# HSG-AIML/MaskedSST

Measured on AMD Instinct MI355X. Metric: pretrain samples/sec, higher is better.
Workload: dtype bf16; 1 GPU; SimMIM pretrain step (fwd+bwd+AdamW), EnMAP-shape cubes 8x8x200, depth 12x2, dim 96, heads 8, mlp 64, mask 0.7/4/tube, dropout 0.1; global_batch=256, per_gpu_batch=256, parallelism=dp1

## Files before the change

include/msst.h:

```cpp
#ifndef MSST_H
#define MSST_H
#include <stdint.h>

#ifdef __cplusplus
extern "C" {
#endif

#define MSST_VERSION 109
#define MSST_DIM 96
#define MSST_DIM_HEAD 64
#define MSST_MLP 64

#define MSST_PREC_F32 0
#define MSST_PREC_BF16 1

#define MSST_KERNEL_GENERIC (16 << 8)
#define MSST_KERNEL_FWD_4WAVE (64 << 8)
#define MSST_X1_BF16 (1024 << 8)
#define MSST_FWD_HALF (4096 << 8)
#define MSST_LSE_RENORM (8192 << 8)
#define MSST_LN1_FROM_XN (2048 << 8)
#define MSST_BWD_DEFER_REDUCE (512 << 8)
#define MSST_KERNEL_ATTN_R3 (128 << 8)

// ... 54 lines not shown
                            const float* b_emb, const float* post_g, const float* post_b, const float* dx0, float* slab,
                            int nchunk, float* dpre_g, float* dpre_b, float* dw_emb, float* db_emb, float* dpost_g,
                            float* dpost_b, float* dpos_a, float* dpos_b, int pos_split, int Bs, int Hs, int Ws, int window,
                            int stride, long win0, int nwin, int S, int P, float emb_dropout_p, uint32_t seed, void* stream);

int msst_tokenize_at_fwd(const float* scene, const int32_t* origins, const float* pre_g, const float* pre_b, const float* w_emb,
                         const float* b_emb, const float* post_g, const float* post_b, const float* pos_a, const float* pos_b,
                         int pos_split, float* out, int Bs, int Hs, int Ws, int window, int nwin, int S, int P,
                         float emb_dropout_p, uint32_t seed, void* stream);
int msst_tokenize_at_bwd(const float* scene, const int32_t* origins, const float* pre_g, const float* pre_b, const float* w_emb,
                         const float* b_emb, const float* post_g, const float* post_b, const float* dx0, float* slab, int nchunk,
                         float* dpre_g, float* dpre_b, float* dw_emb, float* db_emb, float* dpost_g, float* dpost_b, float* dpos_a,
                         float* dpos_b, int pos_split, int Bs, int Hs, int Ws, int window, int nwin, int S, int P,
                         float emb_dropout_p, uint32_t seed, void* stream);

int msst_tokenize_at_fwd_masked(const float* scene, const int32_t* origins, const float* pre_g, const float* pre_b, const float* w_emb,
                                const float* b_emb, const float* post_g, const float* post_b, const float* pos_a, const float* pos_b,
                                int pos_split, const float* mask_token, const uint8_t* mask, float* out, int Bs, int Hs, int Ws,
                                int window, int nwin, int S, int P, void* stream);
int msst_tokenize_at_bwd_masked(const float* scene, const int32_t* origins, const float* pre_g, const float* pre_b, const float* w_emb,
                                const float* b_emb, const float* post_g, const float* post_b, const uint8_t* mask, const float* dx0,
                                float* slab, int nchunk, float* dpre_g, float* dpre_b, float* dw_emb, float* db_emb, float* dpost_g,
                                float* dpost_b, float* dpos_a, float* dpos_b, int pos_split, float* dmask_token, int Bs, int Hs, int Ws,
                                int window, int nwin, int S, int P, void* stream);
int msst_head_at_fwd(const float* y, const float* scene, const int32_t* origins, const int32_t* idx, const float* w_pix,
                     const float* b_pix, int per_block, float* dpred, float* pred , float* partial, float* loss, int Bs,
                     int Hs, int Ws, int window, int nwin, int S, int P, int K, void* stream);

int msst_tokenize_at_fwd_orient(const float* scene, const int32_t* origins, const uint8_t* orient, const float* pre_g, const float* pre_b,
                                const float* w_emb, const float* b_emb, const float* post_g, const float* post_b, const float* pos_a,
                                const float* pos_b, int pos_split, float* out, int Bs, int Hs, int Ws, int window, int nwin, int S, int P,
                                float emb_dropout_p, uint32_t seed, void* stream);
int msst_tokenize_at_bwd_orient(const float* scene, const int32_t* origins, const uint8_t* orient, const float* pre_g, const float* pre_b,
                                const float* w_emb, const float* b_emb, const float* post_g, const float* post_b, const float* dx0,
                                float* slab, int nchunk, float* dpre_g, float* dpre_b, float* dw_emb, float* db_emb, float* dpost_g,
                                float* dpost_b, float* dpos_a, float* dpos_b, int pos_split, int Bs, int Hs, int Ws, int window, int nwin,
                                int S, int P, float emb_dropout_p, uint32_t seed, void* stream);
int msst_tokenize_at_fwd_masked_orient(const float* scene, const int32_t* origins, const uint8_t* orient, const float* pre_g,
                                       const float* pre_b, const float* w_emb, const float* b_emb, const float* post_g,
                                       const float* post_b, const float* pos_a, const float* pos_b, int pos_split,
                                       const float* mask_token, const uint8_t* mask, float* out, int Bs, int Hs, int Ws, int window,
                                       int nwin, int S, int P, void* stream);
int msst_tokenize_at_bwd_masked_orient(const float* scene, const int32_t* origins, const uint8_t* orient, const float* pre_g,
                                       const float* pre_b, const float* w_emb, const float* b_emb, const float* post_g,
                                       const float* post_b, const uint8_t* mask, const float* dx0, float* slab, int nchunk, float* dpre_g,
                                       float* dpre_b, float* dw_emb, float* db_emb, float* dpost_g, float* dpost_b, float* dpos_a,
                                       float* dpos_b, int pos_split, float* dmask_token, int Bs, int Hs, int Ws, int window, int nwin,
                                       int S, int P, void* stream);
int msst_head_at_fwd_orient(const float* y, const float* scene, const int32_t* origins, const uint8_t* orient, const int32_t* idx,
                            const float* w_pix, const float* b_pix, int per_block, float* dpred, float* pred , float* partial,
                            float* loss, int Bs, int Hs, int Ws, int window, int nwin, int S, int P, int K, void* stream);

int msst_scene_assemble(const float* win_logits, long win0, int nwin, float* logits, int64_t* classes, int Bs,
                        int n_classes, int Hs, int Ws, int window, int stride, int finalize, void* stream);

int msst_tokenize_scene_fwd_masked(const float* scene, const float* pre_g, const float* pre_b, const float* w_emb,
                                   const float* b_emb, const float* post_g, const float* post_b, const float* pos_a,
                                   const float* pos_b, int pos_split, const float* mask_token, const uint8_t* scene_mask, float* out,
                                   int Bs, int Hs, int Ws, int window, int stride, long win0, int nwin, int S, int P, void* stream);

int msst_scene_recon_assemble(const float* win_recon, long win0, int nwin, const float* scene, const uint8_t* scene_mask, float* cube,
                              double* band_err , int32_t* band_cnt , int32_t* cover, int Bs, int S, int P,
                              int Hs, int Ws, int window, int stride, int finalize, int blend, void* stream);

int msst_pool_spectral_fwd(const float* y, float* out, int B, int S, int N, void* stream);

int msst_scene_embed_assemble(const float* win_feat, long win0, int nwin, float* feat, int32_t* cover, int Bs, int D, int Hs, int Ws,
                              int window, int stride, int finalize, int l2norm, void* stream);

#define MSST_ATTN_PER_SEQ 0
#define MSST_ATTN_MEAN_SEQ 1
int msst_attn_maps(const float* x, const float* ln_g, const float* ln_b, const float* wqkv, float* maps, long sample_stride, int mode,
                   int B, int S, int N, int heads, int reduce, void* stream);

#define MSST_SAVED_XN 1
#define MSST_SAVED_LSE 2
#define MSST_SAVED_RSTD 4
long msst_block_lse_floats(int mode, int B, int S, int N, int heads);
long msst_block_tiles(int mode, int B, int S, int N);
int msst_block_fwd(const MsstBlockWeights* w , const float* x, float* y, float* x1, int mode,
                   int B, int S, int N, int heads, int prec, int max_grid, float dropout_p, uint32_t seed,
                   int layer, void* xn_out, float* lse_out, int* saved , void* stream);

int msst_block_fwd_stack(const MsstBlockWeights* const* w , int nblk, const float* x0, float* const* y ,
                         float* const* x1 , void* const* xn_out , float* const* lse_out , int mode,
                         int B, int S, int N, int heads, int prec, int max_grid, float dropout_p, uint32_t seed, int layer0,
                         int* saved , void* stream);

int msst_head_fwd(const float* y, const float* img, const int32_t* idx, const float* w_pix,
                  const float* b_pix, int per_block, float* dpred, float* pred, float* partial,
                  float* loss, int B, int S, int N, int P, int K, void* stream);

int msst_recon_fwd(const float* y, const float* img, const uint8_t* mask, const float* w_pix, const float* b_pix, int per_block,
                   int blend, float* recon, double* band_err , int32_t* band_cnt , int B, int S, int N,
                   int P, void* stream);


int msst_head_bwd(const float* y, const float* dpred, const int32_t* csr_ptr, const int32_t* csr_pos,
                  const float* w_pix, int per_block, float gscale, const float* gout, float* dy, float* slab,
                  int nchunk, float* dw_pix, float* db_pix, int B, int S, int N, int P, int K, void* stream);

typedef struct MsstBlockGrads {
    float* ln1_g; float* ln1_b; float* wqkv; float* wout; float* bo;
    float* ln2_g; float* ln2_b; float* w1; float* b1; float* w2; float* b2;
} MsstBlockGrads;

#define MSST_MLP_SLAB (64 * 96 + 96 * 64 + 64 + 96 + 96 + 96)
#define MSST_ATTN_SLAB (3 * 64 * 96 + 96 * 64)
#define MSST_LN1_SLAB 288

int msst_block_bwd(const MsstBlockWeights* w , const MsstBlockGrads* g , const float* x,
                   const float* x1, const float* dy, float* dx, float* dx1, void* dxn_part, float* slab,
                   int grid_rows, int nchunk, int mode, int B, int S, int N, int heads, int prec,
                   float dropout_p, uint32_t seed, int layer, const void* xn_saved ,
                   const float* lse_saved ,
                   void* dab_ws ,
                   void* stream);

#define MSST_TILE_QUEUE_WORDS 64
int msst_block_bwd_chain(const MsstBlockWeights* w , const MsstBlockGrads* g ,
                         const MsstBlockWeights* w_prev , const MsstBlockGrads* g_prev ,
                         const float* x, const float* x1, const float* x1_prev, const float* dy, float* dx, float* dx1,
                         void* dxn_part, float* slab, int grid_rows, int nchunk, int mode, int B, int S, int N, int heads,
                         int prec, float dropout_p, uint32_t seed, int layer, const void* xn_saved, const float* lse_saved ,
                         void* dab_ws, int first, int32_t* tile_queue , void* stream);

int msst_block_bwd_reduce(const MsstBlockGrads* g , const MsstBlockGrads* g_prev ,
                          float* slab, long slab_stride, long grad_stride, int count, int count_prev, int first,
                          int grid_rows, int nchunk, int mode, int B, int S, int N, int heads, int prec, void* stream);

int msst_tokenize_bwd(const float* img, const float* pre_g, const float* pre_b, const float* w_emb,
                      const float* b_emb, const float* post_g, const float* post_b, const uint8_t* mask,
                      const float* dx0, float* slab, int nchunk, float* dpre_g, float* dpre_b,
                      float* dw_emb, float* db_emb, float* dpost_g, float* dpost_b, float* dpos_a,
                      float* dpos_b, int pos_split, float* dmask_token, int B, int S, int N, int P,
                      float emb_dropout_p, uint32_t seed, void* stream);

int msst_tokenize_bwd_input(const float* img, const float* pre_g, const float* pre_b, const float* w_emb, const float* b_emb,
                            const float* post_g, const float* post_b, const uint8_t* mask , const float* dx0,
                            const float* dtarget , float* dimg, int B, int S, int N, int P, float emb_dropout_p,
                            uint32_t seed, void* stream);
int msst_head_bwd_target(const float* dpred, const int32_t* csr_ptr, const int32_t* csr_pos, const float* gout ,
                         float* dtarget, int B, int S, int N, int P, int K, void* stream);
int msst_tokenize_scene_bwd_input(const float* scene, const float* pre_g, const float* pre_b, const float* w_emb, const float* b_emb,
                                  const float* post_g, const float* post_b, const float* dx0, float* dscene, int Bs, int Hs, int Ws,
                                  int window, int stride, long win0, int nwin, int S, int P, float emb_dropout_p, uint32_t seed,
                                  void* stream);

int msst_tokenize_at_bwd_input(const float* scene, const int32_t* origins, const float* pre_g, const float* pre_b, const float* w_emb,
                               const float* b_emb, const float* post_g, const float* post_b, const float* dx0, float* dwin, int Bs,
                               int Hs, int Ws, int window, int nwin, int S, int P, float emb_dropout_p, uint32_t seed, void* stream);
int msst_scene_fold_at(const float* dwin, const int32_t* cell_ptr, const int32_t* cell_win, float* dscene, int Bs, int C, int Hs, int Ws,
                       int window, int nwin, int group, int accumulate, void* stream);

int msst_cls_head_fwd(const float* y, const float* ln_g, const float* ln_b, const float* w, const float* b,
                      float* logits, int B, int S, int N, int n_classes, void* stream);
int msst_cls_head_bwd(const float* y, const float* dlogits, const float* ln_g, const float* ln_b, const float* w,
                      float* dy, float* slab, float* dln_g, float* dln_b, float* dw, float* db, int B, int S,
                      int N, int n_classes, void* stream);

int msst_spec_head_fwd(const float* y, const float* ln_g, const float* ln_b, const float* w, const float* b,
                       float* logits, int B, int S, int N, int n_classes, void* stream);
long msst_spec_head_bwd_slab(int B, int S, int N, int n_classes);
int msst_spec_head_bwd(const float* y, const float* dlogits, const float* ln_g, const float* ln_b, const float* w,
                       float* dy, float* slab, float* dln_g, float* dln_b, float* dw, float* db, int B, int S,
                       int N, int n_classes, void* stream);
// ... 82 lines not shown
```

maskedsst_amd/_lib.py:

```python
import ctypes
import os
from ctypes import c_int, c_int32, c_uint32, c_long, c_float, c_void_p, c_char_p, POINTER, Structure

HERE = os.path.dirname(os.path.abspath(__file__))
LIB_PATH = os.path.join(HERE, "libmsst.so")
HEADER_PATH = os.path.normpath(os.path.join(HERE, "..", "include", "msst.h"))

PREC_F32 = 0
PREC_BF16 = 1
MODE_SPATIAL = 0
MODE_SPECTRAL = 1
MLP_SLAB = 64 * 96 + 96 * 64 + 64 + 96 + 96 + 96
ATTN_SLAB = 3 * 64 * 96 + 96 * 64
LN1_SLAB = 288


class MsstError(RuntimeError):
    pass


class MsstPrepJob(Structure):
    _fields_ = [("src", c_void_p), ("dst", c_void_p), ("rows", c_int32), ("cols", c_int32),
                ("transpose", c_int32), ("pack", c_int32), ("scale_rows", c_int32), ("scale", c_float)]


class MsstBlockWeights(Structure):
    _fields_ = [("struct_bytes", ctypes.c_uint64)] + [(n, c_void_p) for n in (
        "wqkv", "wout", "w1", "w2", "wqkvT", "woutT", "w1T", "w2T",
        "ln1_g", "ln1_b", "bo", "ln2_g", "ln2_b", "b1", "b2", "wqkv32", "woutT32", "wqkvT32",
        "wqkv_h", "wout_h", "w1_h", "w2_h")]


class MsstBlockGrads(Structure):
    _fields_ = [(n, c_void_p) for n in (
        "ln1_g", "ln1_b", "wqkv", "wout", "bo", "ln2_g", "ln2_b", "w1", "b1", "w2", "b2")]


class MsstAdamGroup(Structure):
    _fields_ = [("start", c_long), ("end", c_long), ("lr", c_float), ("weight_decay", c_float), ("step", c_int), ("flags", c_int)]


class MsstGradRange(Structure):
    _fields_ = [("start", c_long), ("end", c_long)]


_P = c_void_p
GRAD_MAX_RANGES = 64
ADAM_DECOUPLED = 1
ADAM_MAX_GROUPS = 64
BWD_DEFER_REDUCE = 512 << 8
X1_BF16 = 1024 << 8
SAVED_XN, SAVED_LSE, SAVED_RSTD = 1, 2, 4
LN1_FROM_XN = 2048 << 8
FWD_HALF = 4096 << 8
LSE_RENORM = 8192 << 8
PREP_HALF = 256
CE_LOSS_SUM, CE_N_VALID, CE_N_CORRECT, CE_BAD_LABELS, CE_NONFINITE, CE_SUPPORT = range(6)
CE_EXT_LOSS_SUM, CE_EXT_WEIGHT_SUM = range(2)
CE_CONFUSION_MAX_CLASSES = 128
ATTN_PER_SEQ, ATTN_MEAN_SEQ = 0, 1
_SIGS = {
    "msst_version": (c_int, []),
    "msst_last_error": (c_char_p, []),
    "msst_prep_weights": (c_int, [_P, c_int, c_int, c_int, c_int, _P, _P]),
    "msst_tokenize_fwd": (c_int, [_P] * 9 + [c_int, _P, _P, _P, c_int, c_int, c_int, c_int, c_float, c_uint32, _P]),
    "msst_tokenize_scene_fwd": (c_int, [_P] * 9 + [c_int, _P, c_int, c_int, c_int, c_int, c_int, c_long, c_int, c_int, c_int, _P]),
    "msst_tokenize_scene_fwd_train": (c_int, [_P] * 9 + [c_int, _P, c_int, c_int, c_int, c_int, c_int, c_long, c_int, c_int, c_int,
                                              c_float, c_uint32, _P]),
    "msst_tokenize_scene_bwd": (c_int, [_P] * 9 + [c_int] + [_P] * 8 + [c_int] * 6 + [c_long, c_int, c_int, c_int, c_float, c_uint32, _P]),
    "msst_tokenize_at_fwd": (c_int, [_P] * 10 + [c_int, _P] + [c_int] * 7 + [c_float, c_uint32, _P]),
    "msst_tokenize_at_bwd": (c_int, [_P] * 10 + [c_int] + [_P] * 8 + [c_int] * 8 + [c_float, c_uint32, _P]),
    "msst_tokenize_at_fwd_masked": (c_int, [_P] * 10 + [c_int, _P, _P, _P] + [c_int] * 7 + [_P]),
    "msst_tokenize_at_bwd_masked": (c_int, [_P] * 11 + [c_int] + [_P] * 8 + [c_int, _P] + [c_int] * 7 + [_P]),
    "msst_head_at_fwd": (c_int, [_P] * 6 + [c_int] + [_P] * 4 + [c_int] * 8 + [_P]),
    "msst_tokenize_at_fwd_orient": (c_int, [_P] * 11 + [c_int, _P] + [c_int] * 7 + [c_float, c_uint32, _P]),
    "msst_tokenize_at_bwd_orient": (c_int, [_P] * 11 + [c_int] + [_P] * 8 + [c_int] * 8 + [c_float, c_uint32, _P]),
    "msst_tokenize_at_fwd_masked_orient": (c_int, [_P] * 11 + [c_int, _P, _P, _P] + [c_int] * 7 + [_P]),
    "msst_tokenize_at_bwd_masked_orient": (c_int, [_P] * 12 + [c_int] + [_P] * 8 + [c_int, _P] + [c_int] * 7 + [_P]),
    "msst_head_at_fwd_orient": (c_int, [_P] * 7 + [c_int] + [_P] * 4 + [c_int] * 8 + [_P]),
    "msst_tokenize_bwd_input": (c_int, [_P] * 11 + [c_int] * 4 + [c_float, c_uint32, _P]),
    "msst_head_bwd_target": (c_int, [_P] * 5 + [c_int] * 5 + [_P]),
    "msst_tokenize_scene_bwd_input": (c_int, [_P] * 9 + [c_int] * 5 + [c_long, c_int, c_int, c_int, c_float, c_uint32, _P]),
    "msst_tokenize_at_bwd_input": (c_int, [_P] * 10 + [c_int] * 7 + [c_float, c_uint32, _P]),
    "msst_scene_fold_at": (c_int, [_P] * 4 + [c_int] * 8 + [_P]),
    "msst_tokenize_scene_fwd_masked": (c_int, [_P] * 9 + [c_int, _P, _P, _P, c_int, c_int, c_int, c_int, c_int, c_long, c_int, c_int, c_int, _P]),
    "msst_scene_recon_assemble": (c_int, [_P, c_long, c_int, _P, _P, _P, _P, _P, _P] + [c_int] * 9 + [_P]),
    "msst_pool_spectral_fwd": (c_int, [_P, _P, c_int, c_int, c_int, _P]),
    "msst_scene_embed_assemble": (c_int, [_P, c_long, c_int, _P, _P] + [c_int] * 8 + [_P]),
    "msst_attn_maps": (c_int, [_P, _P, _P, _P, _P, c_long, c_int, c_int, c_int, c_int, c_int, c_int, _P]),
    "msst_scene_assemble": (c_int, [_P, c_long, c_int, _P, _P, c_int, c_int, c_int, c_int, c_int, c_int, c_int, _P]),
    "msst_cls_head_fwd": (c_int, [_P] * 6 + [c_int, c_int, c_int, c_int, _P]),
    "msst_cls_head_bwd": (c_int, [_P] * 11 + [c_int, c_int, c_int, c_int, _P]),
    "msst_spec_head_fwd": (c_int, [_P] * 6 + [c_int, c_int, c_int, c_int, _P]),
    "msst_spec_head_bwd_slab": (c_long, [c_int, c_int, c_int, c_int]),
    "msst_spec_head_bwd": (c_int, [_P] * 11 + [c_int, c_int, c_int, c_int, _P]),
    "msst_pix_head_fwd_ws": (c_long, [c_int, c_int]),
    "msst_pix_head_fwd": (c_int, [_P] * 7 + [c_int, c_int, c_int, c_int, _P]),
    "msst_pix_head_bwd_slab": (c_long, [c_int, c_int, c_int, c_int]),
    "msst_pix_head_bwd": (c_int, [_P] * 11 + [c_int, c_int, c_int, c_int, _P]),
    "msst_scene_centre_assemble": (c_int, [_P, c_long, c_int, _P, _P, c_int, c_int, c_int, c_int, c_int, c_int, c_int, _P]),
    "msst_block_lse_floats": (c_long, [c_int, c_int, c_int, c_int, c_int]),
    "msst_block_tiles": (c_long, [c_int, c_int, c_int, c_int]),
    "msst_block_fwd": (c_int, [POINTER(MsstBlockWeights), _P, _P, _P, c_int, c_int, c_int, c_int, c_int,
                               c_int, c_int, c_float, c_uint32, c_int, _P, _P, POINTER(c_int), _P]),
    "msst_block_fwd_stack": (c_int, [_P, c_int, _P, _P, _P, _P, _P, c_int, c_int, c_int, c_int, c_int, c_int, c_int, c_float, c_uint32, c_int,
                                     POINTER(c_int), _P]),
    "msst_head_fwd": (c_int, [_P, _P, _P, _P, _P, c_int, _P, _P, _P, _P, c_int, c_int, c_int, c_int,
                              c_int, _P]),
    "msst_head_bwd": (c_int, [_P, _P, _P, _P, _P, c_int, c_float, _P, _P, _P, c_int, _P, _P, c_int, c_int, c_int,
                              c_int, c_int, _P]),
    "msst_block_bwd": (c_int, [POINTER(MsstBlockWeights), POINTER(MsstBlockGrads), _P, _P, _P, _P, _P, _P, _P,
                               c_int, c_int, c_int, c_int, c_int, c_int, c_int, c_int, c_float, c_uint32, c_int, _P, _P, _P, _P]),
    "msst_block_bwd_chain": (c_int, [POINTER(MsstBlockWeights), POINTER(MsstBlockGrads), POINTER(MsstBlockWeights),
                                     POINTER(MsstBlockGrads), _P, _P, _P, _P, _P, _P, _P, _P,
                                     c_int, c_int, c_int, c_int, c_int, c_int, c_int, c_int, c_float, c_uint32, c_int, _P, _P, _P,
                                     c_int, _P, _P]),
    "msst_block_bwd_reduce": (c_int, [POINTER(MsstBlockGrads), POINTER(MsstBlockGrads), _P, ctypes.c_long, ctypes.c_long,
                                      c_int, c_int, c_int, c_int, c_int, c_int, c_int, c_int, c_int, c_int, c_int, _P]),
    "msst_tokenize_bwd": (c_int, [_P] * 10 + [c_int] + [_P] * 8 + [c_int, _P, c_int, c_int, c_int, c_int, c_float,
                                  c_uint32, _P]),
    "msst_debug_stamps": (c_int, [_P]),
    "msst_debug_cu_thief": (c_int, [c_int, c_int, _P, _P]),
    "msst_debug_box_probe": (c_int, [_P, _P, c_long, _P]),
    "msst_profile_enable": (c_int, [c_int]),
    "msst_profile_select": (c_int, [ctypes.c_ulonglong]),
    "msst_profile_sample": (c_int, [c_int]),
    "msst_profile_kernels": (c_int, []),
    "msst_profile_name": (c_char_p, [c_int]),
    "msst_profile_collect": (c_int, [_P, _P]),
    "msst_layernorm_fwd": (c_int, [_P, _P, _P, _P, _P, _P, c_long, c_int, c_float, _P]),
    "msst_layernorm_bwd_slab": (c_long, [c_long, c_int]),
    "msst_layernorm_bwd": (c_int, [_P, _P, _P, _P, _P, _P, _P, c_long, c_int, c_float, _P]),
    "msst_ce_scratch_bytes": (c_long, [c_int, c_int, c_int]),
    "msst_ce_stats_fwd": (c_int, [_P, _P, _P, c_long, _P, _P, _P, _P, c_int, c_int, c_int, _P]),
    "msst_ce_bwd": (c_int, [_P, _P, _P, _P, c_int, c_int, c_int, _P]),
    "msst_ce_ext_scratch_bytes": (c_long, [c_int, c_int, c_int, c_int]),
    "msst_ce_ext_fwd": (c_int, [_P, _P, _P, c_long, _P, c_float, _P, _P, _P, _P, _P, _P, c_int, c_int, c_int, _P]),
    "msst_ce_ext_bwd": (c_int, [_P, _P, _P, _P, c_int, c_int, c_int, _P]),
    "msst_recon_fwd": (c_int, [_P, _P, _P, _P, _P, c_int, c_int, _P, _P, _P, c_int, c_int, c_int, c_int, _P]),
    "msst_adamw": (c_int, [_P, _P, _P, _P, c_long, c_float, c_float, c_float, c_float, c_float, c_int,
                           c_float, c_float, _P]),
    "msst_adam_groups": (c_int, [_P, _P, _P, _P, POINTER(MsstAdamGroup), c_int, c_int, ctypes.c_double, ctypes.c_double,
                                 c_float, c_float, _P]),
    "msst_grad_accum_scratch_bytes": (c_long, [c_int]),
    "msst_grad_accumulate": (c_int, [_P, _P, POINTER(MsstGradRange), c_int, c_int, c_int, _P, c_float, _P, _P]),
    "msst_grad_finalize": (c_int, [_P, _P, POINTER(MsstGradRange), c_int, c_int, c_float, c_float, _P, _P, _P]),
}

_lib = None


def declared_symbols():
    return sorted(_SIGS)


def header_version(path=None):
    import re
    with open(path or HEADER_PATH) as f:
        m = re.search(r"^#define\s+MSST_VERSION\s+(\d+)", f.read(), re.M)
    if not m:
        raise MsstError(f"no MSST_VERSION in {path or HEADER_PATH}")
    return int(m.group(1))


def load():
    global _lib
    if _lib is not None:
        return _lib
    if not os.path.exists(LIB_PATH):
        raise MsstError(
            f"{LIB_PATH} not found: build the HIP extension first (python -m maskedsst_amd.build). "
            "maskedsst_amd has no CPU / eager fallback.")
    lib = ctypes.CDLL(LIB_PATH)
    for name, (res, args) in _SIGS.items():
        fn = getattr(lib, name, None)
        if fn is None:
            raise MsstError(f"libmsst.so does not export {name} (stale build? run python -m maskedsst_amd.build)")
        fn.restype = res
        fn.argtypes = args
    got, want = int(lib.msst_version()), header_version()
    if got == -want and os.environ.get("MSST_ALLOW_LAB") == "1":
        import warnings
        warnings.warn("maskedsst_amd: loading a -DMSST_LAB kernel-study build (results may be wrong by design)")
        got = want
    if got != want:
        raise MsstError(
            f"{LIB_PATH} reports msst_version() = {got}, include/msst.h says MSST_VERSION {want}: "
# ... 11 lines not shown
```

maskedsst_amd/build.py:

```python
import os
import subprocess
import sys
from concurrent.futures import ThreadPoolExecutor

HERE = os.path.dirname(os.path.abspath(__file__))
CSRC = os.path.join(HERE, "csrc")
LIB = os.path.join(HERE, "libmsst.so")
SOURCES = ["msst_fwd.hip", "msst_fwd3.hip", "msst_bwd.hip", "msst_bwd3.hip", "msst_bwd4.hip", "msst_bwd5.hip", "msst_ln.hip", "msst_opt.hip", "msst_accum.hip", "msst_head.hip", "msst_pixhead.hip", "msst_loss.hip", "msst_recon.hip", "msst_scene_recon.hip", "msst_scene_embed.hip", "msst_input_grad.hip", "msst_attn_maps.hip", "msst_api.hip"]
HEADERS = ["msst_dev.h", "msst_kernels.h", os.path.join("..", "..", "include", "msst.h")]
FLAGS = ["--offload-arch=gfx950", "-O3", "-std=c++17", "-fPIC", "-fno-gpu-rdc", "-Wno-unused-result"]


def _hipcc():
    for c in (os.environ.get("HIPCC"), "/opt/rocm/bin/hipcc", "hipcc"):
        if c and (os.path.isabs(c) and os.path.exists(c) or not os.path.isabs(c)):
            return c
    return "hipcc"


def _stale(target, deps):
    if not os.path.exists(target):
        return True
    t = os.path.getmtime(target)
    return any(os.path.getmtime(d) > t for d in deps if os.path.exists(d))


def build(force=False, verbose=False, extra_flags=(), lib=None, tag=None):
    srcs = [os.path.join(CSRC, s) for s in SOURCES if os.path.exists(os.path.join(CSRC, s))]
    hdrs = [os.path.normpath(os.path.join(CSRC, h)) for h in HEADERS]
    objdir = os.path.join(HERE, "build", tag) if tag else os.path.join(HERE, "build")
    LIB = lib or globals()["LIB"]
    os.makedirs(objdir, exist_ok=True)
    hipcc = _hipcc()

    def compile_one(src):
        obj = os.path.join(objdir, os.path.basename(src) + ".o")
        if force or _stale(obj, [src] + hdrs):
            cmd = [hipcc] + FLAGS + list(extra_flags) + ["-c", src, "-o", obj]
            if verbose:
                print(" ".join(cmd), flush=True)
            r = subprocess.run(cmd, capture_output=True, text=True)
            if r.returncode != 0:
                raise RuntimeError(f"hipcc failed for {src}:\n{r.stdout}\n{r.stderr}")
        return obj

    with ThreadPoolExecutor(max_workers=4) as ex:
        objs = list(ex.map(compile_one, srcs))
    if force or _stale(LIB, objs):
        cmd = [hipcc, "--offload-arch=gfx950", "-shared", "-fPIC", "-o", LIB] + objs
        if verbose:
            print(" ".join(cmd), flush=True)
        r = subprocess.run(cmd, capture_output=True, text=True)
        if r.returncode != 0:
            raise RuntimeError(f"link failed:\n{r.stdout}\n{r.stderr}")
    return LIB


if __name__ == "__main__":
    print(build(force="--force" in sys.argv or "--stamps" in sys.argv, verbose=True,
                extra_flags=("-DMSST_STAMPS",) if "--stamps" in sys.argv else ()))
```

maskedsst_amd/csrc/msst_api.hip:

```cpp
#include "../../include/msst.h"
#include "msst_kernels.h"
#include <stdio.h>
#include <stdlib.h>
#include <string.h>
#include <math.h>
#include <atomic>
#include <mutex>
#include <vector>

namespace msst {

static thread_local char g_err[256] = "";

static int fail(int code, const char* what) {
    if (code > 0) snprintf(g_err, sizeof(g_err), "%s: hip error %d (%s)", what, code, hipGetErrorString((hipError_t)code));
    else if (code < 0) snprintf(g_err, sizeof(g_err), "%s: msst error %d", what, code);
    return code;
}

template <class E>
__global__ __launch_bounds__(256) void prep_weights_kernel(const MsstPrepJob* jobs, int* err_flag) {
    const MsstPrepJob j = jobs[blockIdx.y];
    const bool half = sizeof(E) == 2 && (j.pack & MSST_PREP_HALF);
    if (j.pack < 0 || (j.pack & ~MSST_PREP_HALF) > 1 || (sizeof(E) != 2 && (j.pack & MSST_PREP_HALF)) || j.rows < 1 || j.cols < 1) {
// ... 434 lines not shown
    hipStream_t st = (hipStream_t)stream;
    int rc = launch_scene_fold(a, win_logits, logits, n_classes, 16, scene_call_rows(a, wps), st);
    if (!rc && finalize) rc = launch_scene_finalize(a, st);
    return fail(rc, "msst_scene_assemble");
}

int msst_scene_recon_assemble(const float* win_recon, long win0, int nwin, const float* scene, const uint8_t* scene_mask, float* cube,
                              double* band_err, int32_t* band_cnt, int32_t* cover, int Bs, int S, int P, int Hs, int Ws, int window,
                              int stride, int finalize, int blend, void* stream) {
    if (Bs < 1 || S < 1 || P < 1 || Hs < 1 || Ws < 1 || window < 1 || stride < 1 || nwin < 0 || win0 < 0)
        return fail(MSST_ERR_BADARG, "msst_scene_recon_assemble");
    if (stride > window || window > Hs || window > Ws || window * window > 64 || S > 64 || P > 16)
        return fail(MSST_ERR_UNSUPPORTED, "msst_scene_recon_assemble (1 <= stride <= window <= Hs, Ws; window * window <= 64, S <= 64, P <= 16)");
    if ((nwin > 0 && !win_recon) || !scene || !scene_mask || !cube || !cover || (band_err == nullptr) != (band_cnt == nullptr))
        return fail(MSST_ERR_BADARG, "msst_scene_recon_assemble (null argument, or one of band_err / band_cnt without the other)");
    int nr = 0, nq = 0;
    scene_grid(Bs, Hs, Ws, window, stride, &nr, &nq);
    const long wps = (long)nr * nq;
    if (win0 + nwin > (long)Bs * wps) return fail(MSST_ERR_BADARG, "msst_scene_recon_assemble (windows out of range)");
    if (((long)Bs * Hs * Ws + 255) / 256 > 0x7fffffffL || (long)Bs * S * P > 0x7fffffffL) return fail(MSST_ERR_UNSUPPORTED, "msst_scene_recon_assemble (scene batch too large)");
    SceneReconArgs a;
    fill_grid(a, win0, nwin, Bs, Hs, Ws, window, stride, nr, nq);
    a.win_recon = win_recon; a.scene = scene; a.scene_mask = scene_mask; a.cube = cube; a.band_err = band_err; a.band_cnt = band_cnt;
    a.cover = cover; a.S = S; a.P = P; a.blend = blend != 0;
    hipStream_t st = (hipStream_t)stream;
    int rc = launch_scene_fold(a, win_recon, cube, S * P, P, scene_call_rows(a, wps), st);
    if (!rc && finalize) rc = launch_scene_recon_finalize(a, st);
    return fail(rc, "msst_scene_recon_assemble");
}

int msst_pool_spectral_fwd(const float* y, float* out, int B, int S, int N, void* stream) {
    if (B < 1 || S < 1 || N < 1) return fail(MSST_ERR_BADARG, "msst_pool_spectral_fwd");
    if (N > 64 || S > 64) return fail(MSST_ERR_UNSUPPORTED, "msst_pool_spectral_fwd (N <= 64, S <= 64)");
    if (!y || !out || ((uintptr_t)y & 15)) return fail(MSST_ERR_BADARG, "msst_pool_spectral_fwd (null argument, or y not 16-byte aligned)");
    return fail(launch_pool_spectral(y, out, B, S, N, (hipStream_t)stream), "msst_pool_spectral_fwd");
}

int msst_attn_maps(const float* x, const float* ln_g, const float* ln_b, const float* wqkv, float* maps, long sample_stride, int mode,
                   int B, int S, int N, int heads, int reduce, void* stream) {
    if (B < 1 || S < 1 || N < 1 || heads < 1) return fail(MSST_ERR_BADARG, "msst_attn_maps");
    if (N > 64 || S > 64 || heads > 16) return fail(MSST_ERR_UNSUPPORTED, "msst_attn_maps (N <= 64, S <= 64, heads <= 16)");
    if ((mode != MSST_MODE_SPATIAL && mode != MSST_MODE_SPECTRAL) || (reduce != MSST_ATTN_PER_SEQ && reduce != MSST_ATTN_MEAN_SEQ))
        return fail(MSST_ERR_BADARG, "msst_attn_maps (mode or reduce outside {0, 1})");
    if (!x || !ln_g || !ln_b || !wqkv || !maps || ((uintptr_t)x & 15) || ((uintptr_t)maps & 15))
        return fail(MSST_ERR_BADARG, "msst_attn_maps (null argument, or x / maps not 16-byte aligned)");
    const long L = mode == MSST_MODE_SPATIAL ? N : S, G = mode == MSST_MODE_SPATIAL ? S : N;
    if (sample_stride < (reduce == MSST_ATTN_PER_SEQ ? G : 1) * heads * L * L)
        return fail(MSST_ERR_BADARG, "msst_attn_maps (sample_stride smaller than one sample's maps)");
    return fail(launch_attn_maps(x, ln_g, ln_b, wqkv, maps, sample_stride, mode, B, S, N, heads, reduce, (hipStream_t)stream),
                "msst_attn_maps");
}

int msst_scene_embed_assemble(const float* win_feat, long win0, int nwin, float* feat, int32_t* cover, int Bs, int D, int Hs, int Ws,
                              int window, int stride, int finalize, int l2norm, void* stream) {
    if (Bs < 1 || D < 1 || Hs < 1 || Ws < 1 || window < 1 || stride < 1 || nwin < 0 || win0 < 0)
        return fail(MSST_ERR_BADARG, "msst_scene_embed_assemble");
    if (stride > window || window > Hs || window > Ws || window * window > 64 || D > 128)
        return fail(MSST_ERR_UNSUPPORTED, "msst_scene_embed_assemble (1 <= stride <= window <= Hs, Ws; window * window <= 64, D <= 128)");
    if ((nwin > 0 && !win_feat) || !feat || (finalize && !cover)) return fail(MSST_ERR_BADARG, "msst_scene_embed_assemble (null argument)");
    int nr = 0, nq = 0;
    scene_grid(Bs, Hs, Ws, window, stride, &nr, &nq);
    const long wps = (long)nr * nq;
    if (win0 + nwin > (long)Bs * wps) return fail(MSST_ERR_BADARG, "msst_scene_embed_assemble (windows out of range)");
    if (((long)Bs * Hs * Ws + 255) / 256 > 0x7fffffffL) return fail(MSST_ERR_UNSUPPORTED, "msst_scene_embed_assemble (scene batch too large)");
    SceneEmbedArgs a;
    fill_grid(a, win0, nwin, Bs, Hs, Ws, window, stride, nr, nq);
    a.win_feat = win_feat; a.feat = feat; a.cover = cover; a.D = D; a.l2norm = l2norm != 0;
    hipStream_t st = (hipStream_t)stream;
    int rc = launch_scene_fold(a, win_feat, feat, D, 16, scene_call_rows(a, wps), st);
    if (!rc && finalize) rc = launch_scene_embed_finalize(a, st);
    return fail(rc, "msst_scene_embed_assemble");
}

long msst_block_lse_floats(int mode, int B, int S, int N, int heads) {
    if (B < 1 || S < 1 || N < 1 || heads < 1 || N > 64 || S > 64) return 0;
    return (long)ntiles_of(make_tilemap(mode, B, S, N)) * heads * 64 + (long)B * S * N;
}

long msst_block_tiles(int mode, int B, int S, int N) {
    if (B < 1 || S < 1 || N < 1 || N > 64 || S > 64) return 0;
    return (long)ntiles_of(make_tilemap(mode, B, S, N));
}

int msst_block_fwd(const MsstBlockWeights* w, const float* x, float* y, float* x1, int mode, int B, int S,
                   int N, int heads, int prec, int max_grid, float dropout_p, uint32_t seed, int layer,
                   void* xn_out, float* lse_out, int* saved, void* stream) {
    if (int rc = block_shape(mode, B, S, N, heads)) return fail(rc, "msst_block_fwd (B, S, N, heads < 1, mode not 0 / 1, or sequence length > 64)");
    if (!bw_ok(w) || !x || !y || x == y) return fail(MSST_ERR_BADARG, "msst_block_fwd (null argument, or MsstBlockWeights of another header revision)");
    const int dbg = (prec >> 8) & 0xffff;
    prec &= 0xff;
    BlockArgs a;
    a.w = to_bw(w);
    a.x = x; a.y = y; a.x1 = x1;
    a.tm = make_tilemap(mode, B, S, N);
    a.ntiles = ntiles_of(a.tm);
    a.max_grid = max_grid > 0 ? max_grid : a.ntiles;
    a.H = heads;
    a.scale = 0.125f;
    a.dbg = dbg & ~8;
    a.stamps = nullptr;
#ifdef MSST_STAMPS
    a.stamps = g_stamps;
    if (g_stamps) a.dbg = dbg;
#elif defined(MSST_LAB)
    a.stamps = g_stamps;
#endif
    a.x1_bf16 = (dbg & 1024) ? 1 : 0;
    if (a.x1_bf16 && !(prec == MSST_PREC_BF16 && heads == 8 && !(dbg & (16 | 64))))
        return fail(MSST_ERR_UNSUPPORTED, "msst_block_fwd (MSST_X1_BF16 needs the role-split bf16 forward: 8 heads, no MSST_KERNEL_* flags)");
    a.half = (dbg & 4096) ? 1 : 0;
    if (a.half) {
        if (!(prec == MSST_PREC_BF16 && heads == 8 && !(dbg & (16 | 64))))
            return fail(MSST_ERR_UNSUPPORTED, "msst_block_fwd (MSST_FWD_HALF needs the role-split bf16 forward: 8 heads, no MSST_KERNEL_* flags)");
        if (!w->wqkv_h || !w->wout_h || !w->w1_h || !w->w2_h) return fail(MSST_ERR_BADARG, "msst_block_fwd (MSST_FWD_HALF without the half weight copies)");
        a.w.wqkv = w->wqkv_h; a.w.wout = w->wout_h; a.w.w1 = w->w1_h; a.w.w2 = w->w2_h;
    }
    a.drop = make_drop(dropout_p, seed, layer);
    a.xn_out = (xn_out && block_fwd_writes_xn(a, prec)) ? xn_out : nullptr;
    a.lse_out = (lse_out && block_fwd_writes_lse(a, prec)) ? lse_out : nullptr;
    if (saved) *saved = (a.xn_out ? MSST_SAVED_XN : 0) | (a.lse_out ? (MSST_SAVED_LSE | MSST_SAVED_RSTD) : 0);
    return fail(launch_block_fwd(a, prec, (hipStream_t)stream), "msst_block_fwd");
}

int msst_block_fwd_stack(const MsstBlockWeights* const* w, int nblk, const float* x0, float* const* y, float* const* x1,
                         void* const* xn_out, float* const* lse_out, int mode, int B, int S, int N, int heads, int prec, int max_grid,
                         float dropout_p, uint32_t seed, int layer0, int* saved, void* stream) {
    if (int rc = block_shape(mode, B, S, N, heads)) return fail(rc, "msst_block_fwd_stack (B, S, N, heads < 1, mode not 0 / 1, or sequence length > 64)");
    if (!w || !x0 || !y || nblk < 1) return fail(MSST_ERR_BADARG, "msst_block_fwd_stack");
    if (nblk > MSST_MAX_STACK) return fail(MSST_ERR_UNSUPPORTED, "msst_block_fwd_stack (more than 16 blocks)");
    const int dbg = (prec >> 8) & 0xffff;
    prec &= 0xff;
    if (prec != MSST_PREC_BF16 || heads != 8 || (dbg & ~(1024 | 4096))) return fail(MSST_ERR_UNSUPPORTED, "msst_block_fwd_stack (bf16, 8 heads, no MSST_KERNEL_* flags)");
    const bool half = (dbg & 4096) != 0;
    for (int j = 0; j < nblk; ++j) {
        if (!bw_ok(w[j])) return fail(MSST_ERR_BADARG, "msst_block_fwd_stack (null block, or MsstBlockWeights of another header revision)");
        if (half && (!w[j]->wqkv_h || !w[j]->wout_h || !w[j]->w1_h || !w[j]->w2_h)) return fail(MSST_ERR_BADARG, "msst_block_fwd_stack (MSST_FWD_HALF without the half weight copies)");
    }
    StackArgs sa;
    BlockArgs& a = sa.base;
    memset(&a.w, 0, sizeof(a.w));
    a.x = x0; a.y = nullptr; a.x1 = nullptr; a.xn_out = nullptr; a.lse_out = nullptr;
    a.tm = make_tilemap(mode, B, S, N);
    a.ntiles = ntiles_of(a.tm);
    a.max_grid = max_grid > 0 ? max_grid : a.ntiles;
    a.H = heads;
    a.scale = 0.125f;
    a.dbg = 0;
    a.stamps = nullptr;
    a.x1_bf16 = (dbg & 1024) ? 1 : 0;
    a.half = half ? 1 : 0;
    a.drop = make_drop(dropout_p, seed, layer0);
    if (lse_out && !block_fwd_writes_lse(a, prec)) lse_out = nullptr;
    sa.nblk = nblk;
    auto blk_of = [&](int j, const float* xin) {
        StackBlk sb;
        sb.wqkv = half ? w[j]->wqkv_h : w[j]->wqkv; sb.wout = half ? w[j]->wout_h : w[j]->wout;
        sb.w1 = half ? w[j]->w1_h : w[j]->w1; sb.w2 = half ? w[j]->w2_h : w[j]->w2;
        sb.ln1_g = w[j]->ln1_g; sb.ln1_b = w[j]->ln1_b; sb.bo = w[j]->bo; sb.ln2_g = w[j]->ln2_g; sb.ln2_b = w[j]->ln2_b; sb.b1 = w[j]->b1; sb.b2 = w[j]->b2;
        sb.x = xin; sb.y = y[j]; sb.x1 = x1 ? x1[j] : nullptr; sb.xn_out = xn_out ? xn_out[j] : nullptr; sb.lse_out = lse_out ? lse_out[j] : nullptr;
        sb.layer = layer0 + j; sb.pad_ = 0;
        return sb;
    };
    for (int j = 0; j < nblk; ++j)
        if (!bw_ok(w[j]) || !y[j] || y[j] == (j ? y[j - 1] : x0))
            return fail(MSST_ERR_BADARG, "msst_block_fwd_stack (null argument, or MsstBlockWeights of another header revision)");
    sa.b0 = blk_of(0, x0);
    memset(&sa.st, 0, sizeof(sa.st));
    bool affine = true;
    if (nblk > 1) {
        const StackBlk b1 = blk_of(1, y[0]);
        auto dist = [&](const void* p1, const void* p0, int& out) {
            const long d = (const char*)p1 - (const char*)p0;
            if (d > 0x7fffffffL || d < -0x7fffffffL) affine = false;
            out = (int)d;
        };
        dist(b1.wqkv, sa.b0.wqkv, sa.st.wqkv); dist(b1.wout, sa.b0.wout, sa.st.wout); dist(b1.w1, sa.b0.w1, sa.st.w1); dist(b1.w2, sa.b0.w2, sa.st.w2);
        dist(b1.ln1_g, sa.b0.ln1_g, sa.st.ln1_g); dist(b1.ln1_b, sa.b0.ln1_b, sa.st.ln1_b); dist(b1.bo, sa.b0.bo, sa.st.bo);
        dist(b1.ln2_g, sa.b0.ln2_g, sa.st.ln2_g); dist(b1.ln2_b, sa.b0.ln2_b, sa.st.ln2_b); dist(b1.b1, sa.b0.b1, sa.st.b1); dist(b1.b2, sa.b0.b2, sa.st.b2);
        dist(b1.y, sa.b0.y, sa.st.y); dist(b1.x1, sa.b0.x1, sa.st.x1); dist(b1.xn_out, sa.b0.xn_out, sa.st.xn_out); dist(b1.lse_out, sa.b0.lse_out, sa.st.lse_out);
        sa.st.x = sa.st.y;
        const float* xin = y[0];
        for (int j = 1; j < nblk && affine; ++j) {
            const StackBlk bj = blk_of(j, xin);
            auto same = [&](const void* pj, const void* p0, int stride) { return !p0 ? !pj : (const char*)pj == (const char*)p0 + (long)j * stride; };
            affine = same(bj.wqkv, sa.b0.wqkv, sa.st.wqkv) && same(bj.wout, sa.b0.wout, sa.st.wout) && same(bj.w1, sa.b0.w1, sa.st.w1) &&
                     same(bj.w2, sa.b0.w2, sa.st.w2) && same(bj.ln1_g, sa.b0.ln1_g, sa.st.ln1_g) && same(bj.ln1_b, sa.b0.ln1_b, sa.st.ln1_b) &&
                     same(bj.bo, sa.b0.bo, sa.st.bo) && same(bj.ln2_g, sa.b0.ln2_g, sa.st.ln2_g) && same(bj.ln2_b, sa.b0.ln2_b, sa.st.ln2_b) &&
                     same(bj.b1, sa.b0.b1, sa.st.b1) && same(bj.b2, sa.b0.b2, sa.st.b2) && same(bj.y, sa.b0.y, sa.st.y) &&
                     same(bj.x1, sa.b0.x1, sa.st.x1) && same(bj.xn_out, sa.b0.xn_out, sa.st.xn_out) && same(bj.lse_out, sa.b0.lse_out, sa.st.lse_out);
            xin = y[j];
        }
    }
    if (!affine) return fail(MSST_ERR_UNSUPPORTED, "msst_block_fwd_stack (per-block operands not a constant stride apart)");
    sa.x_rest = nblk > 1 ? reinterpret_cast<const float*>(reinterpret_cast<const char*>(y[0]) - (long)sa.st.y) : x0;
    if (saved) *saved = (xn_out ? MSST_SAVED_XN : 0) | (lse_out ? (MSST_SAVED_LSE | MSST_SAVED_RSTD) : 0);
    if (a.ntiles < 1) return 0;
    int ncu = 256, dev = 0;
    hipGetDevice(&dev);
    if (hipDeviceGetAttribute(&ncu, hipDeviceAttributeMultiprocessorCount, dev) != hipSuccess || ncu < 1) ncu = 256;
    int grid = a.max_grid < a.ntiles ? a.max_grid : a.ntiles;
    if (grid > ncu) grid = ncu;
    return fail(launch_block_fwd_rs_stack(sa, grid, (hipStream_t)stream), "msst_block_fwd_stack");
}

// ... 831 lines not shown
```

maskedsst_amd/csrc/msst_fwd.hip:

```cpp
#include <atomic>
#include "msst_dev.h"
#include "msst_kernels.h"

namespace msst {

enum { TOK_BATCH = 0, TOK_SCENE = 1, TOK_SCENE_MASKED = 2, TOK_AT = 3, TOK_AT_MASKED = 4, TOK_AT_OR = 5, TOK_AT_OR_MASKED = 6 };
template <int SRC>
__device__ __forceinline__ const float* tok_window_origin(const TokArgs& a, int b) {
    if constexpr (SRC == TOK_AT || SRC == TOK_AT_MASKED || SRC == TOK_AT_OR || SRC == TOK_AT_OR_MASKED) return listed_window_origin(a, b);
    else return scene_window_origin(a, b);
}
template <int PC, int SRC>
__device__ __forceinline__ void tokenize_fwd_body(const TokArgs& a) {
    constexpr bool SCENE = SRC != TOK_BATCH, NOMASK = SRC == TOK_SCENE || SRC == TOK_AT || SRC == TOK_AT_OR;
    constexpr bool ORIENT = SRC == TOK_AT_OR || SRC == TOK_AT_OR_MASKED;
    __shared__ float patch[16][64];
    __shared__ float W[96][17];
    __shared__ float bias[96];
    const int c = blockIdx.x, b = blockIdx.y, tid = threadIdx.x;
    const int P = PC ? PC : a.P, N = a.N;
    if constexpr (SCENE) {
        const long plane = (long)a.Hs * a.Ws;
        const float* src = tok_window_origin<SRC>(a, b) + (long)c * P * plane;
        WinSteps ws{};
// ... 765 lines not shown
                a.dpred[((long)b * a.K + k) * P + p] = d > 0.f ? 1.f : (d < 0.f ? -1.f : 0.f);
                if (a.pred) a.pred[((long)b * a.K + k) * P + p] = pred;
            }
        }
    }
#pragma unroll
    for (int o = 32; o > 0; o >>= 1) lsum += __shfl_xor(lsum, o);
    if ((tid & 63) == 0) red[tid >> 6] = lsum;
    __syncthreads();
    if (tid == 0) a.partial[blockIdx.y * gridDim.x + blockIdx.x] = (red[0] + red[1]) + (red[2] + red[3]);
}

__global__ __launch_bounds__(256) void loss_reduce_kernel(const float* partial, int n, float scale, float* loss) {
    __shared__ double red[256];
    double s = 0.0;
    for (int i = threadIdx.x; i < n; i += 256) s += (double)partial[i];
    red[threadIdx.x] = s;
    __syncthreads();
    for (int o = 128; o > 0; o >>= 1) {
        if (threadIdx.x < o) red[threadIdx.x] += red[threadIdx.x + o];
        __syncthreads();
    }
    if (threadIdx.x == 0) *loss = (float)(red[0] * (double)scale);
}

template <int SRC>
static int launch_tokenize_fwd_src(const TokArgs& a, hipStream_t st) {
    if (a.P > 16 || a.N > 64) return MSST_ERR_UNSUPPORTED;
    if (SRC != TOK_BATCH && a.B < 1) return 0;
    ProfScope ps(K_TOK_FWD, st);
    if (a.P == 10 && a.N == 64) {
        int nchunk = 1024 / (a.S > 0 ? a.S : 1);
        if (nchunk < 1) nchunk = 1;
        if (nchunk > a.B) nchunk = a.B;
        hipLaunchKernelGGL(tokenize_fwd_mfma_kernel<SRC>, dim3(a.S, nchunk), dim3(256), 0, st, a);
    } else {
        if (SRC != TOK_BATCH && a.B > 65535) return MSST_ERR_UNSUPPORTED;
        if (a.P == 10) hipLaunchKernelGGL((tokenize_fwd_kernel<10, SRC>), dim3(a.S, a.B), dim3(256), 0, st, a);
        else hipLaunchKernelGGL((tokenize_fwd_kernel<0, SRC>), dim3(a.S, a.B), dim3(256), 0, st, a);
    }
    return (int)hipGetLastError();
}
int launch_tokenize_fwd(const TokArgs& a, hipStream_t st) { return launch_tokenize_fwd_src<TOK_BATCH>(a, st); }
int launch_tokenize_scene_fwd(const TokArgs& a, hipStream_t st) { return launch_tokenize_fwd_src<TOK_SCENE>(a, st); }
int launch_tokenize_scene_fwd_masked(const TokArgs& a, hipStream_t st) { return launch_tokenize_fwd_src<TOK_SCENE_MASKED>(a, st); }
int launch_tokenize_at_fwd(const TokArgs& a, hipStream_t st) { return launch_tokenize_fwd_src<TOK_AT>(a, st); }
int launch_tokenize_at_fwd_masked(const TokArgs& a, hipStream_t st) { return launch_tokenize_fwd_src<TOK_AT_MASKED>(a, st); }
int launch_tokenize_at_fwd_orient(const TokArgs& a, bool masked, hipStream_t st) {
    return masked ? launch_tokenize_fwd_src<TOK_AT_OR_MASKED>(a, st) : launch_tokenize_fwd_src<TOK_AT_OR>(a, st);
}

template <class P>
static int launch_block_fwd_t(const BlockArgs& a, int grid, hipStream_t st) {
    static std::atomic<bool> attr_set{false};
    const size_t smem = sizeof(FwdSmem<P>);
    if (!attr_set) {
        hipError_t e = hipFuncSetAttribute(reinterpret_cast<const void*>(&block_fwd_kernel<P>),
                                           hipFuncAttributeMaxDynamicSharedMemorySize, (int)smem);
        if (e != hipSuccess) return (int)e;
        attr_set = true;
    }
    ProfScope ps(K_BLOCK_FWD, st);
    hipLaunchKernelGGL(block_fwd_kernel<P>, dim3(grid), dim3(256), smem, st, a);
    return (int)hipGetLastError();
}

static int launch_block_fwd_bf16(const BlockArgs& a, int grid, hipStream_t st) {
    static std::atomic<bool> attr_set{false};
    const size_t smem = sizeof(FwdSmem<PBF16>) + 640 * sizeof(float) + 24 * 1024;
    if (!attr_set) {
        hipError_t e = hipFuncSetAttribute(reinterpret_cast<const void*>(&block_fwd_bf16_kernel),
                                           hipFuncAttributeMaxDynamicSharedMemorySize, (int)smem);
        if (e != hipSuccess) return (int)e;
        attr_set = true;
    }
    ProfScope ps(K_BLOCK_FWD, st);
    hipLaunchKernelGGL(block_fwd_bf16_kernel, dim3(grid), dim3(256), smem, st, a);
    return (int)hipGetLastError();
}

int launch_block_fwd(const BlockArgs& a, int prec, hipStream_t st) {
    if (a.tm.L > 64 || a.tm.L < 1) return MSST_ERR_UNSUPPORTED;
    if (a.ntiles < 1) return 0;
    if (prec == MSST_PREC_F32 || (a.dbg & 16)) {
        const int grid = a.ntiles < a.max_grid ? a.ntiles : a.max_grid;
        return prec == MSST_PREC_F32 ? launch_block_fwd_t<PF32>(a, grid, st) : launch_block_fwd_t<PBF16>(a, grid, st);
    }
    if (a.H == 8 && !(a.dbg & 64)) {
        static std::atomic<int> ncu_cached{0};
        int ncu = ncu_cached.load(std::memory_order_relaxed);
        if (!ncu) {
            int dev = 0;
            hipGetDevice(&dev);
            if (hipDeviceGetAttribute(&ncu, hipDeviceAttributeMultiprocessorCount, dev) != hipSuccess || ncu < 1) ncu = 256;
            ncu_cached.store(ncu, std::memory_order_relaxed);
        }
        int grid = a.max_grid < a.ntiles ? a.max_grid : a.ntiles;
        if (grid > ncu) grid = ncu;
        return launch_block_fwd_rs(a, grid, st);
    }
    int grid = a.max_grid < a.ntiles ? a.max_grid : a.ntiles;
    if (grid > 512) grid = 512;
    return launch_block_fwd_bf16(a, grid, st);
}

bool block_fwd_writes_lse(const BlockArgs& a, int prec) {
    return prec == MSST_PREC_BF16 && a.H == 8 && !(a.dbg & (16 | 64)) && (long)a.ntiles * a.H * 256 < 0x7fffffffL;
}

bool block_fwd_writes_xn(const BlockArgs& a, int prec) {
    return prec == MSST_PREC_BF16 && !(a.dbg & 16);
}

template <bool AT, bool ORIENT = false>
static int launch_head_fwd_src(const HeadArgs& a, float* loss, hipStream_t st) {
    if (a.P > 16) return MSST_ERR_UNSUPPORTED;
    dim3 grid((a.K + 63) / 64, a.B);
    { ProfScope ps(K_HEAD_FWD, st);
    hipLaunchKernelGGL((head_fwd_kernel<AT, ORIENT>), grid, dim3(256), 0, st, a); }
    const int np = grid.x * grid.y;
    const float scale = 1.0f / ((float)a.B * (float)a.K * (float)a.P) / (float)a.K;
    ProfScope ps(K_LOSS_REDUCE, st);
    hipLaunchKernelGGL(loss_reduce_kernel, dim3(1), dim3(256), 0, st, a.partial, np, scale, loss);
    return (int)hipGetLastError();
}
int launch_head_fwd(const HeadArgs& a, float* loss, hipStream_t st) { return launch_head_fwd_src<false>(a, loss, st); }
int launch_head_at_fwd(const HeadArgs& a, float* loss, hipStream_t st) { return launch_head_fwd_src<true>(a, loss, st); }
int launch_head_at_fwd_orient(const HeadArgs& a, float* loss, hipStream_t st) { return launch_head_fwd_src<true, true>(a, loss, st); }

}

namespace msst {

__global__ __launch_bounds__(256) void cls_head_fwd_kernel(ClsArgs a) {
    const int b = blockIdx.x, tid = threadIdx.x, n = tid >> 2, part = tid & 3;
    if (n >= a.N) return;
    float m[24];
#pragma unroll
    for (int i = 0; i < 24; ++i) m[i] = 0.f;
    for (int c = 0; c < a.S; ++c) {
        const f32x4* src = reinterpret_cast<const f32x4*>(a.y + ((long)b * a.T + c * a.N + n) * 96 + part * 24);
#pragma unroll
        for (int i = 0; i < 6; ++i) { const f32x4 t4 = src[i]; m[4*i] += t4[0]; m[4*i+1] += t4[1]; m[4*i+2] += t4[2]; m[4*i+3] += t4[3]; }
    }
    const float invS = 1.f / a.S;
    float s = 0.f;
#pragma unroll
    for (int i = 0; i < 24; ++i) { m[i] *= invS; s += m[i]; }
    s += __shfl_xor(s, 1); s += __shfl_xor(s, 2);
    const float mean = s * (1.f / 96.f);
    float vs = 0.f;
#pragma unroll
    for (int i = 0; i < 24; ++i) { const float d = m[i] - mean; vs += d * d; }
    vs += __shfl_xor(vs, 1); vs += __shfl_xor(vs, 2);
    const float rstd = rsqrtf(vs * (1.f / 96.f) + 1e-5f);
#pragma unroll
    for (int i = 0; i < 24; ++i) m[i] = (m[i] - mean) * rstd * a.ln_g[part * 24 + i] + a.ln_b[part * 24 + i];
    for (int k = 0; k < a.NC; ++k) {
        float acc = 0.f;
#pragma unroll
        for (int i = 0; i < 24; ++i) acc += a.w[k * 96 + part * 24 + i] * m[i];
        acc += __shfl_xor(acc, 1); acc += __shfl_xor(acc, 2);
        if (part == 0) a.logits[((long)b * a.NC + k) * a.N + n] = acc + a.b[k];
    }
}

int launch_cls_head_fwd(const ClsArgs& a, hipStream_t st) {
    if (a.N > 64) return MSST_ERR_UNSUPPORTED;
    hipLaunchKernelGGL(cls_head_fwd_kernel, dim3(a.B), dim3(256), 0, st, a);
    return (int)hipGetLastError();
}

__global__ __launch_bounds__(256) void scene_fold_kernel(SceneGrid a, const float* src, float* dst, int C, int group, long pixels) {
    const long p = (long)blockIdx.x * 256 + threadIdx.x;
    if (p >= pixels) return;
    const int c0 = blockIdx.y * group, cn = min(group, C - c0);
    const long R = a.row0 + p / a.Ws;
    const int x = (int)(p % a.Ws);
    const long s = R / a.Hs;
    const int y = (int)(R - s * a.Hs);
// ... 68 lines not shown
```

maskedsst_amd/csrc/msst_fwd3.hip:

```cpp
#include <atomic>
#include "msst_dev.h"
#include "msst_kernels.h"
#include <type_traits>

#ifndef MSST_F3_RING
#define MSST_F3_RING 4
#endif
#ifndef MSST_F3_RPRIO
#define MSST_F3_RPRIO 1
#endif
#ifndef MSST_F3_BAND
#define MSST_F3_BAND 1
#endif
#ifndef MSST_F3_GROUP
#define MSST_F3_GROUP 10
#endif
#if defined(MSST_LAB) && !defined(MSST_LAB_X1OLD)
#define MSST_LAB_X1OLD 0
#endif
#if !defined(MSST_LAB) || !defined(MSST_LAB_NOLSE)
#define MSST_F3_LSE_STORE 1
#else
#define MSST_F3_LSE_STORE 0
#endif
// ... 37 lines not shown
    int seqb[4][64];
    float lnp[2][640];
    float lseb[2][256];
    char wmlp[24 * 1024];
    const char* blktab[MSST_MAX_STACK][16];
    unsigned steptab[1024];
};
constexpr int F3_MAX_STEPS = 1024;
constexpr int BT_WQKV = 0, BT_W1 = 2, BT_LN1G = 4, BT_X = 11;

struct StepBlk {
    const elem* wqkv; const elem* wout;
    const float* x; float* y; float* x1; elem* xn_out;
    int layer;
};

__device__ __forceinline__ int sopaque3(int v) {
    asm volatile("" : "+s"(v));
    return v;
}

template <bool HALF>
__device__ __forceinline__ s16x4 cv4(f32x4 c) {
    if constexpr (HALF) return f2h4(c); else return f2bf4(c);
}
template <bool HALF>
__device__ __forceinline__ f32x4 mma16(frag a, frag b, f32x4 c) {
    if constexpr (HALF) {
        typedef _Float16 h8 __attribute__((ext_vector_type(8)));
        return __builtin_amdgcn_mfma_f32_16x16x32_f16(__builtin_bit_cast(h8, a), __builtin_bit_cast(h8, b), c, 0, 0, 0);
    } else return P::mma(a, b, c);
}
template <bool HALF>
__device__ __forceinline__ frag pack2f(f32x4 lo, f32x4 hi) {
    const s16x4 a = cv4<HALF>(lo), b = cv4<HALF>(hi);
    frag r;
    r[0] = a[0]; r[1] = a[1]; r[2] = a[2]; r[3] = a[3];
    r[4] = b[0]; r[5] = b[1]; r[6] = b[2]; r[7] = b[3];
    return r;
}

__device__ __forceinline__ frag ld_w_gather3(const elem* w, int K, int row32, int k0, int voff) {
    const int f = (row32 >> 4) * (K >> 5) + (k0 >> 5);
    const __amdgpu_buffer_rsrc_t rs = __builtin_amdgcn_make_buffer_rsrc(const_cast<elem*>(w), 0, 0x7fffffff, 0x00020000);
    const u32x4 v = __builtin_amdgcn_raw_buffer_load_b128(rs, voff, f * 1024, 0);
    return __builtin_bit_cast(frag, v);
}

#ifndef MSST_F3_WOFF
#define MSST_F3_WOFF 1
#endif
__device__ __forceinline__ frag ld_wb3(const elem* w, int voff, int soff) {
    const __amdgpu_buffer_rsrc_t rs = __builtin_amdgcn_make_buffer_rsrc(const_cast<elem*>(w), 0, 0x7fffffff, 0x00020000);
    return __builtin_bit_cast(frag, __builtin_amdgcn_raw_buffer_load_b128(rs, voff, soff, 0));
}
__device__ __forceinline__ void load_pair3(int pi, frag (&out)[2], const elem* wqkv, int H, int h, const int (&voff)[2], int hb, int HB, int l16) {
    if (MSST_F3_WOFF) {
        if (pi < 12) {
            const int st = pi / 3, ks = pi % 3;
            const int o = hb + (st >> 1) * HB + (st & 1) * 6144 + ks * 1024;
            out[0] = ld_wb3(wqkv, l16, o);
            out[1] = ld_wb3(wqkv, l16, o + 3072);
        } else {
            const int mm = (pi - 12) / 3, ks = (pi - 12) % 3;
            const int o = hb + 2 * HB + mm * 6144 + ks * 1024;
            out[0] = ld_wb3(wqkv, voff[0], o);
            out[1] = ld_wb3(wqkv, voff[1], o);
        }
    } else if (pi < 12) {
        const int st = pi / 3, ks = pi % 3;
        const int r0 = ((st >> 1) * H + h) * 64 + (st & 1) * 32;
        out[0] = P::ld_w(wqkv, 96, r0, ks * 32);
        out[1] = P::ld_w(wqkv, 96, r0 + 16, ks * 32);
    } else {
        const int mm = (pi - 12) / 3, ks = (pi - 12) % 3;
        const int r32 = (2 * H + h) * 64 + mm * 32;
        out[0] = ld_w_gather3(wqkv, 96, r32, ks * 32, voff[0]);
        out[1] = ld_w_gather3(wqkv, 96, r32, ks * 32, voff[1]);
    }
}

}

template <bool DROP, bool STACK, bool HALF>
__global__ __launch_bounds__(512, 2) void block_fwd_rs_kernel(typename std::conditional<STACK, StackArgs, BlockArgs>::type args) {
    const BlockArgs& a = [&]() -> const BlockArgs& { if constexpr (STACK) return args.base; else return args; }();
    typedef Fwd3Smem SM;
    constexpr int LDX = SM::LDX, LDH = SM::LDH, LDO = SM::LDO;
    extern __shared__ __attribute__((aligned(16))) char smem_raw[];
    SM& sm = *reinterpret_cast<SM*>(smem_raw);

    const int tid = threadIdx.x, wv = __builtin_amdgcn_readfirstlane(tid >> 6), l = tid & 63, g = l >> 4, c = l & 15;
    const int H = a.H, inner = H * 64;
    const TileMap tm = a.tm;
    const int L = tm.L;
    const int G = (int)gridDim.x;
    const int nmine = ((int)blockIdx.x < a.ntiles) ? (a.ntiles - 1 - (int)blockIdx.x) / G + 1 : 0;
    int nsteps = nmine;
    if constexpr (STACK) {
        const int nblk = args.nblk;
        const int ng = max(1, nmine / MSST_F3_GROUP), gbase = nmine / ng, gextra = nmine - gbase * ng;
        const int p1 = max(gbase + 1, 3), p0 = max(gbase, 3);
        nsteps = nmine ? nblk * (gextra * p1 + (ng - gextra) * p0) : 0;
        for (int s_ = tid; s_ < nsteps; s_ += 512) {
            const int head = gextra * nblk * p1;
            int j, r, pp, sz, before;
            if (s_ < head) { j = s_ / (nblk * p1); r = s_ - j * nblk * p1; pp = p1; sz = gbase + 1; before = j * (gbase + 1); }
            else { j = gextra + (s_ - head) / (nblk * p0); r = s_ - head - (j - gextra) * nblk * p0; pp = p0; sz = gbase; before = gextra * (gbase + 1) + (j - gextra) * gbase; }
            const int blk = r / pp, pos = r - blk * pp;
            const unsigned idle = pos >= sz ? 1u : 0u;
            sm.steptab[s_] = (unsigned)(before + min(pos, sz - 1)) | ((unsigned)blk << 16) | ((unsigned)((j * nblk + blk) & 1) << 24) | (idle << 31);
        }
    }
    if constexpr (STACK) {
        static_assert(offsetof(StackBlk, lse_out) == 15 * 8 && offsetof(StackStride, lse_out) == 15 * 4, "blktab follows StackBlk's member order");
        for (int e = tid; e < args.nblk * 16; e += 512) {
            const int j = e >> 4, f = e & 15;
            auto kp = (const __attribute__((address_space(4))) char*)__builtin_amdgcn_kernarg_segment_ptr();
            const char* p0 = *(const char* const __attribute__((address_space(4)))*)(kp + offsetof(StackArgs, b0) + f * 8);
            const int stride = *(const int __attribute__((address_space(4)))*)(kp + offsetof(StackArgs, st) + f * 4);
            const char* pj = p0 ? p0 + (long)j * stride : nullptr;
            if (f == BT_X && j) pj = reinterpret_cast<const char*>(args.x_rest) + (long)j * args.st.y;
            sm.blktab[j][f] = pj;
        }
    }
    constexpr unsigned F3_IDLE = 0x80000000u;
    auto load_word = [&](int k) -> unsigned {
        if constexpr (STACK) return (k >= 0 && k < nsteps) ? (unsigned)__builtin_amdgcn_readfirstlane((int)sm.steptab[k]) : F3_IDLE;
        else return (k >= 0 && k < nmine) ? (unsigned)k : F3_IDLE;
    };
    int kc = 0;
    unsigned swm2 = F3_IDLE, swm1 = F3_IDLE, sw0 = F3_IDLE, swp1 = F3_IDLE, swp2 = F3_IDLE;
    auto step_word = [&](int k) -> unsigned {
        if constexpr (!STACK) return load_word(k);
        else { const int d = k - kc; return d == 0 ? sw0 : d == 1 ? swp1 : d == -1 ? swm1 : d == 2 ? swp2 : d == -2 ? swm2 : load_word(k); }
    };
    auto words_init = [&]() { kc = 0; swm2 = F3_IDLE; swm1 = F3_IDLE; sw0 = load_word(0); swp1 = load_word(1); swp2 = load_word(2); };
    auto words_advance = [&]() { swm2 = swm1; swm1 = sw0; sw0 = swp1; swp1 = swp2; swp2 = load_word(kc + 3); };
    auto tile_at = [&](int k) -> int {
        const unsigned w_ = step_word(k);
        return (w_ >> 31) ? -1 : (int)blockIdx.x + (int)(w_ & 0xffffu) * G;
    };
    auto blk_at = [&](int k) -> int { if constexpr (STACK) return (int)((step_word(k) >> 16) & 0xffu); else return 0; };
    auto slot_at = [&](int k) -> int { if constexpr (STACK) return (int)((step_word(k) >> 24) & 1u); else return 0; };
    auto in_walk = [&](int k) -> bool { return k >= 0 && k < nsteps; };
    auto epoch_differs = [&](int k1, int k0) -> bool {
        if constexpr (STACK) return in_walk(k1) && in_walk(k0) && ((step_word(k1) ^ step_word(k0)) & 0x01ff0000u) != 0u;
        else return false;
    };
    auto at_blk = [&](const void* p0, int stride, int blk) -> const char* { return reinterpret_cast<const char*>(p0) + (long)blk * (long)stride; };
    auto step_blk = [&](int k) -> StepBlk {
        StepBlk q;
        if constexpr (STACK) {
            const int j = blk_at(k);
            const StackBlk& b0 = args.b0;
            const StackStride& st = args.st;
            q.wqkv = reinterpret_cast<const elem*>(at_blk(b0.wqkv, st.wqkv, j)); q.wout = reinterpret_cast<const elem*>(at_blk(b0.wout, st.wout, j));
            q.x = reinterpret_cast<const float*>(sm.blktab[j][BT_X]);
            q.y = reinterpret_cast<float*>(const_cast<char*>(sm.blktab[j][BT_X + 1]));
            q.x1 = reinterpret_cast<float*>(const_cast<char*>(sm.blktab[j][BT_X + 2]));
            q.xn_out = reinterpret_cast<elem*>(const_cast<char*>(sm.blktab[j][BT_X + 3]));
            q.layer = b0.layer + j;
        } else {
            q.wqkv = reinterpret_cast<const elem*>(a.w.wqkv); q.wout = reinterpret_cast<const elem*>(a.w.wout);
            q.x = a.x; q.y = a.y; q.x1 = a.x1; q.xn_out = reinterpret_cast<elem*>(a.xn_out); q.layer = a.drop.layer;
        }
        return q;
    };
    auto drop_at = [&](int k) -> Drop { Drop d = a.drop; if constexpr (STACK) d.layer = args.b0.layer + blk_at(k); return d; };
    auto lnp_at = [&](int k) -> const float* { return sm.lnp[slot_at(k)]; };
    struct LnpRegs { float v[7]; };
    auto fetch_lnp = [&](int blk, int t96) -> LnpRegs {
        const float *g1, *b1_, *bo, *g2, *b2_, *bb2, *bb1;
        if constexpr (STACK) {
            auto fp_ = [&](int f) { return reinterpret_cast<const float*>(sm.blktab[blk][f]); };
            g1 = fp_(BT_LN1G); b1_ = fp_(BT_LN1G + 1); bo = fp_(BT_LN1G + 2); g2 = fp_(BT_LN1G + 3); b2_ = fp_(BT_LN1G + 4); bb1 = fp_(BT_LN1G + 5); bb2 = fp_(BT_LN1G + 6);
        }
        else { g1 = a.w.ln1_g; b1_ = a.w.ln1_b; bo = a.w.bo; g2 = a.w.ln2_g; b2_ = a.w.ln2_b; bb2 = a.w.b2; bb1 = a.w.b1; }
        LnpRegs r;
        r.v[0] = g1[t96]; r.v[1] = b1_[t96]; r.v[2] = bo[t96]; r.v[3] = g2[t96]; r.v[4] = b2_[t96]; r.v[5] = bb2[t96];
        r.v[6] = bb1[t96 < 64 ? t96 : 0];
        return r;
    };
    auto commit_lnp = [&](int slot, int t96, const LnpRegs& r) {
        float* lnp = sm.lnp[slot];
#pragma unroll
        for (int i = 0; i < 6; ++i) lnp[96 * i + t96] = r.v[i];
        if (t96 < 64) lnp[576 + t96] = r.v[6];
    };
    auto load_lnp = [&](int slot, int blk, int t96) { commit_lnp(slot, t96, fetch_lnp(blk, t96)); };
    auto mlp_w = [&](int blk, int which) -> const char* {
        if constexpr (STACK) return sm.blktab[blk][BT_W1 + which];
        else return reinterpret_cast<const char*>(which ? a.w.w2 : a.w.w1);
    };

    if (STACK) __syncthreads();
    words_init();
    if (tid < 96) load_lnp(slot_at(0), blk_at(0), tid);
#pragma unroll
    for (int i3 = 0; i3 < 3; ++i3) {
        const int f = wv * 3 + i3;
        dma_frag(f < 12 ? mlp_w(blk_at(0), 0) + f * 1024 : mlp_w(blk_at(0), 1) + (f - 12) * 1024, sm.wmlp + f * 1024);
    }
    wait_vm0();
    if (tid < 64) {
        const int sq = tid / L, ps = tid - sq * L;
        sm.rowmap[tid] = ((unsigned)(sq >= tm.TS ? 0xffff : sq) << 16) | (unsigned)ps;
    }
    auto fill_seq = [&](int k, int t64) {
        const int tile_ = tile_at(k);
        const int q = tile_ * tm.TS + t64;
        int base = -1;
        if (tile_ >= 0 && t64 < tm.TS && q < tm.nseq) {
            if (tm.mode == 0) base = q * tm.N;
            else { const int b = tm.nshift >= 0 ? (q >> tm.nshift) : q / tm.N; base = b * tm.T + (q - b * tm.N); }
        }
        sm.seqb[k & 3][t64] = base;
    };
    if (tid < 64) { fill_seq(0, tid); fill_seq(1, tid); }
    if (tid >= 64 && tid < 128) {
        const int r = tid - 64, sq = r / L;
        unsigned long long m = ~0ull;
        if (sq < tm.TS && L < 64) m = ((1ull << L) - 1ull) << (sq * L);
        sm.vm[r] = m;
    }
    __syncthreads();
    auto tok_of = [&](int k, int r) -> long {
        const unsigned sp = sm.rowmap[r];
        const int base = sm.seqb[k & 3][min((int)(sp >> 16), 63)];
        return ((sp >> 16) == 0xffffu || base < 0) ? -1 : (long)(base + (int)(sp & 0xffffu) * (tm.mode == 0 ? 1 : tm.N));
    };

    if (wv < 4) {
        int voff[2];
#pragma unroll
        for (int hi = 0; hi < 2; ++hi) {
            const int rs = 8 * (c >> 2) + (c & 3) + 4 * hi;
            voff[hi] = ((rs >> 4) * 3) * 1024 + (g * 16 + (rs & 15)) * 16;
        }
        bool band = L < 64 && MSST_F3_BAND;
#pragma unroll
        for (int j = 0; j < 4; ++j) {
            const int s_lo = (16 * j) / L, s_hi = min((16 * j + 15) / L, tm.TS - 1);
            const int k_lo = s_lo * L, k_hi = (s_hi + 1) * L - 1;
            const unsigned allow = j == 0 ? 0x3u : j == 1 ? 0x7u : j == 2 ? 0xeu : 0xcu;
            for (int t = 0; t < 4; ++t)
                if (s_lo <= s_hi && 16 * t <= k_hi && 16 * t + 15 >= k_lo && !((allow >> t) & 1u)) band = false;
        }
        constexpr int NR = MSST_F3_RING;
        static_assert(NR >= 2 && NR <= 9, "ring depth");
        frag ring[NR][2];
        auto next_pair = [](int pi) { return pi + NR < 18 ? pi + NR : pi % NR; };
        const int HB = H * 12288, l16 = l * 16;
        {
            const elem* wq0 = step_blk(0).wqkv;
#pragma unroll
            for (int pi = 0; pi < NR; ++pi) load_pair3(pi, ring[pi], wq0, H, wv, voff, wv * 12288, HB, l16);
        }

        __syncthreads();
        for (kc = 0; kc < nsteps; ++kc) {
            const int k = kc;
            const int tile = tile_at(k);
            const StepBlk sb = step_blk(k);
            const elem* wqkv = sb.wqkv;
            const elem* wqkv_next = (STACK && k + 1 < nsteps) ? step_blk(k + 1).wqkv : sb.wqkv;
            const Drop drop_k = drop_at(k);
#ifdef MSST_STAMPS
            const bool stamp_on = (a.dbg & 8) && a.stamps && blockIdx.x == 100 && l == 0 && k == nsteps / 2;
#endif
            F3_STAMP(0);
#pragma unroll
            for (int rd = 0; rd < 2; ++rd) {
                const elem* wq_wrap = rd == 1 ? wqkv_next : wqkv;
                const int h = wv + 4 * rd;
                const int hn = wv + 4 * (1 - rd);
                const int hb_c = sopaque3(h * 12288), hb_n = sopaque3(hn * 12288);
                frag qB[4][2], kA[4][2], vA[4][2];
                {
// ... 90 lines not shown
                                    for (int r = 0; r < 4; ++r) mx[u] = fmaxf(mx[u], s[u][t][r]);
                        } else {
#pragma unroll
                            for (int u = 0; u < 2; ++u) {
                                const unsigned long long vmq = sm.vm[(2 * jp + u) * 16 + cq];
                                const int vlo = (int)(unsigned)vmq, vhi = (int)(unsigned)(vmq >> 32);
#pragma unroll
                                for (int t = 0; t < 4; ++t) {
                                    if (!((NM[u] >> t) & 1u)) continue;
#pragma unroll
                                    for (int r = 0; r < 4; ++r) {
                                        const int m = __builtin_amdgcn_sbfe(t < 2 ? vlo : vhi, 16 * (t & 1) + sh0 + r, 1);
                                        const float v = __int_as_float((__float_as_int(s[u][t][r]) & m) | (~m & (int)0xff800000));
                                        s[u][t][r] = v;
                                        mx[u] = fmaxf(mx[u], v);
                                    }
                                }
                            }
                        }
                        float mc[2], sum[2] = {0.f, 0.f}, inv[2];
#pragma unroll
                        for (int u = 0; u < 2; ++u) mc[u] = colgroup_max(mx[u]) * cs;
#pragma unroll
                        for (int t = 0; t < 4; ++t)
#pragma unroll
                            for (int u = 0; u < 2; ++u) {
                                if (!((NM[u] >> t) & 1u)) continue;
#pragma unroll
                                for (int r = 0; r < 4; ++r) { const float e = __builtin_amdgcn_exp2f(fmaf(s[u][t][r], cs, -mc[u])); s[u][t][r] = e; sum[u] += e; }
                            }
#pragma unroll
                        for (int u = 0; u < 2; ++u) {
                            const float st = colgroup_sum(sum[u]);
                            inv[u] = (DROP ? drop_k.scale : 1.f) * __builtin_amdgcn_rcpf(st);
                            if (MSST_F3_LSE_STORE) sm.lseb[rd][wv * 64 + (2 * jp + u) * 16 + cq] = mc[u] + __builtin_amdgcn_logf(st);
                        }
#pragma unroll
                        for (int u = 0; u < 2; ++u) {
#pragma unroll
                            for (int t = 0; t < 4; ++t) {
                                if (!((NM[u] >> t) & 1u)) continue;
                                s[u][t] = s[u][t] * inv[u];
                                if (DROP) {
                                    s[u][t] = drop4_noscale(drop_k, 1, (unsigned)(((tile * H + h) * 64 + (2 * jp + u) * 16 + cq) * 16 + t * 4 + (sh0 >> 2)), s[u][t]);
                                }
                            }
                        }
                    }
#pragma unroll
                    for (int u = 0; u < 2; ++u) {
                        const frag p0 = pack2f<HALF>(s[u][0], s[u][1]), p1 = pack2f<HALF>(s[u][2], s[u][3]);
#pragma unroll
                        for (int dd = 0; dd < 4; ++dd) {
                            o[u][dd] = zero4();
                            if (NM[u] & 3u) o[u][dd] = mma16<HALF>(vA[dd][0], p0, o[u][dd]);
                            if (NM[u] & 12u) o[u][dd] = mma16<HALF>(vA[dd][1], p1, o[u][dd]);
                        }
                    }
                    int l4 = threadIdx.x & 63;
                    asm volatile("" : "+v"(l4));
#pragma unroll
                    for (int u = 0; u < 2; ++u) {
                        elem* orow = &sm.ob[rd][(2 * jp + u) * 16 + (l4 & 15)][wv * 64 + 8 * (l4 >> 4)];
                        *reinterpret_cast<frag*>(orow) = pack2f<HALF>(o[u][0], o[u][1]);
                        *reinterpret_cast<frag*>(orow + 32) = pack2f<HALF>(o[u][2], o[u][3]);
                    }
                    F3_STAMP(2 + 5 * rd + 2 * jp);
                    lds_barrier();
                    F3_STAMP(3 + 5 * rd + 2 * jp);
                };
                typedef std::integral_constant<int, 0> I0;
                typedef std::integral_constant<int, 1> I1;
                if (L == 64) {
                    attn_pair(I0{}, std::false_type{}, std::integral_constant<int, 0xf>{}, std::integral_constant<int, 0xf>{});
                    attn_pair(I1{}, std::false_type{}, std::integral_constant<int, 0xf>{}, std::integral_constant<int, 0xf>{});
                } else if (band) {
                    attn_pair(I0{}, std::true_type{}, std::integral_constant<int, 0x3>{}, std::integral_constant<int, 0x7>{});
                    attn_pair(I1{}, std::true_type{}, std::integral_constant<int, 0xe>{}, std::integral_constant<int, 0xc>{});
                } else {
                    attn_pair(I0{}, std::true_type{}, std::integral_constant<int, 0xf>{}, std::integral_constant<int, 0xf>{});
                    attn_pair(I1{}, std::true_type{}, std::integral_constant<int, 0xf>{}, std::integral_constant<int, 0xf>{});
                }
            }
            if constexpr (STACK) words_advance();
        }
#pragma unroll
        for (int i = 0; i < 4; ++i) lds_barrier();
        return;
    }

    const int rw = wv - 4, mh = rw & 1, rh = rw >> 1;
    const int rt = tid - 256;

    f32x4 xv[6];
    auto request_ln1 = [&](int k) {
        int rt = (int)threadIdx.x - 256;
        asm volatile("" : "+v"(rt));
        const long tok = tok_of(k, rt >> 2);
        const float* xrow = step_blk(k).x + (tok >= 0 ? tok : 0) * 96 + 4 * (rt & 3);
#pragma unroll
        for (int i = 0; i < 6; ++i) xv[i] = *reinterpret_cast<const f32x4*>(xrow + 16 * i);
    };
    auto ln1 = [&](int k) {
        int rt = (int)threadIdx.x - 256;
        asm volatile("" : "+v"(rt));
        const int lr = rt >> 2, part = rt & 3;
        const long tok = tok_of(k, lr);
        const float* lnp = lnp_at(k);
        elem* const xn_out = step_blk(k).xn_out;
        float* stats;
        if constexpr (STACK) stats = reinterpret_cast<float*>(const_cast<char*>(sm.blktab[blk_at(k)][BT_X + 4]));
        else stats = a.lse_out;
        float v[24];
#pragma unroll
        for (int i = 0; i < 6; ++i) { v[4*i] = xv[i][0]; v[4*i+1] = xv[i][1]; v[4*i+2] = xv[i][2]; v[4*i+3] = xv[i][3]; }
        if (tok < 0) {
#pragma unroll
            for (int i = 0; i < 24; ++i) v[i] = 0.f;
        }
        float s = 0.f;
#pragma unroll
        for (int i = 0; i < 24; ++i) s += v[i];
        const float mean = quad_sum(s) * (1.f / 96.f);
        float vs = 0.f;
#pragma unroll
        for (int i = 0; i < 24; ++i) { const float d = v[i] - mean; vs += d * d; }
        const float rstd = rsqrtf(quad_sum(vs) * (1.f / 96.f) + 1e-5f);
        if (MSST_F3_RSTD_STORE && stats && tok >= 0 && part == 0) stats[(long)a.ntiles * H * 64 + tok] = rstd;
#pragma unroll
        for (int i = 0; i < 6; ++i) {
            const int f0 = 16 * i + 4 * part;
            f32x4 n4;
#pragma unroll
            for (int e = 0; e < 4; ++e) n4[e] = (v[4*i+e] - mean) * rstd * lnp[f0 + e] + lnp[96 + f0 + e];
            const s16x4 nb = f2bf4(n4);
            *reinterpret_cast<s16x4*>(&sm.xn[k & 1][lr][f0]) = HALF ? cv4<HALF>(n4) : nb;
            if (xn_out && tok >= 0) *reinterpret_cast<s16x4*>(xn_out + tok * 96 + f0) = nb;
        }
    };

    f32x4 acc[2][3];
    f32x4 x1r[2][3];
    f32x4 xr[2][3];
    float mean_w[2], m2_w[2], mean_r[2] = {0.f, 0.f};
#define F3_LANE() int l3 = threadIdx.x & 63; asm volatile("" : "+v"(l3)); const int g3 = l3 >> 4, c3 = l3 & 15; (void)g3; (void)c3

    auto request_xr = [&](int k) {
        F3_LANE();
#pragma unroll
        for (int jj = 0; jj < 2; ++jj) {
            const long tok = tok_of(k, 32 * rh + 16 * jj + c3);
            const float* xrow = step_blk(k).x + (tok >= 0 ? tok : 0) * 96 + 48 * mh + 4 * g3;
#pragma unroll
            for (int i = 0; i < 3; ++i) xr[jj][i] = *reinterpret_cast<const f32x4*>(xrow + 16 * i);
        }
    };
    frag fw[8][3];
    auto request_fw = [&](int rd, int kstep) {
        const elem* wout = step_blk(kstep).wout;
#pragma unroll
        for (int s8 = 0; s8 < 8; ++s8)
#pragma unroll
            for (int i = 0; i < 3; ++i) fw[s8][i] = P::ld_w(wout, inner, (3 * sopaque3(mh) + i) * 16, (8 * rd + s8) * 32);
    };
    auto outproj = [&](int rd) {
        F3_LANE();
        frag fo[4][2];
// ... 164 lines not shown
        }
    };
    auto copy_lse = [&](int k, int rd) {
        if (!MSST_F3_LSE_STORE) return;
        const int tile_ = tile_at(k);
        float* stats;
        if constexpr (STACK) stats = reinterpret_cast<float*>(const_cast<char*>(sm.blktab[blk_at(k)][BT_X + 4]));
        else stats = a.lse_out;
        if (!stats || tile_ < 0) return;
        int rt_ = (int)threadIdx.x - 256;
        asm volatile("" : "+v"(rt_));
        stats[((long)tile_ * H + 4 * rd) * 64 + rt_] = sm.lseb[rd][rt_];
    };
    auto zero_acc = [&]() {
#pragma unroll
        for (int jj = 0; jj < 2; ++jj)
#pragma unroll
            for (int i = 0; i < 3; ++i) acc[jj][i] = zero4();
    };

    request_ln1(0);
    ln1(0);
    zero_acc();
    request_fw(0, 0);
    __syncthreads();
    if (MSST_F3_RPRIO) __builtin_amdgcn_s_setprio(MSST_F3_RPRIO);
    bool lnp_switch = false;
    LnpRegs lnp_regs = {};
    for (kc = 0; kc <= nsteps; ++kc) {
        const int k = kc;
        const bool have_prev = k >= 1, have_cur = k < nsteps;
#ifdef MSST_STAMPS
        const bool stamp_on = (a.dbg & 8) && a.stamps && blockIdx.x == 100 && l == 0 && k == nsteps / 2;
#endif
        F3_STAMP(0);
        if (MSST_F3_RPRIO02 != MSST_F3_RPRIO) __builtin_amdgcn_s_setprio(MSST_F3_RPRIO02);
        if constexpr (STACK) {
            if (k >= 2 && epoch_differs(k - 1, k - 2)) {
                const int bk = blk_at(k - 1);
#pragma unroll
                for (int i6 = 0; i6 < 6; ++i6) {
                    const int f = rw * 6 + i6;
                    dma_frag_async(f < 12 ? mlp_w(bk, 0) + f * 1024 : mlp_w(bk, 1) + (f - 12) * 1024, sm.wmlp + f * 1024);
                }
            }
            lnp_switch = k + 1 < nsteps && epoch_differs(k + 1, k);
            if (lnp_switch && rt < 96) lnp_regs = fetch_lnp(blk_at(k + 1), rt);
        }
        if (have_prev) { request_xr(k - 1); outproj(1); F3_STAMP(1); epilogue1(k - 1); copy_lse(k - 1, 1); }
        F3_STAMP(2);
        if constexpr (STACK) {
            if (lnp_switch && rt < 96) commit_lnp(slot_at(k + 1), rt, lnp_regs);
            wait_vm0();
        }
        lds_barrier();
        F3_STAMP(3);
        if (MSST_F3_RPRIO02 != MSST_F3_RPRIO) __builtin_amdgcn_s_setprio(MSST_F3_RPRIO);
        if (have_prev) ln2(k - 1);
        if (rt < 64) fill_seq(k + 2, rt);
        if (have_cur) zero_acc();
        request_fw(0, have_cur ? k : k - 1);
        F3_STAMP(4);
        lds_barrier();
        F3_STAMP(5);
        if (MSST_F3_RPRIO02 != MSST_F3_RPRIO) __builtin_amdgcn_s_setprio(MSST_F3_RPRIO02);
        if (MSST_F3_LN1Q == 2 && k + 1 < nsteps) request_ln1(k + 1);
        if (have_cur) outproj(0);
        F3_STAMP(6);
        if (have_prev) { store_x1_bf16(k - 1); mlp1(k - 1); }
        if (have_cur) copy_lse(k, 0);
        if (MSST_F3_LN1Q == 2 && k + 1 < nsteps) ln1(k + 1);
        if (MSST_F3_LN1Q == 3 && k + 1 < nsteps) request_ln1(k + 1);
        F3_STAMP(7);
        lds_barrier();
        F3_STAMP(8);
        if (MSST_F3_RPRIO02 != MSST_F3_RPRIO) __builtin_amdgcn_s_setprio(MSST_F3_RPRIO);
        if (have_prev) mlp2(k - 1);
        F3_STAMP(9);
        if (MSST_F3_LN1Q == 3 && k + 1 < nsteps) ln1(k + 1);
        request_fw(1, have_cur ? k : k - 1);
        F3_STAMP(10);
        lds_barrier();
        F3_STAMP(11);
        if constexpr (STACK) words_advance();
    }
}

static int fwd3_attrs() {
    static std::atomic<bool> attr_set{false};
    if (attr_set) return 0;
    const void* ks[8] = {reinterpret_cast<const void*>(&block_fwd_rs_kernel<false, false, false>), reinterpret_cast<const void*>(&block_fwd_rs_kernel<true, false, false>),
                         reinterpret_cast<const void*>(&block_fwd_rs_kernel<false, true, false>), reinterpret_cast<const void*>(&block_fwd_rs_kernel<true, true, false>),
                         reinterpret_cast<const void*>(&block_fwd_rs_kernel<false, false, true>), reinterpret_cast<const void*>(&block_fwd_rs_kernel<true, false, true>),
                         reinterpret_cast<const void*>(&block_fwd_rs_kernel<false, true, true>), reinterpret_cast<const void*>(&block_fwd_rs_kernel<true, true, true>)};
    for (int i = 0; i < 8; ++i) {
        hipError_t e = hipFuncSetAttribute(ks[i], hipFuncAttributeMaxDynamicSharedMemorySize, (int)sizeof(Fwd3Smem));
        if (e != hipSuccess) return (int)e;
    }
    attr_set = true;
    return 0;
}

int block_fwd_stack_max_steps() { return F3_MAX_STEPS; }

int launch_block_fwd_rs_stack(const StackArgs& sa, int grid, hipStream_t st) {
    const BlockArgs& a = sa.base;
    if (a.H != 8 || sa.nblk < 1 || sa.nblk > MSST_MAX_STACK || grid < 1) return MSST_ERR_UNSUPPORTED;
    const int nmine = (a.ntiles + grid - 1) / grid;
    if (sa.nblk * (nmine < 3 ? 3 : nmine) > F3_MAX_STEPS) return MSST_ERR_UNSUPPORTED;
    int rc = fwd3_attrs();
    if (rc) return rc;
    ProfScope ps(K_BLOCK_FWD, st);
    const size_t smem = sizeof(Fwd3Smem);
    if (a.half) {
        if (a.drop.thr) hipLaunchKernelGGL((block_fwd_rs_kernel<true, true, true>), dim3(grid), dim3(512), smem, st, sa);
        else hipLaunchKernelGGL((block_fwd_rs_kernel<false, true, true>), dim3(grid), dim3(512), smem, st, sa);
    } else {
        if (a.drop.thr) hipLaunchKernelGGL((block_fwd_rs_kernel<true, true, false>), dim3(grid), dim3(512), smem, st, sa);
        else hipLaunchKernelGGL((block_fwd_rs_kernel<false, true, false>), dim3(grid), dim3(512), smem, st, sa);
    }
    return (int)hipGetLastError();
}

int launch_block_fwd_rs(const BlockArgs& a, int grid, hipStream_t st) {
    const size_t smem = sizeof(Fwd3Smem);
    if (a.H != 8) return MSST_ERR_UNSUPPORTED;
    int rc = fwd3_attrs();
    if (rc) return rc;
    ProfScope ps(K_BLOCK_FWD, st);
    if (a.half) {
        if (a.drop.thr) hipLaunchKernelGGL((block_fwd_rs_kernel<true, false, true>), dim3(grid), dim3(512), smem, st, a);
        else hipLaunchKernelGGL((block_fwd_rs_kernel<false, false, true>), dim3(grid), dim3(512), smem, st, a);
    } else {
        if (a.drop.thr) hipLaunchKernelGGL((block_fwd_rs_kernel<true, false, false>), dim3(grid), dim3(512), smem, st, a);
        else hipLaunchKernelGGL((block_fwd_rs_kernel<false, false, false>), dim3(grid), dim3(512), smem, st, a);
    }
    return (int)hipGetLastError();
}

}
```

maskedsst_amd/csrc/msst_kernels.h:

```cpp
#pragma once
#include <hip/hip_runtime.h>
#include <stdint.h>
#include "msst_dev.h"

#define MSST_PREC_F32 0
#define MSST_PREC_BF16 1
#define MSST_ERR_UNSUPPORTED (-2)
#define MSST_ERR_BADARG (-3)
#define MSST_ADAM_MAX_GROUPS 64
#define MSST_GRAD_MAX_RANGES 64

namespace msst {

struct BlockWeights {
    const void* wqkv;
    const void* wout;
    const void* w1;
    const void* w2;
    const void* wqkvT;
    const void* woutT;
    const void* w1T;
    const void* w2T;
    const float* ln1_g; const float* ln1_b; const float* bo;
    const float* ln2_g; const float* ln2_b; const float* b1; const float* b2;
    const void* wqkv32; const void* woutT32; const void* wqkvT32;
};

struct BlockArgs {
    BlockWeights w;
    const float* x;
    float* y;
    float* x1;
    int x1_bf16;
    int half;
    void* xn_out;
    float* lse_out;
    TileMap tm;
    int ntiles, max_grid, H;
    float scale;
    int dbg;
    unsigned long long* stamps;
    Drop drop;
};

#define MSST_MAX_STACK 16
struct StackBlk {
    const void* wqkv; const void* wout; const void* w1; const void* w2;
    const float* ln1_g; const float* ln1_b; const float* bo; const float* ln2_g; const float* ln2_b; const float* b1; const float* b2;
    const float* x; float* y; float* x1; void* xn_out; float* lse_out;
    int layer, pad_;
};
struct StackStride {
    int wqkv, wout, w1, w2, ln1_g, ln1_b, bo, ln2_g, ln2_b, b1, b2, x, y, x1, xn_out, lse_out;
};
struct StackArgs {
    BlockArgs base;
    int nblk;
    StackBlk b0;
    StackStride st;
    const float* x_rest;
};
static_assert(sizeof(StackArgs) <= 4096, "StackArgs travels as a kernel argument");

struct TokArgs {
    const float* img;
    const float* pre_g; const float* pre_b;
    const float* w_emb;
    const float* b_emb;
    const float* post_g; const float* post_b;
    const float* pos_a;
    const float* pos_b;
    const float* mask_token;
    const uint8_t* mask;
    float* out;
    int B, S, N, T, P, pos_split;
    Drop drop;
    long win0;
    int Hs, Ws, win, stride, nq, wps;
    const int32_t* origins;
    const uint8_t* orient;
};

template <class Args>
__device__ __forceinline__ const float* scene_window_origin(const Args& a, int b) {
    const long i = a.win0 + b;
    const long s = i / a.wps;
    const int rem = (int)(i - s * a.wps), r = rem / a.nq, q = rem - r * a.nq;
    return a.img + ((s * a.S * a.P) * a.Hs + (long)r * a.stride) * a.Ws + (long)q * a.stride;
}

template <class Args>
__device__ __forceinline__ const float* listed_window_origin(const Args& a, int b) {
    const int32_t* o = a.origins + 3 * (long)b;
    const long s = o[0];
    return a.img + ((s * a.S * a.P) * a.Hs + (long)o[1]) * a.Ws + (long)o[2];
}

struct WinSteps { int start, si, sj; };
__device__ __forceinline__ WinSteps window_steps(int o, int win, int Ws) {
    const int k = o & 3, m = win - 1;
    const int yi = (k == 0) - (k == 2), yj = (k == 1) - (k == 3), y0 = k >= 2 ? m : 0;
    int xi = (k == 3) - (k == 1), xj = (k == 0) - (k == 2), x0 = (k == 1 || k == 2) ? m : 0;
    if (o & 4) { x0 = m - x0; xi = -xi; xj = -xj; }
    return WinSteps{y0 * Ws + x0, yi * Ws + xi, yj * Ws + xj};
}
template <class Args>
__device__ __forceinline__ long oriented_pixel(const Args& a, int b, int n) {
    const WinSteps w = window_steps(a.orient[b], a.win, a.Ws);
    return (long)w.start + (long)(n / a.win) * w.si + (long)(n % a.win) * w.sj;
}

__device__ __forceinline__ const uint8_t* scene_window_mask(const TokArgs& a, int b, int c) {
    const long i = a.win0 + b;
    const long s = i / a.wps;
    const int rem = (int)(i - s * a.wps), r = rem / a.nq, q = rem - r * a.nq;
    return a.mask + (((s * a.S + c) * a.Hs) + (long)r * a.stride) * a.Ws + (long)q * a.stride;
}

template <class Args>
__device__ __forceinline__ bool scene_cover(const Args& a, int y, int x, int& rlo, int& rhi, int& qlo, int& qhi) {
    rlo = y < a.win ? 0 : (y - a.win) / a.stride + 1;
    rhi = min(y / a.stride, a.nr - 1);
    qlo = x < a.win ? 0 : (x - a.win) / a.stride + 1;
    qhi = min(x / a.stride, a.nq - 1);
    return rlo <= rhi && qlo <= qhi;
// ... 57 lines not shown
    long ntok;
    float scale;
    int dbg;
    unsigned long long* stamps;
    Drop drop;
    int* queue;
    const float* lse;
    int lse_renorm;
};

struct Ln1BwdArgs {
    const float* x; const float* dx1; const void* dxn_part; const float* ln1_g; float* dx; float* slab;
    long ntok;
    int H;
    Drop drop;
};

struct LnMlpArgs {
    BlockWeights w;
    const float* ln1_g;
    const float* ln1_b;
    const void* xn;
    const float* rstd;
    const float* x;
    float* dx1;
    const void* dxn_part;
    const float* x1;
    int x1_bf16;
    void* dab;
    float* slab_mlp;
    float* slab_ln1;
    long ntok;
    int nparts;
    Drop drop_i, drop_p;
    unsigned long long* stamps;
    int* queue;
};

struct TokBwdArgs {
    const float* img; const float* pre_g; const float* pre_b; const float* w_emb; const float* b_emb;
    const float* post_g; const float* post_b; const uint8_t* mask; const float* dx0; float* slab;
    int B, S, N, T, P;
    Drop drop;
};
struct TokSceneBwdArgs : TokBwdArgs {
    long win0;
    int Hs, Ws, win, stride, nq, wps;
};
struct TokAtBwdArgs : TokSceneBwdArgs {
    const int32_t* origins;
};
__device__ __forceinline__ const float* scene_window_origin(const TokAtBwdArgs& a, int b) { return listed_window_origin(a, b); }
struct TokAtOrBwdArgs : TokAtBwdArgs {
    const uint8_t* orient;
};
__device__ __forceinline__ const float* scene_window_origin(const TokAtOrBwdArgs& a, int b) { return listed_window_origin(a, b); }

struct TokInArgs {
    const float* img; const float* pre_g; const float* pre_b; const float* w_emb; const float* b_emb;
    const float* post_g; const float* post_b;
    const uint8_t* mask;
    const float* dx0;
    const float* dtarget;
    float* dimg;
    int B, S, N, T, P;
    Drop drop;
    long win0;
    int Hs, Ws, win, stride, nq, wps;
};
struct TokInAtArgs : TokInArgs {
    const int32_t* origins;
};
struct SceneFoldAtArgs {
    const float* dwin; const int32_t* cell_ptr; const int32_t* cell_win; float* dscene;
    int Bs, C, Hs, Ws, win, nwin, group, accumulate;
};
int launch_tokenize_bwd_input(const TokInArgs& a, hipStream_t st);
int launch_tokenize_scene_bwd_input(const TokInArgs& a, hipStream_t st);
int launch_tokenize_at_bwd_input(const TokInAtArgs& a, hipStream_t st);
int launch_scene_fold_at(const SceneFoldAtArgs& a, hipStream_t st);
int launch_scene_border_zero(float* dscene, long rows, int Hs, int Ws, int rows_in, int cols_in, hipStream_t st);
int launch_head_bwd_target(const float* dpred, const int* csr_ptr, const int* csr_pos, const float* gout, float gscale, float* dtarget,
                           int B, int S, int N, int P, int K, hipStream_t st);

enum KernelId {
    K_PREP = 0, K_TOK_FWD, K_BLOCK_FWD, K_HEAD_FWD, K_LOSS_REDUCE, K_HEAD_BWD, K_REDUCE, K_BWD_MLP, K_BWD_ATTN,
    K_ATTN_REDUCE, K_BWD_LN1, K_TOK_BWD, K_POS_SPLIT, K_ADAMW, K_BWD_LN1MLP, K_LAYERNORM, K_ADAM_GROUPS, K_CE, K_RECON, K_TOK_BWD_INPUT,
    K_HEAD_BWD_TARGET, K_GRAD_ACCUM, K_GRAD_FINAL, K_COUNT
};
void prof_begin(int id, hipStream_t st);
void prof_end(hipStream_t st);
struct ProfScope {
    hipStream_t st;
    ProfScope(int id, hipStream_t s) : st(s) { prof_begin(id, s); }
    ~ProfScope() { prof_end(st); }
};

struct ClsArgs {
    const float* y; const float* ln_g; const float* ln_b; const float* w; const float* b; float* logits;
    int B, S, N, T, NC;
};
struct ClsBwdArgs {
    const float* y; const float* dlogits; const float* ln_g; const float* ln_b; const float* w;
    float* dy; float* slab;
    int B, S, N, T, NC;
};
int launch_cls_head_fwd(const ClsArgs& a, hipStream_t st);
int launch_cls_head_bwd(const ClsBwdArgs& a, hipStream_t st);
struct SpecHeadArgs {
    const float* y; const float* ln_g; const float* ln_b; const float* w; const float* b; const float* dlogits;
    float* logits; float* dy; float* stats; float* slab;
    long slab_stride;
    int B, S, N, T, NC, R, G, RC;
};
void spec_head_chunks(long R, int& G, int& RC);
long spec_head_bwd_slab_floats(int B, int S, int N, int NC);
int launch_spec_head_fwd(const SpecHeadArgs& a, hipStream_t st);
int launch_spec_head_bwd_rows(const SpecHeadArgs& a, hipStream_t st);
int launch_spec_head_wgrad(const SpecHeadArgs& a, hipStream_t st);
int launch_spec_head_wgrad_finish(const SpecHeadArgs& a, const float* A, const float* db, float* dw, float* dg, float* dbeta,
                                  hipStream_t st);
struct PixHeadArgs {
    const float* y; const float* ln_g; const float* ln_b; const float* w; const float* b; const float* dlogits;
    float* logits; float* xn; float* dy; float* slab;
    int B, S, N, T, NC, G;
};
int pix_head_groups(int B);
long pix_head_bwd_slab_floats(int B, int N, int NC);
int launch_pix_head_fwd(const PixHeadArgs& a, hipStream_t st);
int launch_pix_head_bwd(const PixHeadArgs& a, hipStream_t st);
int launch_scene_centre_scatter(const SceneArgs& a, hipStream_t st);
int launch_scene_centre_fill(const SceneArgs& a, hipStream_t st);

int launch_tokenize_fwd(const TokArgs& a, hipStream_t st);
int launch_tokenize_scene_fwd(const TokArgs& a, hipStream_t st);
int launch_tokenize_scene_fwd_masked(const TokArgs& a, hipStream_t st);
int launch_tokenize_at_fwd(const TokArgs& a, hipStream_t st);
int launch_tokenize_at_fwd_orient(const TokArgs& a, bool masked, hipStream_t st);
int launch_tokenize_at_fwd_masked(const TokArgs& a, hipStream_t st);
int launch_head_bwd(const HeadBwdArgs& a, int nchunk, hipStream_t st);
struct RSeg {
    const float* src; float* dst;
    long slab_stride;
    int nslab, n, row_len, row_stride, blk0, vec4;
    int ny;
};
#define MSST_MAX_RSEG 72
struct RSegs { RSeg s[MSST_MAX_RSEG]; int nseg; int nblocks; int ny_max; long src_ystride, dst_ystride; };
struct RSegBuilder {
    RSegs r;
    RSegBuilder() { r.nseg = 0; r.nblocks = 0; r.ny_max = 1; r.src_ystride = 0; r.dst_ystride = 0; }
    bool add(const float* src, long slab_stride, int nslab, float* dst, int n, int row_len = 0, int row_stride = 0, int ny = 1) {
        if (r.nseg >= MSST_MAX_RSEG) return false;
        if (ny < 1) return true;
        RSeg& g = r.s[r.nseg++];
        g.ny = ny;
        if (ny > r.ny_max) r.ny_max = ny;
        g.src = src; g.dst = dst; g.slab_stride = slab_stride; g.nslab = nslab; g.n = n;
        g.row_len = row_len > 0 ? row_len : n; g.row_stride = row_stride > 0 ? row_stride : n;
        g.blk0 = r.nblocks;
        g.vec4 = (n % 4 == 0 && g.row_len % 4 == 0 && g.row_stride % 4 == 0 && slab_stride % 4 == 0 &&
                  ((uintptr_t)src % 16) == 0 && ((uintptr_t)dst % 16) == 0) ? 1 : 0;
        const int per_block = g.vec4 ? 128 : 32;
        r.nblocks += (n + per_block - 1) / per_block;
        return true;
    }
// ... 128 lines not shown
```

maskedsst_amd/engine.py:

```python
import collections
import ctypes
import os

import numpy as np
import torch

from . import _lib
from ._lib import (MsstBlockWeights, MsstBlockGrads, MsstPrepJob, PREC_BF16, PREC_F32, MODE_SPATIAL,
                   MODE_SPECTRAL, MLP_SLAB, ATTN_SLAB, LN1_SLAB)
from .flat import FlatParams

D = 96
DH = 64
STACK_MAX_TILES = 12
MLP = 64
_MODE = {"spatial": MODE_SPATIAL, "spectral": MODE_SPECTRAL}

_Head = collections.namedtuple("_Head", "fwd bwd linear shape fwd_ws bwd_slab assemble")
_HEADS = {
    "cls": _Head("msst_cls_head_fwd", "msst_cls_head_bwd", 1, lambda B, nc, N: (B, nc, N), None,
                 lambda lib, B, S, N, nc: B * (nc * 97 + 192), "msst_scene_assemble"),
    "spec": _Head("msst_spec_head_fwd", "msst_spec_head_bwd", 1, lambda B, nc, N: (B, nc, N), None,
                  lambda lib, B, S, N, nc: lib.msst_spec_head_bwd_slab(B, S, N, nc), "msst_scene_assemble"),
    "pix": _Head("msst_pix_head_fwd", "msst_pix_head_bwd", 2, lambda B, nc, N: (B, nc),
                 lambda lib, B, S, N, nc: lib.msst_pix_head_fwd_ws(B, N),
                 lambda lib, B, S, N, nc: lib.msst_pix_head_bwd_slab(B, S, N, nc), "msst_scene_centre_assemble"),
}


class Windows:

    def __init__(self, kind, img, origins=None, csr=None, sink=None, s=None, orient=None):
        self.kind, self.img, self.origins, self.csr, self.sink = kind, img.contiguous().float(), origins, csr, sink
        self.orient = orient
        if orient is not None and (kind != "listed" or csr is not None or sink is not None):
            raise NotImplementedError("orient goes with listed windows only, and without the scenes' gradient")
        if kind == "tiles":
            self.grid = (img.shape[-2] // s, img.shape[-1] // s)
            self.n = img.shape[0] * self.grid[0] * self.grid[1]
        else:
            self.n = origins.shape[0] if kind == "listed" else img.shape[0]


_TOK_FWD = {("batch", False): "msst_tokenize_fwd", ("batch", True): "msst_tokenize_fwd", ("tiles", False): "msst_tokenize_scene_fwd_train",
            ("listed", False): "msst_tokenize_at_fwd", ("listed", True): "msst_tokenize_at_fwd_masked"}
_TOK_BWD = {("batch", False): "msst_tokenize_bwd", ("batch", True): "msst_tokenize_bwd", ("tiles", False): "msst_tokenize_scene_bwd",
            ("listed", False): "msst_tokenize_at_bwd", ("listed", True): "msst_tokenize_at_bwd_masked"}
_TOK_INPUT_BWD = {("batch", False): "msst_tokenize_bwd_input", ("batch", True): "msst_tokenize_bwd_input",
                  ("tiles", False): "msst_tokenize_scene_bwd_input", ("listed", False): "msst_tokenize_at_bwd_input"}


def _tok_entry(table, method, src, masked, emb_drop=(0.0, 0)):
    name = table.get((src.kind, masked))
    if name is not None and src.orient is not None:
        name = name + "_orient" if table is not _TOK_INPUT_BWD else None
    if name is None:
        raise NotImplementedError(f"{method}: no entry point for {'oriented ' if src.orient is not None else ''}{src.kind} windows "
                                  f"{'with' if masked else 'without'} a token mask")
    if masked and src.kind == "listed":
        if emb_drop[0] > 0:
            raise NotImplementedError(f"{method}: no entry point for listed windows with a token mask and embedding dropout")
        return name, ()
    return name, tuple(emb_drop)


def _prec_of(name):
    name = (name or os.environ.get("MSST_PRECISION", "bf16")).lower()
    if name in ("fp32", "f32", "32-true", "float32"):
        return PREC_F32
    if name in ("bf16", "bf16-mixed", "bfloat16"):
        return PREC_BF16
    raise ValueError(f"unknown precision {name!r} (use 'bf16' or 'fp32')")


def _kernel_flags():
    v = int(os.environ.get("MSST_DBG", "0"))
    allowed = 16 | 64 | 128
    if v & 8:
        allowed |= 8 | 0x300
    return (v & allowed) << 8


def _stream():
    return ctypes.c_void_p(torch.cuda.current_stream().cuda_stream)


def _p(t):
    return ctypes.c_void_p(t.data_ptr()) if t is not None else ctypes.c_void_p(0)


def recon_fwd(y, img, mask_u8, w_pix, b_pix, per_block, blend, S, N, P, stats=True, lib=None):
    lib = lib or _lib.load()
    for t in (y, img, mask_u8):
        if not t.is_cuda:
            raise RuntimeError("maskedsst_amd runs on an MI355X only (tensor is on %s); there is no CPU fallback" % t.device)
    B = y.shape[0]
    if (y.dtype, img.dtype, mask_u8.dtype) != (torch.float32, torch.float32, torch.uint8):
        raise ValueError("recon_fwd takes fp32 y and img and a uint8 mask")
    if tuple(y.shape) != (B, S * N, D) or img.numel() != B * S * P * N or mask_u8.numel() != B * S * N:
        raise ValueError(f"recon_fwd: y {tuple(y.shape)}, img {tuple(img.shape)}, mask {tuple(mask_u8.shape)} do not fit "
                         f"B = {B}, S = {S}, N = {N}, P = {P}")
    y, img, mask_u8 = y.contiguous(), img.contiguous(), mask_u8.contiguous()
    tables = []
    for t, n in ((w_pix, P * D), (b_pix, P)):
        if torch.is_tensor(t):
            if not t.is_cuda or t.dtype != torch.float32 or t.numel() != (S if per_block else 1) * n:
                raise ValueError("recon_fwd: to_pixels tables must be fp32 cuda tensors [S or 1, P, 96] and [S or 1, P]")
            t = t.contiguous()
        tables.append(t)
    recon = torch.empty(B, S * P, N, dtype=torch.float32, device=y.device)
    err = torch.empty(B, S * P, dtype=torch.float64, device=y.device) if stats else None
    cnt = torch.empty(B, S * P, dtype=torch.int32, device=y.device) if stats else None
    wp, bp = (_p(t) if torch.is_tensor(t) else t for t in tables)
    _lib.check(lib.msst_recon_fwd(_p(y), _p(img), _p(mask_u8), wp, bp, int(bool(per_block)), int(bool(blend)), _p(recon), _p(err),
                                  _p(cnt), B, S, N, P, _stream()), "msst_recon_fwd")
    return recon, err, cnt


class Engine:
    def __init__(self, encoder, mim):
        self.enc = encoder
        self.mim = mim
        self.lib = _lib.load()
        self.fp = FlatParams(encoder, mim)
# ... 204 lines not shown
        return r is not None and r <= self.LN1_XN_MAX_RATIO

    def half_ok(self):
        b = getattr(self, "_half_bound", None)
        return b is not None and b <= self.HALF_MAX_BOUND

    def _pos_tables(self, buf=None):
        fp = self.fp
        if self.enc.spectral_pos_embed:
            return self.enc.pos_embed.shape[-1], fp.ptr("pos_embed", buf), fp.ptr("channel_embed", buf)
        return 0, fp.ptr("pos_embedding", buf), 0

    def _zero_mask_for(self, n, device):
        if self._zero_mask is None or self._zero_mask.numel() < n or self._zero_mask.device != torch.device(device):
            self._zero_mask = torch.zeros(n, dtype=torch.uint8, device=device)
        return self._zero_mask

    def _tok_params(self, grad=False):
        buf = self.fp.grad if grad else None
        return tuple(ctypes.c_void_p(self.fp.ptr(k, buf)) for k in ("pre_g", "pre_b", "embed.w.0", "embed.b.0", "post_g", "post_b"))

    def _tok_bwd_slab(self, nsamples, device):
        S, N, P = self.S, self.N, self.P
        nchunk = max(1, min(nsamples, self.tok_chunks))
        ss = N * 96 + 96 * P + 96 * 4 + 32
        return nchunk, torch.empty(S * nchunk * ss + S * N * 96, dtype=torch.float32, device=device)

    TILE_WINDOWS_PER_LAUNCH = 65535

    def _launch_chunk(self, src, emb_drop):
        total = src.n
        chunk = total if (self.P == 10 and self.enc.num_spatial_patches_sqrt == 8) else min(total, self.TILE_WINDOWS_PER_LAUNCH)
        if chunk < total and emb_drop[0] > 0:
            raise NotImplementedError(f"embedding dropout over {total} windows in one step needs more than one launch of the generic "
                                      f"tokenizer ({self.TILE_WINDOWS_PER_LAUNCH} windows each): "
                                      f"{'use fewer tiles' if src.kind == 'tiles' else 'list fewer windows'} per step")
        return chunk

    def _src(self, src):
        return src if isinstance(src, Windows) else Windows("batch", src)

    def _src_args(self, src, win0, n):
        S, P = self.S, self.P
        if src.kind == "batch":
            return (_p(src.img),), (n, S, self.N, P)
        Bs, _, Hs, Ws = src.img.shape
        s = self.enc.num_spatial_patches_sqrt
        if src.kind == "tiles":
            return (_p(src.img),), (Bs, Hs, Ws, s, s, win0, n, S, P)
        lead = (_p(src.img), _p(src.origins[win0:] if win0 else src.origins))
        if src.orient is not None:
            lead += (_p(src.orient[win0:] if win0 else src.orient),)
        return lead, (Bs, Hs, Ws, s, n, S, P)

    def tokenize(self, src, mask_u8=None, with_pos=True, emb_drop=(0.0, 0)):
        src = self._src(src)
        self._require_cuda(src.img)
        self.ensure()
        masked = mask_u8 is not None
        name, drop_args = _tok_entry(_TOK_FWD, "tokenize", src, masked, emb_drop)
        S, N, total = self.S, self.N, src.n
        T = S * N
        dev = src.img.device
        out = torch.empty(total, T, D, dtype=torch.float32, device=dev)
        fp, V = self.fp, ctypes.c_void_p
        if not with_pos:
            if getattr(self, "_zero_pos", None) is None or self._zero_pos.numel() < T * D:
                self._zero_pos = torch.zeros(T * D, dtype=torch.float32, device=dev)
            split, pos_a, pos_b = 0, self._zero_pos.data_ptr(), 0
        else:
            split, pos_a, pos_b = self._pos_tables()
        mask_args, chunk = (), total
        if src.kind == "batch" or masked:
            mask_args = (V(fp.ptr("mask_token") if self.mim is not None else fp.ptr("post_b")),
                         _p(mask_u8 if masked else self._zero_mask_for(total * T, dev)))
        else:
            chunk = self._launch_chunk(src, emb_drop)
        fn, par, st = getattr(self.lib, name), self._tok_params(), _stream()
        for win0 in (range(0, total, chunk) if chunk < total else (0,)):
            lead, dims = self._src_args(src, win0, min(chunk, total - win0))
            _lib.check(fn(*lead, *par, V(pos_a), V(pos_b), split, *mask_args, _p(out[win0:] if win0 else out), *dims, *drop_args, st), name)
        return out

    def blocks_fwd(self, x0, save=True, drop=(0.0, 0)):
        acts = [x0]
        x1s = []
        flags = _kernel_flags()
        role_split = self._role_split(flags)
        x1_bf16 = save and role_split and os.environ.get("MSST_X1_BF16", "1") != "0"
        want_lse = save and role_split and os.environ.get("MSST_LSE", "1") != "0"
        layers = self._layers()
        want_stack = os.environ.get("MSST_FWD_STACK", "auto")
        stacked = role_split and want_stack != "0"
        i0 = 0
        self.fwd_launch_blocks = []
        while i0 < len(layers):
            i1 = i0
            while i1 < len(layers) and layers[i1][0] == layers[i0][0] and i1 - i0 < 16:
                i1 += 1
            use = stacked and (want_stack == "1" or self._tiles_per_workgroup(layers[i0][0], x0.shape[0]) <= STACK_MAX_TILES)
            if use and self._fwd_stack(acts, x1s, i0, i1, save, drop, x1_bf16, want_lse):
                self.fwd_launch_blocks.append(i1 - i0)
            else:
                for i in range(i0, i1):
                    self._fwd_block(acts, x1s, i, save, drop, x1_bf16, want_lse, flags)
                self.fwd_launch_blocks += [1] * (i1 - i0)
            i0 = i1
        return acts, x1s

    def blocks_fwd_pingpong(self, x0, drop=(0.0, 0), other=None, n=None, stream=None):
        B = x0.shape[0] if n is None else n
        S, N, H = self.S, self.N, self.enc.heads
        flags = _kernel_flags()
        prec = self.prec | flags | self._half_flag(flags)
        x, y = x0, torch.empty_like(x0) if other is None else other
        wrote = ctypes.c_int(0)
        st = _stream() if stream is None else stream
        for i, (sname, _) in enumerate(self._layers()):
            _lib.check(self.lib.msst_block_fwd(ctypes.byref(self._bw[i]), _p(x), _p(y), None, _MODE[sname], B, S, N, H, prec, self.max_grid,
                                               drop[0], drop[1], i, None, None, ctypes.byref(wrote), st), "msst_block_fwd")
            x, y = y, x
        return x

    def _tiles_per_workgroup(self, sname, B):
        mode = _MODE[sname]
        key = (mode, B)
        hit = self._tpw.get(key)
        if hit is None:
            tiles = int(self.lib.msst_block_tiles(mode, B, self.S, self.N))
            grid = max(1, min(tiles, self._cu_count(), self.max_grid if self.max_grid > 0 else tiles))
            hit = self._tpw[key] = -(-tiles // grid)
        return hit

    def _role_split(self, flags):
        return self.prec == PREC_BF16 and self.enc.heads == 8 and flags == 0

    def _half_flag(self, flags):
        self.fwd_half = self._role_split(flags) and os.environ.get("MSST_FWD_HALF", "1") != "0" and self.half_ok()
        return _lib.FWD_HALF if self.fwd_half else 0

    def _attach_saved(self, x1, wrote, xn, lse):
        x1._msst_xn = xn if (wrote & _lib.SAVED_XN) else None
        x1._msst_lse = lse if (lse is not None and (wrote & _lib.SAVED_LSE)) else None
        x1._msst_rstd = bool(wrote & _lib.SAVED_RSTD) and x1._msst_lse is not None
        x1._msst_half = bool(self.fwd_half)

    def _fwd_block(self, acts, x1s, i, save, drop, x1_bf16, want_lse, flags):
        x = acts[-1]
        B = x.shape[0]
        S, N, H = self.S, self.N, self.enc.heads
        sname, l = self._layers()[i]
        y = torch.empty_like(x)
        x1 = (torch.empty(x.shape, dtype=torch.bfloat16, device=x.device) if x1_bf16 else torch.empty_like(x)) if save else None
        xn = torch.empty(x.shape, dtype=torch.bfloat16, device=x.device) if (save and self.prec != PREC_F32) else None
        mode = _MODE[sname]
        lse = None
        if xn is not None and want_lse:
            lse = torch.empty(int(self.lib.msst_block_lse_floats(mode, B, S, N, H)), dtype=torch.float32, device=x.device)
        wrote = ctypes.c_int(0)
        _lib.check(self.lib.msst_block_fwd(ctypes.byref(self._bw[i]), _p(x), _p(y), _p(x1), mode, B, S, N, H,
                                           self.prec | flags | (_lib.X1_BF16 if x1_bf16 else 0) | self._half_flag(flags), self.max_grid, drop[0], drop[1], i, _p(xn), _p(lse),
                                           ctypes.byref(wrote), _stream()),
                   "msst_block_fwd")
        if x1 is not None:
            self._attach_saved(x1, wrote.value, xn, lse)
        acts.append(y)
        x1s.append(x1)

    def _fwd_stack(self, acts, x1s, i0, i1, save, drop, x1_bf16, want_lse):
        x0 = acts[-1]
        B = x0.shape[0]
        S, N, H = self.S, self.N, self.enc.heads
        dev = x0.device
        n = i1 - i0
        mode = _MODE[self._layers()[i0][0]]
        def slices(dtype, shape=None):
            t = torch.empty((n,) + tuple(shape if shape is not None else x0.shape), dtype=dtype, device=dev)
            return [t[j] for j in range(n)]
        ys = slices(x0.dtype)
        x1 = slices(torch.bfloat16 if x1_bf16 else torch.float32) if save else None
        xn = slices(torch.bfloat16) if save else None
        lse = slices(torch.float32, (int(self.lib.msst_block_lse_floats(mode, B, S, N, H)),)) if (save and want_lse) else None
        wv = (ctypes.POINTER(MsstBlockWeights) * n)(*[ctypes.pointer(self._bw[i0 + j]) for j in range(n)])
        VP = ctypes.c_void_p * n

        def arr(ts):
            return VP(*[t.data_ptr() for t in ts]) if ts is not None else None
        wrote = ctypes.c_int(0)
        rc = self.lib.msst_block_fwd_stack(wv, n, _p(x0), arr(ys), arr(x1), arr(xn), arr(lse), mode, B, S, N, H,
                                           self.prec | (_lib.X1_BF16 if x1_bf16 else 0) | self._half_flag(0), self.max_grid, drop[0], drop[1], i0,
                                           ctypes.byref(wrote), _stream())
        if rc == -2:
            return False
        _lib.check(rc, "msst_block_fwd_stack")
        for j in range(n):
            acts.append(ys[j])
            if save:
                self._attach_saved(x1[j], wrote.value, xn[j], lse[j] if lse is not None else None)
                x1s.append(x1[j])
            else:
                x1s.append(None)
        return True

    def head_fwd(self, y, src, idx32, want_pred=False):
        src = self._src(src)
        if src.kind == "tiles":
            raise NotImplementedError("head_fwd: no entry point for tiles windows")
        B, T, _ = y.shape
        K = idx32.shape[1]
        dev = y.device
        dpred = torch.empty(B, K, self.P, dtype=torch.float32, device=dev)
        pred = torch.empty(B, K, self.P, dtype=torch.float32, device=dev) if want_pred else None
        partial = torch.empty(B * ((K + 63) // 64), dtype=torch.float32, device=dev)
        loss = torch.empty((), dtype=torch.float32, device=dev)
        per_block = 1 if hasattr(self.mim.to_pixels, "layers") else 0
        V = ctypes.c_void_p
        name = "msst_head_fwd" if src.kind != "listed" else "msst_head_at_fwd" if src.orient is None else "msst_head_at_fwd_orient"
        lead, dims = self._src_args(src, 0, B)
        _lib.check(getattr(self.lib, name)(
            _p(y), *lead, _p(idx32), V(self.fp.ptr("to_pixels.w.0")), V(self.fp.ptr("to_pixels.b.0")), per_block,
            _p(dpred), _p(pred), _p(partial), _p(loss), *dims, K, _stream()), name)
        return loss, dpred, pred

    def recon_fwd(self, y, img, mask_u8, blend=True, stats=True):
        per_block = 1 if hasattr(self.mim.to_pixels, "layers") else 0
        V = ctypes.c_void_p
        return recon_fwd(y, img, mask_u8, V(self.fp.ptr("to_pixels.w.0")), V(self.fp.ptr("to_pixels.b.0")), per_block, blend,
                         self.S, self.N, self.P, stats=stats, lib=self.lib)

    def reconstruct(self, img, mask_u8, blend=True):
        self._require_cuda(img)
        if self.mim is None:
            raise RuntimeError("reconstruct needs the SimMIM wrapper's mask token and to_pixels (a bare encoder has neither)")
        img = img.contiguous().float()
        with torch.no_grad():
            self.prep_weights()
            x0 = self.tokenize(img, mask_u8)
            acts, _ = self.blocks_fwd(x0, save=False)
            return self.recon_fwd(acts[-1], img, mask_u8, blend)

    def tokenize_scene_masked(self, scene, scene_mask_u8, stride, win0, nwin, out=None):
        self._require_cuda(scene)
        self._require_cuda(scene_mask_u8)
        if self.mim is None:
            raise RuntimeError("tokenize_scene_masked needs the SimMIM wrapper's mask token (a bare encoder has none)")
        self.ensure()
        Bs, _, Hs, Ws = scene.shape
        S, N, P = self.S, self.N, self.P
# ... 3 lines not shown
            raise ValueError(f"tokenize_scene_masked takes a contiguous fp32 scene and a contiguous uint8 mask [{Bs}, {S}, {Hs}, {Ws}]")
        if out is None:
            out = torch.empty(nwin, S * N, D, dtype=torch.float32, device=scene.device)
        fp = self.fp
        split, pos_a, pos_b = self._pos_tables()
        V = ctypes.c_void_p
        _lib.check(self.lib.msst_tokenize_scene_fwd_masked(
            _p(scene), *self._tok_params(), V(pos_a), V(pos_b), split, V(fp.ptr("mask_token")), _p(scene_mask_u8), _p(out),
            Bs, Hs, Ws, w, stride, win0, nwin, S, P, _stream()), "msst_tokenize_scene_fwd_masked")
        return out

    def reconstruct_scene(self, scene, scene_mask_u8, stride, blend=True, max_windows=2048):
        self._require_cuda(scene)
        self._require_cuda(scene_mask_u8)
        if self.mim is None:
            raise RuntimeError("reconstruct_scene needs the SimMIM wrapper's mask token and to_pixels (a bare encoder has neither)")
        with torch.no_grad():
            scene = scene.contiguous().float()
            scene_mask_u8 = scene_mask_u8.contiguous()
            Bs, C, Hs, Ws = scene.shape
            S, N, P = self.S, self.N, self.P
            w = self.enc.num_spatial_patches_sqrt
            total, chunk = self._scene_chunking(scene, stride, max_windows)
            dev = scene.device
            no_img = torch.zeros(chunk, S * P, N, dtype=torch.float32, device=dev)
            no_mask = self._zero_mask_for(chunk * S * N, dev)
            win_recon = torch.empty(chunk, S * P, N, dtype=torch.float32, device=dev)
            cube = torch.empty(Bs, C, Hs, Ws, dtype=torch.float32, device=dev)
            err = torch.empty(Bs, C, dtype=torch.float64, device=dev)
            cnt = torch.empty(Bs, C, dtype=torch.int32, device=dev)
            cover = torch.empty(Bs, Hs, Ws, dtype=torch.int32, device=dev)
            per_block = 1 if hasattr(self.mim.to_pixels, "layers") else 0
            V = ctypes.c_void_p
            st = _stream()
            for win0, n, y in self._scene_encoder_chunks(scene, stride, total, chunk, st, scene_mask_u8):
                _lib.check(self.lib.msst_recon_fwd(_p(y), _p(no_img), _p(no_mask), V(self.fp.ptr("to_pixels.w.0")),
                                                   V(self.fp.ptr("to_pixels.b.0")), per_block, 0, _p(win_recon), None, None, n, S, N, P, st),
                           "msst_recon_fwd")
                _lib.check(self.lib.msst_scene_recon_assemble(_p(win_recon), win0, n, _p(scene), _p(scene_mask_u8), _p(cube), _p(err),
                                                              _p(cnt), _p(cover), Bs, S, P, Hs, Ws, w, stride, int(win0 + n == total),
                                                              int(bool(blend)), st), "msst_scene_recon_assemble")
            return cube, err, cnt, cover

    def _fire(self, bucket):
        if self.bucket_hook is not None:
            for name, start, end in self.fp.buckets:
                if name == bucket:
                    self.bucket_hook(name, start, end)

    def head_bwd(self, y, dpred, csr_ptr, csr_pos, gout=None):
        B, T, _ = y.shape
        S, N, P = self.S, self.N, self.P
        K = dpred.shape[1]
        dev = y.device
        nchunk = max(1, min(B, int(os.environ.get("MSST_HEAD_CHUNKS", "0")) or 512 // max(S, 1)))
        dy = torch.empty_like(y)
        slab = torch.empty(S * nchunk * (P * 96 + P), dtype=torch.float32, device=dev)
        per_block = 1 if hasattr(self.mim.to_pixels, "layers") else 0
        gscale = 1.0 / (B * K * P) / K
        V = ctypes.c_void_p
        g = self.fp.grad
        _lib.check(self.lib.msst_head_bwd(
            _p(y), _p(dpred), _p(csr_ptr), _p(csr_pos), V(self.fp.ptr("to_pixels.w.0")), per_block, gscale, _p(gout),
            _p(dy), _p(slab), nchunk, V(self.fp.ptr("to_pixels.w.0", g)), V(self.fp.ptr("to_pixels.b.0", g)),
            B, S, N, P, K, _stream()), "msst_head_bwd")
        self._fire("head")
        return dy

    def _grad_stride(self, nlayers):
        blocks = [f"{sname}.{l}" for sname, l in self._layers()[:nlayers]]
        d = self.fp.block_stride(blocks, [n for n, _ in MsstBlockGrads._fields_])
        return -d if d is not None and d < 0 and d % 4 == 0 else None

    def _bwd_workspace(self, B, device):
        H = self.enc.heads
        ntok = B * self.S * self.N
        esz = 4 if self.prec == PREC_F32 else 2
        dx1 = torch.empty(ntok * 96, dtype=torch.float32, device=device)
        part = torch.empty(H * ntok * 96 * esz, dtype=torch.uint8, device=device)
        slab = torch.empty(self.grid_rows * (3 * MLP_SLAB + LN1_SLAB) + self.attn_chunks * H * ATTN_SLAB, dtype=torch.float32, device=device)
        dab = torch.empty(ntok * 96, dtype=torch.bfloat16, device=device) if self.prec != PREC_F32 else None
        return dx1, part, slab, dab

    def blocks_bwd(self, acts, x1s, dy, drop=(0.0, 0)):
        H = self.enc.heads
        ntok = dy.shape[0] * self.S * self.N
        ws = self._bwd_workspace(dy.shape[0], dy.device)
        x1_bf16 = len(x1s) > 0 and all(t.dtype == torch.bfloat16 for t in x1s)
        if not x1_bf16 and any(t.dtype != torch.float32 for t in x1s):
            raise ValueError("saved x1 rows of mixed dtypes")
        nparts = H // 2 if H % 2 == 0 else H
        chain = (self.prec == PREC_BF16 and _kernel_flags() == 0 and all(getattr(t, "_msst_xn", None) is not None for t in x1s)
                 and nparts <= 4 and os.environ.get("MSST_BWD_CHAIN", "1") != "0" and self.enc.depth > 0
                 and ntok * 384 < 2 ** 31 - 16 and nparts * ntok * 192 < 2 ** 31 - 16)
        ln1_from_xn = (chain and x1_bf16 and os.environ.get("MSST_LN1_XN", "1") != "0"
                       and all(getattr(t, "_msst_rstd", False) for t in x1s) and self.ln1_xn_ok())
        self.last_bwd_ln1_from_xn = bool(ln1_from_xn)
        if chain:
            return self._blocks_bwd_chained(acts, x1s, dy, drop, ws,
                                            (_lib.X1_BF16 if x1_bf16 else 0) | (_lib.LN1_FROM_XN if ln1_from_xn else 0))
        return self._blocks_bwd_unchained(acts, x1s, dy, drop, ws)

    def _blocks_bwd_chained(self, acts, x1s, dy, drop, ws, x1flags):
        B = dy.shape[0]
        S, N, H = self.S, self.N, self.enc.heads
        dev = dy.device
        dx1, part, slab, dab = ws
        layers = self._layers()
        queue = None
        if self.tile_queue or os.environ.get("MSST_TILE_QUEUE", "0") == "1":
            if getattr(self, "_queue_ws", None) is None or self._queue_ws.device != dev:
                self._queue_ws = torch.zeros(64, dtype=torch.int32, device=dev)
            queue = self._queue_ws
        last = len(layers) - 1
        dx0 = torch.empty_like(dy)
        null_w = ctypes.POINTER(MsstBlockWeights)()
        null_g = ctypes.POINTER(MsstBlockGrads)()
        gstride = self._grad_stride(len(layers))
        defer = gstride is not None and os.environ.get("MSST_BWD_DEFER", "0") == "1"
        nslab_r = (slab.numel() + 3) // 4 * 4
        if defer:
            slab = torch.empty(nslab_r * len(layers), dtype=torch.float32, device=dev)
        run_start = last
        for i in reversed(range(len(layers))):
            sname, l = layers[i]
            prev = i > 0
            x1 = x1s[i]
            slab_i = slab[(last - i) * nslab_r:] if defer else slab
            _lib.check(self.lib.msst_block_bwd_chain(
                ctypes.byref(self._bw[i]), ctypes.byref(self._bg[i]),
                ctypes.byref(self._bw[i - 1]) if prev else null_w, ctypes.byref(self._bg[i - 1]) if prev else null_g,
                _p(acts[i]), _p(x1), _p(x1s[i - 1]) if prev else _p(None), _p(dy) if i == last else _p(None),
                _p(None) if prev else _p(dx0), _p(dx1), _p(part), _p(slab_i), self.grid_rows, self.attn_chunks, _MODE[sname],
                B, S, N, H, self.prec | x1flags | (_lib.LSE_RENORM if getattr(x1, "_msst_half", False) else 0) |
                (_lib.BWD_DEFER_REDUCE if defer else 0), drop[0], drop[1], i, _p(x1._msst_xn), _p(getattr(x1, "_msst_lse", None)), _p(dab),
                1 if i == last else 0, _p(queue), _stream()),
                "msst_block_bwd_chain")
            if not defer:
                self._fire(f"{sname}.{l}")
            elif i == 0 or layers[i - 1][0] != sname:
                count = run_start - i + 1
                _lib.check(self.lib.msst_block_bwd_reduce(
                    ctypes.byref(self._bg[run_start]), ctypes.byref(self._bg[run_start - 1]) if run_start > 0 else null_g,
                    _p(slab[(last - run_start) * nslab_r:]), nslab_r, gstride, count, count if i > 0 else count - 1,
                    1 if run_start == last else 0, self.grid_rows, self.attn_chunks, _MODE[sname], B, S, N, H, self.prec, _stream()),
                    "msst_block_bwd_reduce")
                for j in range(run_start, i - 1, -1):
                    self._fire(f"{layers[j][0]}.{layers[j][1]}")
                run_start = i - 1
        return dx0

    def _blocks_bwd_unchained(self, acts, x1s, dy, drop, ws):
        layers = self._layers()
        g, other = dy, torch.empty_like(dy)
        for i in reversed(range(len(layers))):
            self.block_bwd_single(i, acts[i], x1s[i], g, other, drop=drop, ws=ws)
            g, other = other, g
            self._fire(f"{layers[i][0]}.{layers[i][1]}")
        return g

    def block_bwd_single(self, i, x, x1, dy, dx=None, drop=(0.0, 0), ws=None):
        dx1, part, slab, dab = ws if ws is not None else self._bwd_workspace(dy.shape[0], dy.device)
        if dx is None:
            dx = torch.empty_like(dy)
        if x1.dtype not in (torch.float32, torch.bfloat16):
            raise ValueError("saved x1 rows must be fp32 or bf16")
        x1flag = _lib.X1_BF16 if x1.dtype == torch.bfloat16 else 0
        _lib.check(self.lib.msst_block_bwd(
            ctypes.byref(self._bw[i]), ctypes.byref(self._bg[i]), _p(x), _p(x1), _p(dy), _p(dx),
            _p(dx1), _p(part), _p(slab), self.grid_rows, self.attn_chunks, _MODE[self._layers()[i][0]], dy.shape[0], self.S, self.N, self.enc.heads,
            self.prec | _kernel_flags() | x1flag | (_lib.LSE_RENORM if getattr(x1, "_msst_half", False) else 0),
            drop[0], drop[1], i, _p(getattr(x1, "_msst_xn", None)), _p(getattr(x1, "_msst_lse", None)), _p(dab), _stream()), "msst_block_bwd")
        return dx

    def tokenize_bwd(self, src, mask_u8, dx0, emb_drop=(0.0, 0), with_pos=True):
        src = self._src(src)
        masked = mask_u8 is not None
        name, drop_args = _tok_entry(_TOK_BWD, "tokenize_bwd", src, masked, emb_drop)
        total, dev = src.n, src.img.device
        nchunk, slab = self._tok_bwd_slab(total, dev)
        g, V = self.fp.grad, ctypes.c_void_p
        split, dpa, dpb = self._pos_tables(g) if with_pos else (0, 0, 0)
        mask_args = dmt_args = ()
        if src.kind == "batch" or masked:
# ... 20 lines not shown
            mask_args = (_p(mask_u8),) if src.kind == "batch" else ()
            target_args = (_p(dtarget),) if src.kind == "batch" else ()
            _lib.check(fn(*lead, *par, *mask_args, _p(dx0), *target_args, _p(dimg), *dims, *drop_args, st), name)
            return dimg
        if src.csr is None:
            raise NotImplementedError("no input gradient through windows at listed origins unless the forward opted in "
                                      "(forward_at(..., scene_grad=True)): they overlap, so d(scene) is an accumulating fold")
        sink = src.sink
        if sink is None:
            out = torch.empty(img.shape, dtype=torch.float32, device=img.device)
        else:
            out = sink.out
            if tuple(out.shape) != tuple(img.shape) or out.dtype != torch.float32 or not out.is_contiguous() or out.device != img.device:
                raise ValueError(f"out must be a contiguous fp32 tensor {tuple(img.shape)} on the scene's device")
        Bs, C, Hs, Ws = img.shape
        dwin = torch.empty(src.n, C, self.N, dtype=torch.float32, device=img.device)
        _lib.check(fn(*lead, *par, _p(dx0), _p(dwin), *dims, *drop_args, st), name)
        _lib.check(self.lib.msst_scene_fold_at(_p(dwin), _p(src.csr[0]), _p(src.csr[1]), _p(out), Bs, C, Hs, Ws, self.enc.num_spatial_patches_sqrt, src.n, self.P,
                                               int(bool(sink and sink.started)), st), "msst_scene_fold_at")
        if sink:
            sink.started = True
        return out

    def head_bwd_target(self, dpred, csr_ptr, csr_pos, gout=None):
        B, K, P = dpred.shape
        dtarget = torch.empty(B, self.S * P, self.N, dtype=torch.float32, device=dpred.device)
        _lib.check(self.lib.msst_head_bwd_target(_p(dpred), _p(csr_ptr), _p(csr_pos), _p(gout), _p(dtarget), B, self.S, self.N, P, K,
                                                 _stream()), "msst_head_bwd_target")
        return dtarget

    def trainable(self):
        if self.fp.flat is None or getattr(self, "_trainable_key", None) != self.fp.version:
            groups, _ = self.fp._ordered()
            self._trainable = [(n, p) for _, g in groups for n, p in g]
            self._trainable_key = self.fp.version if self.fp.flat is not None else None
        return self._trainable

    def dropout_state(self):
        p = float(self.enc.dropout_p) if self.enc.training else 0.0
        if p <= 0.0:
            return 0.0, 0
        if not 0.0 < p < 1.0:
            raise ValueError(f"dropout probability {p} outside (0, 1)")
        seed = int(torch.randint(0, 2 ** 31 - 1, (1,)).item())
        rank = int(getattr(self.mim, "dp_rank", 0)) if self.mim is not None else 0
        if rank:
            seed = (seed ^ (rank * 0x9E3779B1)) & 0x7FFFFFFF
        return p, seed

    def _upload(self, dev, *arrays):
        if getattr(self, "_up", None) is None:
            self._up = {"sets": [None, None], "k": 0}
        up = self._up
        k = up["k"]
        up["k"] = 1 - k
        cur = up["sets"][k]
        sig = tuple((a.shape, a.dtype) for a in arrays)
        if cur is None or cur["sig"] != sig:
            cur = {"sig": sig,
                   "pin": [torch.empty(a.shape, dtype=torch.from_numpy(a).dtype, pin_memory=True) for a in arrays],
                   "ev": torch.cuda.Event()}
            up["sets"][k] = cur
        else:
            cur["ev"].synchronize()
        out = []
        for pin, a in zip(cur["pin"], arrays):
            pin.numpy()[...] = a
            d = torch.empty(pin.shape, dtype=pin.dtype, device=dev)
            d.copy_(pin, non_blocking=True)
            out.append(d)
        cur["ev"].record(torch.cuda.current_stream(dev))
        return out

    def simmim_loss(self, src, bool_mask, idx):
        src = self._src(src)
        img = src.img
        self._require_cuda(img)
        self.ensure()
        T = self.S * self.N
        from .masking import inverse_csr
        bm = bool_mask.cpu().numpy() if torch.is_tensor(bool_mask) else np.asarray(bool_mask)
        ix = idx.cpu().numpy() if torch.is_tensor(idx) else np.asarray(idx)
        ptr, pos = inverse_csr(ix, T)
        mask_u8, idx32, csr_ptr, csr_pos = self._upload(img.device, bm.astype(np.uint8), ix.astype(np.int32), ptr, pos)
        names = [n for n, _ in self.trainable()]
        params = [p for _, p in self.trainable()]
        want_img = src.kind == "batch" and img.requires_grad
        if not torch.is_grad_enabled() or not (want_img or any(p.requires_grad for p in params)):
            self.prep_weights()
            x0 = self.tokenize(src, mask_u8)
            acts, _ = self.blocks_fwd(x0, save=False, drop=self.dropout_state())
            loss, _, _ = self.head_fwd(acts[-1], src, idx32)
            return loss
        return _SimMIMLossFn.apply(self, names, self.dropout_state(), src, img, mask_u8, idx32, csr_ptr, csr_pos, *params)

    def _block_param_names(self):
        return [n for n, _ in self.trainable() if n.startswith(("spatial.", "spectral."))]

    def _embed_param_names(self):
        return [n for n, _ in self.trainable() if n.startswith(("embed.", "pre_", "post_"))]

    def transformer(self, tokens):
        self._require_cuda(tokens)
        self.ensure()
        drop = self.dropout_state()
        tokens = tokens.contiguous().float()
        by_name = dict(self.trainable())
        names = self._block_param_names()
        params = [by_name[n] for n in names]
        if torch.is_grad_enabled() and (tokens.requires_grad or any(p.requires_grad for p in params)):
            return _TransformerFn.apply(self, names, drop, tokens, *params)
        self.prep_weights()
        acts, _ = self.blocks_fwd(tokens, save=False, drop=drop)
        return acts[-1]

    def embed_patches(self, patches):
        self._require_cuda(patches)
        self.ensure()
        B, S, N, P = patches.shape
        want_input = torch.is_grad_enabled() and patches.requires_grad
        img = (patches if want_input else patches.detach()).permute(0, 1, 3, 2).reshape(B, S * P, N).contiguous().float()
        by_name = dict(self.trainable())
        names = self._embed_param_names()
        params = [by_name[n] for n in names]
        if torch.is_grad_enabled() and (want_input or any(p.requires_grad for p in params)):
            return _EmbedFn.apply(self, names, img, *params)
        return self.tokenize(img, None, with_pos=False)

    def features(self, img):
        enc = self.enc
        params = [q for _, q in self.trainable()]
        if torch.is_grad_enabled() and (img.requires_grad or any(q.requires_grad for q in params)):
            self._require_cuda(img)
            patches = enc.to_patch_embedding.to_patch(img.contiguous().float())
            tokens = self.embed_patches(patches).reshape(img.shape[0], -1, D)
            pos = enc.get_pos_embeddings() if enc.spectral_pos_embed else enc.pos_embedding[:, :tokens.shape[1]]
            tokens = tokens + pos
            if enc.training and float(enc.emb_dropout_p) > 0:
                tokens = torch.nn.functional.dropout(tokens, p=float(enc.emb_dropout_p), training=True)
            return self.transformer(tokens)
        pe = float(enc.emb_dropout_p) if enc.training else 0.0
        emb_drop = (pe, int(torch.randint(0, 2 ** 31 - 1, (1,)).item())) if pe > 0 else (0.0, 0)
        x0 = self.tokenize(img, None, with_pos=True, emb_drop=emb_drop)
        with torch.no_grad():
            return self.transformer(x0)

    def _head_kind(self):
        return "pix" if self.enc.pixelwise else "spec" if self.enc.spectral_mlp_head else "cls"

    def _head_params(self, head, buf=None):
        return [ctypes.c_void_p(self.fp.ptr(f"mlp_head.{i}.{wb}", buf)) for i in (0, head.linear) for wb in ("weight", "bias")]

    def _head_fwd(self, kind, y, B=None, logits=None, stream=None):
        head = _HEADS[kind]
        B = y.shape[0] if B is None else B
        nc = self.enc.num_classes
        if logits is None:
            logits = torch.empty(head.shape(B, nc, self.N), dtype=torch.float32, device=y.device)
        ws = None if head.fwd_ws is None else torch.empty(int(head.fwd_ws(self.lib, B, self.S, self.N, nc)), dtype=torch.float32, device=y.device)
        _lib.check(getattr(self.lib, head.fwd)(
            _p(y), *self._head_params(head), _p(logits), *([] if ws is None else [_p(ws)]), B, self.S, self.N, nc,
            _stream() if stream is None else stream), head.fwd)
        return logits

    def _head_bwd(self, kind, y, dlogits, dy=None, want_dy=True):
        head = _HEADS[kind]
        B = y.shape[0]
        nc = self.enc.num_classes
        if dy is None and want_dy:
            dy = torch.empty_like(y)
        slab = torch.empty(int(head.bwd_slab(self.lib, B, self.S, self.N, nc)), dtype=torch.float32, device=y.device)
        g = self._head_params(head, self.fp.grad)
        _lib.check(getattr(self.lib, head.bwd)(
            _p(y), _p(dlogits), *self._head_params(head)[:3], _p(dy), _p(slab), *g, B, self.S, self.N, nc, _stream()), head.bwd)
        self._fire("cls_head")
        return dy

# ... 140 lines not shown
            win_feat = torch.empty(chunk, D, N, dtype=torch.float32, device=dev)
            feat = torch.empty(Bs, D, Hs, Ws, dtype=torch.float32, device=dev)
            cover = torch.empty(Bs, Hs, Ws, dtype=torch.int32, device=dev)
            st = _stream()
            for win0, n, y in self._scene_encoder_chunks(scene, stride, total, chunk, st):
                _lib.check(self.lib.msst_pool_spectral_fwd(_p(y), _p(win_feat), n, S, N, st), "msst_pool_spectral_fwd")
                _lib.check(self.lib.msst_scene_embed_assemble(_p(win_feat), win0, n, _p(feat), _p(cover), Bs, D, Hs, Ws, w, stride,
                                                              int(win0 + n == total), int(bool(normalize)), st),
                           "msst_scene_embed_assemble")
            return feat, cover

    def attn_maps_block(self, i, x, out, reduce):
        self.ensure()
        sname, l = self._layers()[i]
        B = x.shape[0]
        V = ctypes.c_void_p
        fp = self.fp
        _lib.check(self.lib.msst_attn_maps(_p(x), V(fp.ptr(f"{sname}.{l}.ln1_g")), V(fp.ptr(f"{sname}.{l}.ln1_b")),
                                           V(fp.ptr(f"{sname}.{l}.wqkv")), _p(out), out.stride(0) if B > 1 else out[0].numel(),
                                           _MODE[sname], B, self.S, self.N, self.enc.heads, reduce, _stream()), "msst_attn_maps")
        return out

    def _maps_storage(self, B, nblk, tail, device):
        per = int(np.prod(tail))
        pad = (per + 3) // 4 * 4
        flat = torch.empty(B * nblk * pad, dtype=torch.float32, device=device)
        strides, s = [], 1
        for d in reversed(tail):
            strides.insert(0, s)
            s *= d
        return torch.as_strided(flat, (B, nblk) + tuple(tail), (nblk * pad, pad) + tuple(strides))

    def attention_maps_tokens(self, x0, stacks, blocks, reduce):
        B = x0.shape[0]
        S, N, H = self.S, self.N, self.enc.heads
        out = {}
        for sname in stacks:
            L, G = (N, S) if sname == "spatial" else (S, N)
            tail = (H, L, L) if reduce == _lib.ATTN_MEAN_SEQ else (G, H, L, L)
            out[sname] = self._maps_storage(B, len(blocks), tail, x0.device)
        flags = _kernel_flags()
        prec = self.prec | flags | self._half_flag(flags)
        x, y = x0, torch.empty_like(x0)
        wrote = ctypes.c_int(0)
        st = _stream()
        layers = self._layers()
        last = max((i for i, (sname, l) in enumerate(layers) if sname in out and l in blocks), default=-1)
        for i, (sname, l) in enumerate(layers):
            if i > last:
                break
            _lib.check(self.lib.msst_block_fwd(ctypes.byref(self._bw[i]), _p(x), _p(y), None, _MODE[sname], B, S, N, H, prec, self.max_grid,
                                               0.0, 0, i, None, None, ctypes.byref(wrote), st), "msst_block_fwd")
            if sname in out and l in blocks:
                self.attn_maps_block(i, x, out[sname][:, blocks.index(l)], reduce)
            x, y = y, x
        return out.get("spatial"), out.get("spectral")

    def attention_maps(self, img, mask_u8, stacks, blocks, reduce):
        self._require_cuda(img)
        with torch.no_grad():
            self.prep_weights()
            x0 = self.tokenize(img.contiguous().float(), mask_u8)
            return self.attention_maps_tokens(x0, tuple(stacks), list(blocks), reduce)

    def simmim_forward_stages(self, img, bool_mask, idx, drop=(0.0, 0)):
        self._require_cuda(img)
        self.prep_weights()
        dev = img.device
        img = img.contiguous().float()
        mask_u8 = bool_mask.to(device=dev, dtype=torch.uint8).contiguous()
        idx32 = idx.to(device=dev, dtype=torch.int32).contiguous()
        tok_embed = self.tokenize(img, None, with_pos=False)
        x0 = self.tokenize(img, mask_u8)
        acts, x1s = self.blocks_fwd(x0, drop=drop)
        loss, dpred, pred = self.head_fwd(acts[-1], img, idx32, want_pred=True)
        L = self.enc.depth
        return dict(loss=loss, tok_embed=tok_embed, tok_masked=x0, after_spatial=acts[L], enc_out=acts[-1],
                    pred=pred, dpred=dpred, acts=acts, x1s=x1s)


class _SimMIMLossFn(torch.autograd.Function):

    @staticmethod
    def forward(ctx, eng, names, drop, src, img, mask_u8, idx32, csr_ptr, csr_pos, *params):
        eng.prep_weights()
        x0 = eng.tokenize(src, mask_u8)
        acts, x1s = eng.blocks_fwd(x0, save=True, drop=drop)
        ctx.drop = drop
        loss, dpred, _ = eng.head_fwd(acts[-1], src, idx32)
        ctx.eng = eng
        ctx.names = names
        ctx.stash = (src, mask_u8, csr_ptr, csr_pos, acts, x1s, dpred)
        return loss

    @staticmethod
    def backward(ctx, gout):
        eng = ctx.eng
        src, mask_u8, csr_ptr, csr_pos, acts, x1s, dpred = ctx.stash
        ctx.stash = None
        needs = ctx.needs_input_grad[9:]
        _refuse_accumulation(eng, ctx.names, needs)
        gout = gout.contiguous().float()
        dy = eng.head_bwd(acts[-1], dpred, csr_ptr, csr_pos, gout)
        dx0 = eng.blocks_bwd(acts, x1s, dy, drop=ctx.drop)
        dimg = None
        if ctx.needs_input_grad[4] and src.kind == "batch":
            dimg = eng.tokenize_input_bwd(src, mask_u8, dx0, eng.head_bwd_target(dpred, csr_ptr, csr_pos, gout))
        if any(needs):
            eng.tokenize_bwd(src, mask_u8, dx0)
        return (None,) * 4 + (dimg,) + (None,) * 4 + _grad_views(eng, ctx.names, needs)


def _refuse_accumulation(eng, names, needs=None):
    by_name = dict(eng.trainable())
    lo, hi = eng.fp.grad.data_ptr(), eng.fp.grad.data_ptr() + 4 * eng.fp.grad.numel()
    for i, n in enumerate(names):
        if needs is not None and not needs[i]:
            continue
        p = by_name[n]
        if p.grad is not None and lo <= p.grad.data_ptr() < hi:
            raise RuntimeError(
                "maskedsst_amd hands autograd views of its flat gradient buffer: drop the previous gradients "
                "with optimizer.zero_grad(set_to_none=True) (the torch default) before the next backward; "
                "in-place gradient accumulation across backward calls is not supported")


def _grad_views(eng, names, needs=None):
    return tuple(eng.fp.view(n, eng.fp.grad) if needs is None or needs[i] else None for i, n in enumerate(names))


class _TransformerFn(torch.autograd.Function):

    @staticmethod
    def forward(ctx, eng, names, drop, tokens, *params):
        eng.prep_weights()
        acts, x1s = eng.blocks_fwd(tokens, save=True, drop=drop)
        ctx.eng, ctx.names, ctx.drop = eng, names, drop
        ctx.stash = (acts[:-1], x1s)
        return acts[-1]

    @staticmethod
    def backward(ctx, dy):
        eng = ctx.eng
        acts, x1s = ctx.stash
        ctx.stash = None
        needs = ctx.needs_input_grad[4:]
        _refuse_accumulation(eng, ctx.names, needs)
        dx0 = eng.blocks_bwd(acts, x1s, dy.contiguous().float().clone(), drop=ctx.drop)
        return (None, None, None, dx0) + _grad_views(eng, ctx.names, needs)


class _EmbedFn(torch.autograd.Function):

    @staticmethod
    def forward(ctx, eng, names, img, *params):
        ctx.eng, ctx.names = eng, names
        ctx.stash = (img,)
        return eng.tokenize(img, None, with_pos=False)

    @staticmethod
    def backward(ctx, dtok):
        eng = ctx.eng
        (img,) = ctx.stash
        ctx.stash = None
        needs = ctx.needs_input_grad[3:]
        _refuse_accumulation(eng, ctx.names, needs)
        dtok = dtok.contiguous().float()
        dimg = eng.tokenize_input_bwd(img, None, dtok) if ctx.needs_input_grad[2] else None
        if any(needs):
            eng.tokenize_bwd(img, None, dtok, with_pos=False)
        return (None, None, dimg) + _grad_views(eng, ctx.names, needs)


class SceneGradSink:

    def __init__(self, out):
        self.out, self.started = out, False


class _ClassifyFn(torch.autograd.Function):

    @staticmethod
    def forward(ctx, eng, names, drop, emb_drop, src, img, *params):
        eng.prep_weights()
        x0 = eng.tokenize(src, None, emb_drop=emb_drop)
        acts, x1s = eng.blocks_fwd(x0, save=True, drop=drop)
        logits = eng.head_logits(acts[-1])
        ctx.eng, ctx.names, ctx.drop, ctx.emb_drop = eng, names, drop, emb_drop
        ctx.stash = (src, acts, x1s)
        return logits

    @staticmethod
    def backward(ctx, dlogits):
# ... 35 lines not shown
```

maskedsst_amd/masking.py:

```python
import numpy as np
import torch


class MaskGenerator:

    def __init__(self, input_size=16, mask_patch_size=4, model_patch_size=1, mask_ratio=0.6):
        self.input_size = input_size
        self.mask_patch_size = mask_patch_size
        self.model_patch_size = model_patch_size
        self.mask_ratio = mask_ratio
        assert self.input_size % self.mask_patch_size == 0
        assert self.mask_patch_size % self.model_patch_size == 0
        self.rand_size = self.input_size // self.mask_patch_size
        self.scale = self.mask_patch_size // self.model_patch_size
        self.token_count = self.rand_size ** 2
        self.mask_count = int(np.ceil(self.token_count * self.mask_ratio))

    def __call__(self):
        return self._draw(1)[0].astype(int)

    def _draw(self, n):
        sel = np.empty((n, self.mask_count), dtype=np.int64)
        for i in range(n):
            sel[i] = np.random.permutation(self.token_count)[: self.mask_count]
        coarse = np.zeros((n, self.token_count), dtype=bool)
        coarse[np.arange(n)[:, None], sel] = True
        coarse = coarse.reshape(n, self.rand_size, self.rand_size)
        return coarse.repeat(self.scale, axis=1).repeat(self.scale, axis=2)

    @staticmethod
    def _indices(flat, batch, num_masked):
        cols = np.nonzero(flat)[1]
        if cols.shape[0] < batch * num_masked:
            raise RuntimeError(
                f"shape mismatch: {cols.shape[0]} masked entries for {batch} x {num_masked} indices")
        return cols[: batch * num_masked].reshape(batch, num_masked).astype(np.int64)

    def bool_mask_to_indices(self, masked_bool_mask, batch, num_masked, device=None):
        m = masked_bool_mask.cpu().numpy() if torch.is_tensor(masked_bool_mask) else np.asarray(masked_bool_mask)
        return torch.from_numpy(self._indices(m, batch, num_masked))

    def get_batch(self, batch_size, channel_tokens, num_masked, device=None):
        m = self._draw(batch_size * channel_tokens).reshape(batch_size, -1)
        return torch.from_numpy(m), torch.from_numpy(self._indices(m, batch_size, num_masked))

    def get_batch_tube_masked(self, batch_size, channel_tokens, num_masked, device=None, rows=None):
        n = batch_size
        sel = np.empty((n, self.mask_count), dtype=np.int64)
        for i in range(n):
            sel[i] = np.random.permutation(self.token_count)[: self.mask_count]
        lo, hi = (0, n) if rows is None else rows
        hw = self.input_size // self.model_patch_size
        HW = hw * hw
        cell = np.arange(self.token_count)
        cy, cx = cell // self.rand_size, cell % self.rand_size
        dy, dx = np.meshgrid(np.arange(self.scale), np.arange(self.scale), indexing="ij")
        table = ((cy[:, None, None] * self.scale + dy) * hw + (cx[:, None, None] * self.scale + dx)).reshape(self.token_count, -1)
        per = table.shape[1] * self.mask_count
        R = per * channel_tokens
        if n * R < n * num_masked:
            raise RuntimeError(f"shape mismatch: {n * R} masked entries for {n} x {num_masked} indices")
        r0, r1 = (num_masked * lo) // R, -(-(num_masked * hi) // R)
        need = np.arange(min(r0, lo), max(r1, hi))
        pos = np.sort(table[sel[need]].reshape(need.shape[0], per), axis=1)
        base = need[0]
        cols = (np.arange(channel_tokens)[None, :, None] * HW + pos[r0 - base:r1 - base, None, :]).reshape(-1)
        idx = cols[num_masked * lo - R * r0: num_masked * hi - R * r0].reshape(hi - lo, num_masked).astype(np.int64)
        m = np.zeros((hi - lo, HW), dtype=bool)
        m[np.arange(hi - lo)[:, None], pos[lo - base:hi - base]] = True
        m = np.tile(m, (1, channel_tokens))
        return torch.from_numpy(m), torch.from_numpy(idx)


def topk_masks(batch, num_patches, num_masked):
    idx = torch.rand(batch, num_patches).topk(k=num_masked, dim=-1).indices
    bm = torch.zeros((batch, num_patches)).scatter_(-1, idx, 1).bool()
    return bm, idx


def micro_masks(masks, k, steps):
    bm, idx = masks
    B = bm.shape[0]
    if steps < 1 or B % steps or idx.shape[0] != B:
        raise ValueError(f"{B} mask rows ({idx.shape[0]} index rows) do not split into {steps} equal micro-batches")
    if not 0 <= k < steps:
        raise ValueError(f"micro-batch {k} outside 0 .. {steps - 1}")
    m = B // steps
    return bm[k * m:(k + 1) * m], idx[k * m:(k + 1) * m]


def inverse_csr(idx, num_tokens):
    idx = np.asarray(idx)
    B, K = idx.shape
    key = idx.astype(np.uint16) if num_tokens < 65536 else idx
    pos = np.argsort(key, axis=1, kind="stable").astype(np.int32)
    flat = (np.arange(B, dtype=np.int64)[:, None] * (num_tokens + 1) + idx + 1).ravel()
    cnt = np.bincount(flat, minlength=B * (num_tokens + 1)).reshape(B, num_tokens + 1)
    ptr = np.cumsum(cnt, axis=1).astype(np.int32)
    return ptr, pos
```

Measured before the change: 11290 samples/s.

## Skip last spectral block forward tiles that no masked token reads

Adds a listed variant of the role-split bf16 block forward that walks only the spectral tiles containing at least one masked (loss-contributing) token. The host computes the list from the mask indices. Unlisted rows of the outputs and saved activations are zeroed before the backward so the chained backward sees consistent buffers. This is meant to cut forward work for tiles whose outputs cannot reach the SimMIM loss. It adds a host-side split, an extra zeroing kernel and a tile-list upload, and it only helps when whole tiles lack masked tokens.

```diff
diff --git a/include/msst.h b/include/msst.h
--- a/include/msst.h
+++ b/include/msst.h
@@ -160,6 +160,19 @@
                    int B, int S, int N, int heads, int prec, int max_grid, float dropout_p, uint32_t seed,
                    int layer, void* xn_out, float* lse_out, int* saved , void* stream);
 
+int msst_block_fwd_listed(const MsstBlockWeights* w , const float* x, float* y, float* x1, int mode,
+                          int B, int S, int N, int heads, int prec, int max_grid, float dropout_p, uint32_t seed,
+                          int layer, void* xn_out, float* lse_out, int* saved ,
+                          const int32_t* tile_list , int n_listed, void* stream);
+
+typedef struct MsstRowBuf {
+    void* base;
+    int32_t row_bytes;
+    int32_t per_tile;
+} MsstRowBuf;
+int msst_zero_unlisted_rows(const int32_t* unlisted , int n_unlisted, const MsstRowBuf* bufs , int nbuf,
+                            int mode, int B, int S, int N, void* stream);
+
 int msst_block_fwd_stack(const MsstBlockWeights* const* w , int nblk, const float* x0, float* const* y ,
                          float* const* x1 , void* const* xn_out , float* const* lse_out , int mode,
                          int B, int S, int N, int heads, int prec, int max_grid, float dropout_p, uint32_t seed, int layer0,
diff --git a/maskedsst_amd/_lib.py b/maskedsst_amd/_lib.py
--- a/maskedsst_amd/_lib.py
+++ b/maskedsst_amd/_lib.py
@@ -42,6 +42,10 @@
 
 class MsstGradRange(Structure):
     _fields_ = [("start", c_long), ("end", c_long)]
+
+
+class MsstRowBuf(Structure):
+    _fields_ = [("base", c_void_p), ("row_bytes", c_int32), ("per_tile", c_int32)]
 
 
 _P = c_void_p
@@ -103,6 +107,9 @@
     "msst_block_tiles": (c_long, [c_int, c_int, c_int, c_int]),
     "msst_block_fwd": (c_int, [POINTER(MsstBlockWeights), _P, _P, _P, c_int, c_int, c_int, c_int, c_int,
                                c_int, c_int, c_float, c_uint32, c_int, _P, _P, POINTER(c_int), _P]),
+    "msst_block_fwd_listed": (c_int, [POINTER(MsstBlockWeights), _P, _P, _P, c_int, c_int, c_int, c_int, c_int,
+                                      c_int, c_int, c_float, c_uint32, c_int, _P, _P, POINTER(c_int), _P, c_int, _P]),
+    "msst_zero_unlisted_rows": (c_int, [_P, c_int, POINTER(MsstRowBuf), c_int, c_int, c_int, c_int, c_int, _P]),
     "msst_block_fwd_stack": (c_int, [_P, c_int, _P, _P, _P, _P, _P, c_int, c_int, c_int, c_int, c_int, c_int, c_int, c_float, c_uint32, c_int,
                                      POINTER(c_int), _P]),
     "msst_head_fwd": (c_int, [_P, _P, _P, _P, _P, c_int, _P, _P, _P, _P, c_int, c_int, c_int, c_int,
diff --git a/maskedsst_amd/build.py b/maskedsst_amd/build.py
--- a/maskedsst_amd/build.py
+++ b/maskedsst_amd/build.py
@@ -6,7 +6,7 @@
 HERE = os.path.dirname(os.path.abspath(__file__))
 CSRC = os.path.join(HERE, "csrc")
 LIB = os.path.join(HERE, "libmsst.so")
-SOURCES = ["msst_fwd.hip", "msst_fwd3.hip", "msst_bwd.hip", "msst_bwd3.hip", "msst_bwd4.hip", "msst_bwd5.hip", "msst_ln.hip", "msst_opt.hip", "msst_accum.hip", "msst_head.hip", "msst_pixhead.hip", "msst_loss.hip", "msst_recon.hip", "msst_scene_recon.hip", "msst_scene_embed.hip", "msst_input_grad.hip", "msst_attn_maps.hip", "msst_api.hip"]
+SOURCES = ["msst_fwd.hip", "msst_fwd3.hip", "msst_bwd.hip", "msst_bwd3.hip", "msst_bwd4.hip", "msst_bwd5.hip", "msst_ln.hip", "msst_opt.hip", "msst_accum.hip", "msst_head.hip", "msst_pixhead.hip", "msst_loss.hip", "msst_recon.hip", "msst_scene_recon.hip", "msst_scene_embed.hip", "msst_input_grad.hip", "msst_attn_maps.hip", "msst_zero_rows.hip", "msst_api.hip"]
 HEADERS = ["msst_dev.h", "msst_kernels.h", os.path.join("..", "..", "include", "msst.h")]
 FLAGS = ["--offload-arch=gfx950", "-O3", "-std=c++17", "-fPIC", "-fno-gpu-rdc", "-Wno-unused-result"]
 
diff --git a/maskedsst_amd/csrc/msst_api.hip b/maskedsst_amd/csrc/msst_api.hip
--- a/maskedsst_amd/csrc/msst_api.hip
+++ b/maskedsst_amd/csrc/msst_api.hip
@@ -540,9 +540,9 @@
     return (long)ntiles_of(make_tilemap(mode, B, S, N));
 }
 
-int msst_block_fwd(const MsstBlockWeights* w, const float* x, float* y, float* x1, int mode, int B, int S,
-                   int N, int heads, int prec, int max_grid, float dropout_p, uint32_t seed, int layer,
-                   void* xn_out, float* lse_out, int* saved, void* stream) {
+static int block_fwd_call(const MsstBlockWeights* w, const float* x, float* y, float* x1, int mode, int B, int S,
+                          int N, int heads, int prec, int max_grid, float dropout_p, uint32_t seed, int layer,
+                          void* xn_out, float* lse_out, int* saved, const int32_t* tile_list, int n_listed, void* stream) {
     if (int rc = block_shape(mode, B, S, N, heads)) return fail(rc, "msst_block_fwd (B, S, N, heads < 1, mode not 0 / 1, or sequence length > 64)");
     if (!bw_ok(w) || !x || !y || x == y) return fail(MSST_ERR_BADARG, "msst_block_fwd (null argument, or MsstBlockWeights of another header revision)");
     const int dbg = (prec >> 8) & 0xffff;
@@ -576,8 +576,54 @@
     a.drop = make_drop(dropout_p, seed, layer);
     a.xn_out = (xn_out && block_fwd_writes_xn(a, prec)) ? xn_out : nullptr;
     a.lse_out = (lse_out && block_fwd_writes_lse(a, prec)) ? lse_out : nullptr;
+    if (tile_list) {
+        if (n_listed < 1 || n_listed > a.ntiles) return fail(MSST_ERR_BADARG, "msst_block_fwd_listed (1 <= n_listed <= tiles)");
+        if (!(prec == MSST_PREC_BF16 && heads == 8 && !(dbg & (16 | 64))))
+            return fail(MSST_ERR_UNSUPPORTED, "msst_block_fwd_listed (a tile list needs the role-split bf16 forward: 8 heads, no MSST_KERNEL_* flags)");
+        a.tile_list = tile_list; a.nlisted = n_listed;
+    }
     if (saved) *saved = (a.xn_out ? MSST_SAVED_XN : 0) | (a.lse_out ? (MSST_SAVED_LSE | MSST_SAVED_RSTD) : 0);
-    return fail(launch_block_fwd(a, prec, (hipStream_t)stream), "msst_block_fwd");
+    return fail(launch_block_fwd(a, prec, (hipStream_t)stream), tile_list ? "msst_block_fwd_listed" : "msst_block_fwd");
+}
+
+int msst_block_fwd(const MsstBlockWeights* w, const float* x, float* y, float* x1, int mode, int B, int S,
+                   int N, int heads, int prec, int max_grid, float dropout_p, uint32_t seed, int layer,
+                   void* xn_out, float* lse_out, int* saved, void* stream) {
+    return block_fwd_call(w, x, y, x1, mode, B, S, N, heads, prec, max_grid, dropout_p, seed, layer, xn_out, lse_out, saved, nullptr, 0, stream);
+}
+
+int msst_block_fwd_listed(const MsstBlockWeights* w, const float* x, float* y, float* x1, int mode, int B, int S,
+                          int N, int heads, int prec, int max_grid, float dropout_p, uint32_t seed, int layer,
+                          void* xn_out, float* lse_out, int* saved, const int32_t* tile_list, int n_listed, void* stream) {
+    return block_fwd_call(w, x, y, x1, mode, B, S, N, heads, prec, max_grid, dropout_p, seed, layer, xn_out, lse_out, saved, tile_list, n_listed, stream);
+}
+
+int msst_zero_unlisted_rows(const int32_t* unlisted, int n_unlisted, const MsstRowBuf* bufs, int nbuf, int mode, int B, int S, int N,
+                            void* stream) {
+    if (int rc = block_shape(mode, B, S, N, 1)) return fail(rc, "msst_zero_unlisted_rows (B, S, N < 1, mode not 0 / 1, or sequence length > 64)");
+    if (n_unlisted < 0 || nbuf < 0) return fail(MSST_ERR_BADARG, "msst_zero_unlisted_rows");
+    if (n_unlisted == 0 || nbuf == 0) return 0;
+    if (!unlisted || !bufs) return fail(MSST_ERR_BADARG, "msst_zero_unlisted_rows (null argument)");
+    ZeroRowsArgs a;
+    a.unlisted = unlisted;
+    a.tm = make_tilemap(mode, B, S, N);
+    a.ntiles = ntiles_of(a.tm);
+    a.ntok = (long)B * S * N;
+    if (n_unlisted > a.ntiles) return fail(MSST_ERR_BADARG, "msst_zero_unlisted_rows (more unlisted tiles than tiles)");
+    for (int j = 0; j < nbuf; ++j)
+        if (!bufs[j].base || bufs[j].row_bytes < 4 || (bufs[j].row_bytes & 3) || ((uintptr_t)bufs[j].base & 3) || (bufs[j].per_tile & ~1))
+            return fail(MSST_ERR_BADARG, "msst_zero_unlisted_rows (a buffer: null or unaligned base, row_bytes not a positive multiple of 4, per_tile not 0 / 1)");
+    for (int j0 = 0; j0 < nbuf; j0 += MSST_ZERO_MAX_BUFS) {
+        const int n = nbuf - j0 < MSST_ZERO_MAX_BUFS ? nbuf - j0 : MSST_ZERO_MAX_BUFS;
+        for (int j = 0; j < n; ++j) {
+            const MsstRowBuf& b = bufs[j0 + j];
+            ZeroRowsBuf& z = a.buf[j];
+            z.base = reinterpret_cast<char*>(b.base); z.row_bytes = b.row_bytes; z.per_tile = (short)b.per_tile;
+            z.wide = (short)((((uintptr_t)b.base & 15) == 0 && (b.row_bytes & 15) == 0) ? 1 : 0);
+        }
+        if (int rc = launch_zero_unlisted_rows(a, n_unlisted, n, (hipStream_t)stream)) return fail(rc, "msst_zero_unlisted_rows");
+    }
+    return 0;
 }
 
 int msst_block_fwd_stack(const MsstBlockWeights* const* w, int nblk, const float* x0, float* const* y, float* const* x1,
diff --git a/maskedsst_amd/csrc/msst_fwd.hip b/maskedsst_amd/csrc/msst_fwd.hip
--- a/maskedsst_amd/csrc/msst_fwd.hip
+++ b/maskedsst_amd/csrc/msst_fwd.hip
@@ -871,6 +871,7 @@
 int launch_block_fwd(const BlockArgs& a, int prec, hipStream_t st) {
     if (a.tm.L > 64 || a.tm.L < 1) return MSST_ERR_UNSUPPORTED;
     if (a.ntiles < 1) return 0;
+    if (a.tile_list && !(prec == MSST_PREC_BF16 && a.H == 8 && !(a.dbg & (16 | 64)))) return MSST_ERR_UNSUPPORTED;
     if (prec == MSST_PREC_F32 || (a.dbg & 16)) {
         const int grid = a.ntiles < a.max_grid ? a.ntiles : a.max_grid;
         return prec == MSST_PREC_F32 ? launch_block_fwd_t<PF32>(a, grid, st) : launch_block_fwd_t<PBF16>(a, grid, st);
@@ -884,7 +885,8 @@
             if (hipDeviceGetAttribute(&ncu, hipDeviceAttributeMultiprocessorCount, dev) != hipSuccess || ncu < 1) ncu = 256;
             ncu_cached.store(ncu, std::memory_order_relaxed);
         }
-        int grid = a.max_grid < a.ntiles ? a.max_grid : a.ntiles;
+        const int nwalk = a.tile_list ? a.nlisted : a.ntiles;
+        int grid = a.max_grid < nwalk ? a.max_grid : nwalk;
         if (grid > ncu) grid = ncu;
         return launch_block_fwd_rs(a, grid, st);
     }
diff --git a/maskedsst_amd/csrc/msst_fwd3.hip b/maskedsst_amd/csrc/msst_fwd3.hip
--- a/maskedsst_amd/csrc/msst_fwd3.hip
+++ b/maskedsst_amd/csrc/msst_fwd3.hip
@@ -143,7 +143,7 @@
 
 }
 
-template <bool DROP, bool STACK, bool HALF>
+template <bool DROP, bool STACK, bool HALF, bool LIST = false>
 __global__ __launch_bounds__(512, 2) void block_fwd_rs_kernel(typename std::conditional<STACK, StackArgs, BlockArgs>::type args) {
     const BlockArgs& a = [&]() -> const BlockArgs& { if constexpr (STACK) return args.base; else return args; }();
     typedef Fwd3Smem SM;
@@ -156,7 +156,9 @@
     const TileMap tm = a.tm;
     const int L = tm.L;
     const int G = (int)gridDim.x;
-    const int nmine = ((int)blockIdx.x < a.ntiles) ? (a.ntiles - 1 - (int)blockIdx.x) / G + 1 : 0;
+    static_assert(!(STACK && LIST), "the stack walk takes no tile list");
+    const int nwalk = LIST ? a.nlisted : a.ntiles;
+    const int nmine = ((int)blockIdx.x < nwalk) ? (nwalk - 1 - (int)blockIdx.x) / G + 1 : 0;
     int nsteps = nmine;
     if constexpr (STACK) {
         const int nblk = args.nblk;
@@ -173,6 +175,9 @@
             sm.steptab[s_] = (unsigned)(before + min(pos, sz - 1)) | ((unsigned)blk << 16) | ((unsigned)((j * nblk + blk) & 1) << 24) | (idle << 31);
         }
     }
+    if constexpr (LIST) {
+        for (int s_ = tid; s_ < nmine; s_ += 512) sm.steptab[s_] = (unsigned)a.tile_list[(int)blockIdx.x + s_ * G];
+    }
     if constexpr (STACK) {
         static_assert(offsetof(StackBlk, lse_out) == 15 * 8 && offsetof(StackStride, lse_out) == 15 * 4, "blktab follows StackBlk's member order");
         for (int e = tid; e < args.nblk * 16; e += 512) {
@@ -188,18 +193,20 @@
     constexpr unsigned F3_IDLE = 0x80000000u;
     auto load_word = [&](int k) -> unsigned {
         if constexpr (STACK) return (k >= 0 && k < nsteps) ? (unsigned)__builtin_amdgcn_readfirstlane((int)sm.steptab[k]) : F3_IDLE;
+        else if constexpr (LIST) return (k >= 0 && k < nmine) ? (unsigned)__builtin_amdgcn_readfirstlane((int)sm.steptab[k]) : F3_IDLE;
         else return (k >= 0 && k < nmine) ? (unsigned)k : F3_IDLE;
     };
     int kc = 0;
     unsigned swm2 = F3_IDLE, swm1 = F3_IDLE, sw0 = F3_IDLE, swp1 = F3_IDLE, swp2 = F3_IDLE;
     auto step_word = [&](int k) -> unsigned {
-        if constexpr (!STACK) return load_word(k);
+        if constexpr (!STACK && !LIST) return load_word(k);
         else { const int d = k - kc; return d == 0 ? sw0 : d == 1 ? swp1 : d == -1 ? swm1 : d == 2 ? swp2 : d == -2 ? swm2 : load_word(k); }
     };
     auto words_init = [&]() { kc = 0; swm2 = F3_IDLE; swm1 = F3_IDLE; sw0 = load_word(0); swp1 = load_word(1); swp2 = load_word(2); };
     auto words_advance = [&]() { swm2 = swm1; swm1 = sw0; sw0 = swp1; swp1 = swp2; swp2 = load_word(kc + 3); };
     auto tile_at = [&](int k) -> int {
         const unsigned w_ = step_word(k);
+        if constexpr (LIST) return w_ < (unsigned)a.ntiles ? (int)w_ : -1;
         return (w_ >> 31) ? -1 : (int)blockIdx.x + (int)(w_ & 0xffffu) * G;
     };
     auto blk_at = [&](int k) -> int { if constexpr (STACK) return (int)((step_word(k) >> 16) & 0xffu); else return 0; };
@@ -255,7 +262,7 @@
         else return reinterpret_cast<const char*>(which ? a.w.w2 : a.w.w1);
     };
 
-    if (STACK) __syncthreads();
+    if (STACK || LIST) __syncthreads();
     words_init();
     if (tid < 96) load_lnp(slot_at(0), blk_at(0), tid);
 #pragma unroll
@@ -512,7 +519,7 @@
                     attn_pair(I1{}, std::true_type{}, std::integral_constant<int, 0xf>{}, std::integral_constant<int, 0xf>{});
                 }
             }
-            if constexpr (STACK) words_advance();
+            if constexpr (STACK || LIST) words_advance();
         }
 #pragma unroll
         for (int i = 0; i < 4; ++i) lds_barrier();
@@ -843,18 +850,20 @@
         F3_STAMP(10);
         lds_barrier();
         F3_STAMP(11);
-        if constexpr (STACK) words_advance();
+        if constexpr (STACK || LIST) words_advance();
     }
 }
 
 static int fwd3_attrs() {
     static std::atomic<bool> attr_set{false};
     if (attr_set) return 0;
-    const void* ks[8] = {reinterpret_cast<const void*>(&block_fwd_rs_kernel<false, false, false>), reinterpret_cast<const void*>(&block_fwd_rs_kernel<true, false, false>),
+    const void* ks[12] = {reinterpret_cast<const void*>(&block_fwd_rs_kernel<false, false, false>), reinterpret_cast<const void*>(&block_fwd_rs_kernel<true, false, false>),
                          reinterpret_cast<const void*>(&block_fwd_rs_kernel<false, true, false>), reinterpret_cast<const void*>(&block_fwd_rs_kernel<true, true, false>),
                          reinterpret_cast<const void*>(&block_fwd_rs_kernel<false, false, true>), reinterpret_cast<const void*>(&block_fwd_rs_kernel<true, false, true>),
-                         reinterpret_cast<const void*>(&block_fwd_rs_kernel<false, true, true>), reinterpret_cast<const void*>(&block_fwd_rs_kernel<true, true, true>)};
-    for (int i = 0; i < 8; ++i) {
+                         reinterpret_cast<const void*>(&block_fwd_rs_kernel<false, true, true>), reinterpret_cast<const void*>(&block_fwd_rs_kernel<true, true, true>),
+                         reinterpret_cast<const void*>(&block_fwd_rs_kernel<false, false, false, true>), reinterpret_cast<const void*>(&block_fwd_rs_kernel<true, false, false, true>),
+                         reinterpret_cast<const void*>(&block_fwd_rs_kernel<false, false, true, true>), reinterpret_cast<const void*>(&block_fwd_rs_kernel<true, false, true, true>)};
+    for (int i = 0; i < 12; ++i) {
         hipError_t e = hipFuncSetAttribute(ks[i], hipFuncAttributeMaxDynamicSharedMemorySize, (int)sizeof(Fwd3Smem));
         if (e != hipSuccess) return (int)e;
     }
@@ -889,6 +898,18 @@
     int rc = fwd3_attrs();
     if (rc) return rc;
     ProfScope ps(K_BLOCK_FWD, st);
+    if (a.tile_list) {
+        if (a.nlisted < 1 || a.nlisted > a.ntiles || grid < 1 || grid > a.nlisted) return MSST_ERR_BADARG;
+        if ((a.nlisted + grid - 1) / grid > F3_MAX_STEPS) return MSST_ERR_UNSUPPORTED;
+        if (a.half) {
+            if (a.drop.thr) hipLaunchKernelGGL((block_fwd_rs_kernel<true, false, true, true>), dim3(grid), dim3(512), smem, st, a);
+            else hipLaunchKernelGGL((block_fwd_rs_kernel<false, false, true, true>), dim3(grid), dim3(512), smem, st, a);
+        } else {
+            if (a.drop.thr) hipLaunchKernelGGL((block_fwd_rs_kernel<true, false, false, true>), dim3(grid), dim3(512), smem, st, a);
+            else hipLaunchKernelGGL((block_fwd_rs_kernel<false, false, false, true>), dim3(grid), dim3(512), smem, st, a);
+        }
+        return (int)hipGetLastError();
+    }
     if (a.half) {
         if (a.drop.thr) hipLaunchKernelGGL((block_fwd_rs_kernel<true, false, true>), dim3(grid), dim3(512), smem, st, a);
         else hipLaunchKernelGGL((block_fwd_rs_kernel<false, false, true>), dim3(grid), dim3(512), smem, st, a);
diff --git a/maskedsst_amd/csrc/msst_kernels.h b/maskedsst_amd/csrc/msst_kernels.h
--- a/maskedsst_amd/csrc/msst_kernels.h
+++ b/maskedsst_amd/csrc/msst_kernels.h
@@ -41,6 +41,8 @@
     int dbg;
     unsigned long long* stamps;
     Drop drop;
+    const int* tile_list = nullptr;
+    int nlisted = 0;
 };
 
 #define MSST_MAX_STACK 16
@@ -264,6 +266,22 @@
 int launch_scene_border_zero(float* dscene, long rows, int Hs, int Ws, int rows_in, int cols_in, hipStream_t st);
 int launch_head_bwd_target(const float* dpred, const int* csr_ptr, const int* csr_pos, const float* gout, float gscale, float* dtarget,
                            int B, int S, int N, int P, int K, hipStream_t st);
+
+#define MSST_ZERO_MAX_BUFS 64
+struct ZeroRowsBuf {
+    char* base;
+    int row_bytes;
+    short per_tile;
+    short wide;
+};
+struct ZeroRowsArgs {
+    const int* unlisted;
+    TileMap tm;
+    int ntiles;
+    long ntok;
+    ZeroRowsBuf buf[MSST_ZERO_MAX_BUFS];
+};
+int launch_zero_unlisted_rows(const ZeroRowsArgs& a, int n_unlisted, int nbuf, hipStream_t st);
 
 enum KernelId {
     K_PREP = 0, K_TOK_FWD, K_BLOCK_FWD, K_HEAD_FWD, K_LOSS_REDUCE, K_HEAD_BWD, K_REDUCE, K_BWD_MLP, K_BWD_ATTN,
diff --git a/maskedsst_amd/csrc/msst_zero_rows.hip b/maskedsst_amd/csrc/msst_zero_rows.hip
--- /dev/null
+++ b/maskedsst_amd/csrc/msst_zero_rows.hip
@@ -0,0 +1,38 @@
+#include "msst_dev.h"
+#include "msst_kernels.h"
+
+namespace msst {
+
+__global__ __launch_bounds__(256) void zero_unlisted_rows_kernel(ZeroRowsArgs a) {
+    const int tile = a.unlisted[blockIdx.x];
+    if (tile < 0 || tile >= a.ntiles) return;
+    const ZeroRowsBuf zb = a.buf[blockIdx.y];
+    const TileMap tm = a.tm;
+    const int unit = zb.wide ? 16 : 4, upr = zb.row_bytes / unit;
+    if (zb.per_tile) {
+        char* const p = zb.base + (long)tile * zb.row_bytes;
+        for (int i = (int)threadIdx.x; i < upr; i += 256) {
+            if (zb.wide) *reinterpret_cast<f32x4*>(p + 16 * i) = zero4();
+            else *reinterpret_cast<float*>(p + 4 * i) = 0.f;
+        }
+        return;
+    }
+    const int rows = tm.TS * tm.L;
+    for (int i = (int)threadIdx.x; i < rows * upr; i += 256) {
+        const int r = i / upr, u = i - r * upr;
+        const long tok = tm.token(tile, r);
+        if (tok < 0 || tok >= a.ntok) continue;
+        char* const p = zb.base + tok * zb.row_bytes + (long)u * unit;
+        if (zb.wide) *reinterpret_cast<f32x4*>(p) = zero4();
+        else *reinterpret_cast<float*>(p) = 0.f;
+    }
+}
+
+int launch_zero_unlisted_rows(const ZeroRowsArgs& a, int n_unlisted, int nbuf, hipStream_t st) {
+    if (n_unlisted < 1 || nbuf < 1) return 0;
+    if (nbuf > MSST_ZERO_MAX_BUFS || n_unlisted > a.ntiles) return MSST_ERR_BADARG;
+    hipLaunchKernelGGL(zero_unlisted_rows_kernel, dim3(n_unlisted, nbuf), dim3(256), 0, st, a);
+    return (int)hipGetLastError();
+}
+
+}
diff --git a/maskedsst_amd/engine.py b/maskedsst_amd/engine.py
--- a/maskedsst_amd/engine.py
+++ b/maskedsst_amd/engine.py
@@ -40,6 +40,16 @@
             self.n = img.shape[0] * self.grid[0] * self.grid[1]
         else:
             self.n = origins.shape[0] if kind == "listed" else img.shape[0]
+
+
+class TileList:
+
+    def __init__(self, order, n_listed):
+        self.order, self.n_listed, self.used, self.zeroed = order, int(n_listed), False, False
+
+    @property
+    def n_unlisted(self):
+        return self.order.shape[0] - self.n_listed
 
 
 _TOK_FWD = {("batch", False): "msst_tokenize_fwd", ("batch", True): "msst_tokenize_fwd", ("tiles", False): "msst_tokenize_scene_fwd_train",
@@ -410,7 +420,7 @@
             _lib.check(fn(*lead, *par, V(pos_a), V(pos_b), split, *mask_args, _p(out[win0:] if win0 else out), *dims, *drop_args, st), name)
         return out
 
-    def blocks_fwd(self, x0, save=True, drop=(0.0, 0)):
+    def blocks_fwd(self, x0, save=True, drop=(0.0, 0), tiles=None):
         acts = [x0]
         x1s = []
         flags = _kernel_flags()
@@ -422,17 +432,26 @@
         stacked = role_split and want_stack != "0"
         i0 = 0
         self.fwd_launch_blocks = []
+        self.fwd_tiles_listed = None
+        if tiles is not None and tiles.order.shape[0] != int(self.lib.msst_block_tiles(MODE_SPECTRAL, x0.shape[0], self.S, self.N)):
+            raise ValueError("blocks_fwd: the TileList is not one of this batch's spectral tiling")
         while i0 < len(layers):
             i1 = i0
             while i1 < len(layers) and layers[i1][0] == layers[i0][0] and i1 - i0 < 16:
                 i1 += 1
             use = stacked and (want_stack == "1" or self._tiles_per_workgroup(layers[i0][0], x0.shape[0]) <= STACK_MAX_TILES)
+            listed = (tiles is not None and not use and save and x1_bf16 and want_lse and layers[i0][0] == "spectral" and i1 == len(layers)
+                      and 0 < tiles.n_listed < tiles.order.shape[0] and self.tile_list_capable() and self.ln1_xn_ok()
+                      and self._tiles_per_workgroup("spectral", x0.shape[0]) <= 1024)
             if use and self._fwd_stack(acts, x1s, i0, i1, save, drop, x1_bf16, want_lse):
                 self.fwd_launch_blocks.append(i1 - i0)
             else:
                 for i in range(i0, i1):
-                    self._fwd_block(acts, x1s, i, save, drop, x1_bf16, want_lse, flags)
+                    self._fwd_block(acts, x1s, i, save, drop, x1_bf16, want_lse, flags, tiles if listed else None)
                 self.fwd_launch_blocks += [1] * (i1 - i0)
+                if listed:
+                    tiles.used = True
+                    self.fwd_tiles_listed = (tiles.n_listed, tiles.order.shape[0])
             i0 = i1
         return acts, x1s
 
@@ -473,7 +492,7 @@
         x1._msst_rstd = bool(wrote & _lib.SAVED_RSTD) and x1._msst_lse is not None
         x1._msst_half = bool(self.fwd_half)
 
-    def _fwd_block(self, acts, x1s, i, save, drop, x1_bf16, want_lse, flags):
+    def _fwd_block(self, acts, x1s, i, save, drop, x1_bf16, want_lse, flags, tiles=None):
         x = acts[-1]
         B = x.shape[0]
         S, N, H = self.S, self.N, self.enc.heads
@@ -486,12 +505,19 @@
         if xn is not None and want_lse:
             lse = torch.empty(int(self.lib.msst_block_lse_floats(mode, B, S, N, H)), dtype=torch.float32, device=x.device)
         wrote = ctypes.c_int(0)
-        _lib.check(self.lib.msst_block_fwd(ctypes.byref(self._bw[i]), _p(x), _p(y), _p(x1), mode, B, S, N, H,
-                                           self.prec | flags | (_lib.X1_BF16 if x1_bf16 else 0) | self._half_flag(flags), self.max_grid, drop[0], drop[1], i, _p(xn), _p(lse),
-                                           ctypes.byref(wrote), _stream()),
-                   "msst_block_fwd")
+        args = (ctypes.byref(self._bw[i]), _p(x), _p(y), _p(x1), mode, B, S, N, H,
+                self.prec | flags | (_lib.X1_BF16 if x1_bf16 else 0) | self._half_flag(flags), self.max_grid, drop[0], drop[1], i, _p(xn), _p(lse),
+                ctypes.byref(wrote))
+        if tiles is None:
+            _lib.check(self.lib.msst_block_fwd(*args, _stream()), "msst_block_fwd")
+        else:
+            _lib.check(self.lib.msst_block_fwd_listed(*args, _p(tiles.order), tiles.n_listed, _stream()), "msst_block_fwd_listed")
+            need = _lib.SAVED_XN | _lib.SAVED_LSE | _lib.SAVED_RSTD
+            if x1 is None or (wrote.value & need) != need:
+                raise RuntimeError("msst_block_fwd_listed: the forward did not save what the listed backward needs")
         if x1 is not None:
             self._attach_saved(x1, wrote.value, xn, lse)
+            x1._msst_listed = tiles is not None
         acts.append(y)
         x1s.append(x1)
 
@@ -661,8 +687,11 @@
         dab = torch.empty(ntok * 96, dtype=torch.bfloat16, device=device) if self.prec != PREC_F32 else None
         return dx1, part, slab, dab
 
-    def blocks_bwd(self, acts, x1s, dy, drop=(0.0, 0)):
+    def blocks_bwd(self, acts, x1s, dy, drop=(0.0, 0), tiles=None):
         H = self.enc.heads
+        listed = [i for i, t in enumerate(x1s) if getattr(t, "_msst_listed", False)]
+        if listed and (tiles is None or not tiles.used):
+            raise RuntimeError("blocks_bwd: these activations come from a listed forward (blocks_fwd(tiles=...)); pass the same TileList")
         ntok = dy.shape[0] * self.S * self.N
         ws = self._bwd_workspace(dy.shape[0], dy.device)
         x1_bf16 = len(x1s) > 0 and all(t.dtype == torch.bfloat16 for t in x1s)
@@ -673,12 +702,35 @@
                  and nparts <= 4 and os.environ.get("MSST_BWD_CHAIN", "1") != "0" and self.enc.depth > 0
                  and ntok * 384 < 2 ** 31 - 16 and nparts * ntok * 192 < 2 ** 31 - 16)
         ln1_from_xn = (chain and x1_bf16 and os.environ.get("MSST_LN1_XN", "1") != "0"
-                       and all(getattr(t, "_msst_rstd", False) for t in x1s) and self.ln1_xn_ok())
+                       and all(getattr(t, "_msst_rstd", False) for t in x1s) and (self.ln1_xn_ok() or bool(listed)))
         self.last_bwd_ln1_from_xn = bool(ln1_from_xn)
+        if listed:
+            if not ln1_from_xn:
+                raise RuntimeError("blocks_bwd: a listed forward needs the chained backward with MSST_LN1_FROM_XN "
+                                   "(MSST_BWD_CHAIN / MSST_LN1_XN / kernel flags changed between the forward and its backward?)")
+            self.zero_unlisted(acts, x1s, tiles)
         if chain:
             return self._blocks_bwd_chained(acts, x1s, dy, drop, ws,
                                             (_lib.X1_BF16 if x1_bf16 else 0) | (_lib.LN1_FROM_XN if ln1_from_xn else 0))
         return self._blocks_bwd_unchained(acts, x1s, dy, drop, ws)
+
+    def zero_unlisted(self, acts, x1s, tiles):
+        if tiles is None or not tiles.used or tiles.zeroed:
+            return
+        H = self.enc.heads
+        ntiles = tiles.order.shape[0]
+        y = acts[-1]
+        bufs = [(y.data_ptr(), 96 * y.element_size(), 0)]
+        for x1 in x1s:
+            if not getattr(x1, "_msst_listed", False):
+                continue
+            lse = x1._msst_lse
+            bufs += [(x1.data_ptr(), 96 * x1.element_size(), 0), (x1._msst_xn.data_ptr(), 96 * x1._msst_xn.element_size(), 0),
+                     (lse.data_ptr(), H * 64 * 4, 1), (lse.data_ptr() + ntiles * H * 64 * 4, 4, 0)]
+        table = (_lib.MsstRowBuf * len(bufs))(*[_lib.MsstRowBuf(*b) for b in bufs])
+        _lib.check(self.lib.msst_zero_unlisted_rows(_p(tiles.order[tiles.n_listed:]), tiles.n_unlisted, table, len(bufs),
+                                                    MODE_SPECTRAL, y.shape[0], self.S, self.N, _stream()), "msst_zero_unlisted_rows")
+        tiles.zeroed = True
 
     def _blocks_bwd_chained(self, acts, x1s, dy, drop, ws, x1flags):
         B = dy.shape[0]
@@ -865,17 +917,38 @@
         bm = bool_mask.cpu().numpy() if torch.is_tensor(bool_mask) else np.asarray(bool_mask)
         ix = idx.cpu().numpy() if torch.is_tensor(idx) else np.asarray(idx)
         ptr, pos = inverse_csr(ix, T)
-        mask_u8, idx32, csr_ptr, csr_pos = self._upload(img.device, bm.astype(np.uint8), ix.astype(np.int32), ptr, pos)
+        ix32 = ix.astype(np.int32)
         names = [n for n, _ in self.trainable()]
         params = [p for _, p in self.trainable()]
         want_img = src.kind == "batch" and img.requires_grad
-        if not torch.is_grad_enabled() or not (want_img or any(p.requires_grad for p in params)):
+        train = torch.is_grad_enabled() and (want_img or any(p.requires_grad for p in params))
+        split = self.spectral_tile_split(ix32) if train and self.tile_list_capable() else None
+        up = self._upload(img.device, bm.astype(np.uint8), ix32, ptr, pos, *(() if split is None else (split[0],)))
+        mask_u8, idx32, csr_ptr, csr_pos = up[:4]
+        tiles = None if split is None else TileList(up[4], split[1])
+        if not train:
             self.prep_weights()
             x0 = self.tokenize(src, mask_u8)
             acts, _ = self.blocks_fwd(x0, save=False, drop=self.dropout_state())
             loss, _, _ = self.head_fwd(acts[-1], src, idx32)
             return loss
-        return _SimMIMLossFn.apply(self, names, self.dropout_state(), src, img, mask_u8, idx32, csr_ptr, csr_pos, *params)
+        return _SimMIMLossFn.apply(self, names, self.dropout_state(), src, img, mask_u8, idx32, csr_ptr, csr_pos, tiles, *params)
+
+    def tile_list_capable(self):
+        env = os.environ.get
+        H = self.enc.heads
+        return (env("MSST_TILE_LIST", "1") != "0" and self.enc.depth > 0 and self._role_split(_kernel_flags())
+                and env("MSST_X1_BF16", "1") != "0" and env("MSST_LSE", "1") != "0" and env("MSST_BWD_CHAIN", "1") != "0"
+                and env("MSST_LN1_XN", "1") != "0" and H % 2 == 0 and H // 2 <= 4)
+
+    def spectral_tile_split(self, idx):
+        from .masking import spectral_tile_split
+        B = idx.shape[0]
+        TS = 64 // self.S
+        order, n_listed = spectral_tile_split(idx, self.N, TS)
+        if order.shape[0] != int(self.lib.msst_block_tiles(MODE_SPECTRAL, B, self.S, self.N)):
+            raise RuntimeError("spectral_tile_split: the host's tiling is not the library's (msst_block_tiles)")
+        return order, n_listed
 
     def _block_param_names(self):
         return [n for n, _ in self.trainable() if n.startswith(("spatial.", "spectral."))]
@@ -1182,33 +1255,34 @@
 class _SimMIMLossFn(torch.autograd.Function):
 
     @staticmethod
-    def forward(ctx, eng, names, drop, src, img, mask_u8, idx32, csr_ptr, csr_pos, *params):
+    def forward(ctx, eng, names, drop, src, img, mask_u8, idx32, csr_ptr, csr_pos, tiles, *params):
         eng.prep_weights()
         x0 = eng.tokenize(src, mask_u8)
-        acts, x1s = eng.blocks_fwd(x0, save=True, drop=drop)
+        acts, x1s = eng.blocks_fwd(x0, save=True, drop=drop, tiles=tiles)
         ctx.drop = drop
         loss, dpred, _ = eng.head_fwd(acts[-1], src, idx32)
         ctx.eng = eng
         ctx.names = names
-        ctx.stash = (src, mask_u8, csr_ptr, csr_pos, acts, x1s, dpred)
+        ctx.stash = (src, mask_u8, csr_ptr, csr_pos, acts, x1s, dpred, tiles)
         return loss
 
     @staticmethod
     def backward(ctx, gout):
         eng = ctx.eng
-        src, mask_u8, csr_ptr, csr_pos, acts, x1s, dpred = ctx.stash
+        src, mask_u8, csr_ptr, csr_pos, acts, x1s, dpred, tiles = ctx.stash
         ctx.stash = None
-        needs = ctx.needs_input_grad[9:]
+        needs = ctx.needs_input_grad[10:]
         _refuse_accumulation(eng, ctx.names, needs)
         gout = gout.contiguous().float()
+        eng.zero_unlisted(acts, x1s, tiles)
         dy = eng.head_bwd(acts[-1], dpred, csr_ptr, csr_pos, gout)
-        dx0 = eng.blocks_bwd(acts, x1s, dy, drop=ctx.drop)
+        dx0 = eng.blocks_bwd(acts, x1s, dy, drop=ctx.drop, tiles=tiles)
         dimg = None
         if ctx.needs_input_grad[4] and src.kind == "batch":
             dimg = eng.tokenize_input_bwd(src, mask_u8, dx0, eng.head_bwd_target(dpred, csr_ptr, csr_pos, gout))
         if any(needs):
             eng.tokenize_bwd(src, mask_u8, dx0)
-        return (None,) * 4 + (dimg,) + (None,) * 4 + _grad_views(eng, ctx.names, needs)
+        return (None,) * 4 + (dimg,) + (None,) * 5 + _grad_views(eng, ctx.names, needs)
 
 
 def _refuse_accumulation(eng, names, needs=None):
diff --git a/maskedsst_amd/masking.py b/maskedsst_amd/masking.py
--- a/maskedsst_amd/masking.py
+++ b/maskedsst_amd/masking.py
@@ -98,3 +98,14 @@
     cnt = np.bincount(flat, minlength=B * (num_tokens + 1)).reshape(B, num_tokens + 1)
     ptr = np.cumsum(cnt, axis=1).astype(np.int32)
     return ptr, pos
+
+
+def spectral_tile_split(idx, N, TS):
+    idx = np.asarray(idx)
+    B = idx.shape[0]
+    ntiles = -(-B * N // TS)
+    need = np.zeros(ntiles * TS, dtype=bool)
+    need[(idx % N + np.arange(B, dtype=idx.dtype)[:, None] * N).ravel()] = True
+    listed = need.reshape(ntiles, TS).any(axis=1)
+    order = np.concatenate((np.flatnonzero(listed), np.flatnonzero(~listed))).astype(np.int32)
+    return order, int(listed.sum())
```

After: 11330 samples/s, median of 6. No clear change (+0.4%).
